# LARS-research/RED-GNN

Hardware: AMD Instinct MI355X
Metric: edges aggregated/sec + MRR-eval queries/sec, family KG n_layer=3 at 1/2/4/8 GPU (higher is better)
Workload: dtype f32; 1 GPU; C2 synthetic KG 10000 entities / 50 relations / 200000 triples (seed 1234), n_layer=3 hidden_dim=64 attn_dim=5, eval step = expansion + fused layers + GRU/readout + filtered ranking, 1024 queries per GPU; batch_per_gpu=1024, global_batch=1024

## Files before the change

include/redgnn.h:

```cpp
#ifndef REDGNN_H
#define REDGNN_H

#include <stddef.h>
#include <stdint.h>

#ifdef __cplusplus
extern "C" {
#endif

typedef struct rg_graph rg_graph;
typedef struct rg_frontier rg_frontier;

const char* rg_last_error(void);
int rg_version(void);
int rg_hipgraph_fill_nodes(void* hip_graph);

int rg_graph_create(int32_t n_ent, int32_t n_rel, const int32_t* triples_host, int64_t n,
                    int add_inverse, rg_graph** out);
int rg_graph_create_device(int32_t n_ent, int32_t n_rel, const int32_t* triples_dev, int64_t n,
                           int add_inverse, void* stream, rg_graph** out);
int rg_graph_export_packs(const rg_graph* g, int32_t* n_packs, int32_t* n_vrows, int32_t* ent_host, int32_t* pack_host, int32_t* rows_host,
                          int32_t* vrows_host);
int rg_tgraph_create(int32_t n_ent, int32_t n_rela_rows, int32_t n_time, const int32_t* quads_host, int64_t n,
                     rg_graph** out);
int rg_tgraph_create_excluding(int32_t n_ent, int32_t n_rela_rows, int32_t n_time, const int32_t* quads_host, int64_t n,
                               const int64_t* exclude_rows_host, int64_t n_exclude, rg_graph** out);
int rg_graph_destroy(rg_graph* g);
int64_t rg_graph_n_fact(const rg_graph* g);
int rg_graph_export(const rg_graph* g, int32_t* out_ptr_host, int32_t* out_rel_tail_host,
                    int32_t* in_ptr_host, int32_t* in_head_rel_host);
int rg_graph_export_time(const rg_graph* g, int32_t* out_time_host, int32_t* in_time_host);

size_t rg_frontier_workspace_bytes(int32_t n_ent, int32_t batch, int32_t n_levels);
int rg_frontier_create(int32_t n_ent, int32_t batch, int32_t n_levels, void* workspace_dev,
                       size_t workspace_bytes, rg_frontier** out);
int rg_frontier_destroy(rg_frontier* f);
int rg_frontier_reset(rg_frontier* f, const int32_t* q_sub_dev, void* stream);
int rg_frontier_reset_nodes(rg_frontier* f, const int32_t* nodes_dev, int64_t n, void* stream);
int rg_frontier_expand(rg_frontier* f, const rg_graph* g, int64_t* counts_host, void* stream);
int rg_frontier_expand_async(rg_frontier* f, const rg_graph* g, void* stream);
int rg_frontier_expand_nodes_async(rg_frontier* f, const rg_graph* g, int32_t* nodes_out, int32_t* prev_idx_out, void* stream);
int rg_frontier_set_edge_hint(rg_frontier* f, int64_t n_edges);
const int32_t* rg_frontier_count_ptr(const rg_frontier* f);
int rg_frontier_level_counts(const rg_frontier* f, int64_t* counts_host, void* stream);
int rg_frontier_nodes(const rg_frontier* f, int32_t* nodes_out, int32_t* prev_idx_out,
                      int32_t* old_nodes_new_idx_out, void* stream);
size_t rg_frontier_edges_scratch_bytes(int64_t n_new);
int rg_frontier_edges(const rg_frontier* f, const rg_graph* g, int32_t level,
                      const int32_t* nodes_new, int64_t n_new, int32_t* edges_out,
                      int32_t* row_ptr_out, void* scratch_dev, void* stream);

size_t rg_layer_fwd_scratch_bytes(const rg_frontier* f, const rg_graph* g, int32_t ld);
int rg_layer_fwd_plan(const rg_frontier* f, const rg_graph* g, int32_t level, int64_t n_old, int64_t n_new,
                      int64_t n_edges, int32_t ld);
int rg_layer_fwd(const rg_frontier* f, const rg_graph* g, int32_t level, int64_t n_new,
                 const float* hidden, const float* rela, int32_t d, int32_t ld,
                 const float* a_s, const float* a_r, const float* a_q, int32_t ap,
                 const float* w_alpha, const float* b_alpha, int32_t attn_dim,
                 float* agg_out, void* scratch_dev, size_t scratch_bytes, int32_t walk, void* stream);

int rg_attn_tables(int32_t n_layer, int32_t n_rela_rows, int32_t batch, int32_t d, int32_t ld, int32_t attn_dim, int32_t ap,
                   const float* const* rela, const float* const* Wr, const float* const* Wqr, const float* const* bqr,
                   const int64_t* q_rel, float* a_r_out, float* a_q_out, float* rela_pad_out, void* stream);

int rg_tlayer_fwd(const rg_frontier* f, const rg_graph* g, int32_t level, int64_t n_new, const int32_t* q_time,
                  const float* hidden_dir, const float* rela_dir, const float* time_dir, int32_t d, int32_t ld,
                  const float* a_s, const float* a_r, const float* a_q, int32_t ap,
                  const float* w_alpha, const float* b_alpha, int32_t attn_dim,
                  float* agg_out, void* scratch_dev, size_t scratch_bytes, void* stream);

int rg_frontier_set_window(rg_frontier* f, const int32_t* win_lo_dev, const int32_t* win_hi_dev, int32_t n_data);
int rg_xlayer_fwd(const rg_frontier* f, const rg_graph* g, int32_t level, int64_t n_new, const int32_t* q_time,
                  const int32_t* loop_time, const int32_t* row_time, int32_t n_data,
                  const float* hidden_p, const float* rela_p, const float* time_p, int32_t n_tab, int32_t d, int32_t ld,
                  const float* a_s, const float* a_r, const float* a_q, int32_t ap,
                  const float* w_alpha, const float* b_alpha, int32_t attn_dim,
                  float* agg_out, void* scratch_dev, size_t scratch_bytes, void* stream);

size_t rg_layer_bwd_scratch_bytes(const rg_frontier* f, const rg_graph* g, int32_t ld, int32_t ap);
int rg_layer_bwd(const rg_frontier* f, const rg_graph* g, int32_t level, int64_t n_old,
                 const float* hidden, const float* rela, int32_t d, int32_t ld,
                 const float* a_s, const float* a_r, const float* a_q, int32_t ap,
                 const float* w_alpha, const float* b_alpha, int32_t attn_dim,
                 const float* grad_agg,
                 float* grad_hidden, float* grad_rela, float* grad_a_s, float* grad_a_r, float* grad_a_q,
                 float* grad_w_alpha, float* grad_b_alpha,
                 void* scratch_dev, size_t scratch_bytes, void* stream);

size_t rg_tlayer_bwd_scratch_bytes(const rg_frontier* f, const rg_graph* g, int32_t ld, int32_t ap);
int rg_tlayer_bwd(const rg_frontier* f, const rg_graph* g, int32_t level, int64_t n_old, const int32_t* q_time,
                  const float* hidden_dir, const float* rela_dir, const float* time_dir, int32_t d, int32_t ld,
                  const float* a_s, const float* a_r, const float* a_q, int32_t ap,
                  const float* w_alpha, const float* b_alpha, int32_t attn_dim,
                  const float* grad_agg,
                  float* grad_hidden_dir, float* grad_rela_dir, float* grad_time_dir, float* grad_a_s, float* grad_a_r,
                  float* grad_a_q, float* grad_w_alpha,
                  void* scratch_dev, size_t scratch_bytes, void* stream);

int rg_xlayer_bwd(const rg_frontier* f, const rg_graph* g, int32_t level, int64_t n_old, const int32_t* q_time,
                  const int32_t* loop_time, const int32_t* row_time, int32_t n_data,
                  const float* hidden_p, const float* rela_p, const float* time_p, int32_t n_tab, int32_t d, int32_t ld,
                  const float* a_s, const float* a_r, const float* a_q, int32_t ap,
                  const float* w_alpha, const float* b_alpha, int32_t attn_dim,
                  const float* grad_agg,
                  float* grad_hidden_p, float* grad_rela_p, float* grad_time_p, float* grad_a_s, float* grad_a_r,
                  float* grad_a_q, float* grad_w_alpha,
                  void* scratch_dev, size_t scratch_bytes, void* stream);

int rg_dense_fwd_supported(int32_t d, int32_t attn_dim);
int rg_dense_fwd(int64_t n, int32_t d, int32_t ld, const float* agg, const float* hidden_prev,
                 const int32_t* prev_idx, const float* W_h, int32_t act,
                 const float* w_ih, const float* w_hh, const float* b_ih, const float* b_hh,
                 const float* Ws_next, int32_t attn_dim, int32_t ap, float* a_s_out,
                 const float* W_final, const int32_t* nodes, int32_t n_ent, float* scores_all,
                 float* hidden_out, int32_t precision, void* scratch, int64_t scratch_bytes, void* stream);
int64_t rg_dense_scratch_bytes(int32_t d, int32_t precision);

int rg_split3_roundtrip(const float* x, int64_t n_rows, int32_t cols, float* back, float* parts, void* stream);
int rg_split3_product_check(int32_t which, int64_t n, int32_t d, const float* agg, const float* hidden_prev, const int32_t* prev_idx,
                            const float* W_h, int32_t act, const float* w_ih, const float* w_hh, const float* b_ih, const float* b_hh,
                            float* out, void* stream);

size_t rg_gram_tn_scratch_bytes(int32_t m, int32_t n);
int rg_gram_tn(const float* g, int64_t ldg, int32_t m, const float* x, int64_t ldx, int32_t n, int64_t n_rows, float* out, float* colsum,
               void* scratch_dev, size_t scratch_bytes, void* stream);

int rg_rank(const float* scores, int32_t batch, int32_t n_ent,
            const int32_t* ans_ptr, const int32_t* ans_idx,
            const int32_t* filt_ptr, const int32_t* filt_idx,
            float* ranks_out, void* stream);

int rg_topk(const float* scores, int32_t batch, int32_t n_ent, int32_t k, const int64_t* q_key,
            const int64_t* known_keys, const int64_t* known_ptr, const int32_t* known_idx, int64_t n_keys,
            int32_t* idx_out, float* score_out, void* stream);

int rg_dense_fwd_dev(int64_t n_cap, const int32_t* n_dev, int64_t n_hint, int32_t d, int32_t ld, const float* agg, const float* hidden_prev,
                     const int32_t* prev_idx, const float* W_h, int32_t act,
                     const float* w_ih, const float* w_hh, const float* b_ih, const float* b_hh,
                     const float* Ws_next, int32_t attn_dim, int32_t ap, float* a_s_out,
                     const float* W_final, const int32_t* nodes, int32_t n_ent, float* scores_all,
                     float* hidden_out, int32_t precision, void* scratch, int64_t scratch_bytes, void* stream);

int rg_dense_train_fwd(int64_t n, int32_t d, const float* agg, const float* hidden_prev, const int32_t* prev_idx,
                       const float* W_h, int32_t act, const float* w_ih, const float* w_hh, const float* b_ih, const float* b_hh,
                       const float* mask, float* hidden_out, float* x_out, float* gates_ws_out, void* stream);

int rg_dense_train_fwd_as(int64_t n, int32_t d, const float* agg, const float* hidden_prev, const int32_t* prev_idx,
                          const float* W_h, int32_t act, const float* w_ih, const float* w_hh, const float* b_ih, const float* b_hh,
                          const float* mask, const float* Ws_next, int32_t attn_dim, int32_t ap,
                          float* hidden_out, float* x_out, float* gates_ws_out, float* a_s_out, void* stream);

int rg_rows_addmm(const float* base, int64_t ldb, const float* g, int64_t ldg, int32_t k, const float* W, int32_t n, int64_t n_rows,
                  float* out, int64_t ldo, void* stream);

int rg_dense_train_bwd(int64_t n, int32_t d, const float* grad_hidden, const float* gates_ws, const float* x, const float* mask,
                       float keep, int32_t act, const float* W_h, const float* w_ih, const float* w_hh,
                       float* grad_gates_i, float* grad_gates_h, float* grad_pre, float* grad_agg, float* grad_h0, void* stream);

int rg_dense_train_bwd2(int64_t n, int32_t d, const float* grad_hidden, const float* gates_ws, const float* x, const float* mask,
                        float keep, int32_t act, const float* W_h, const float* w_ih, const float* w_hh, const int32_t* prev_idx,
                        float* grad_gates_i, float* grad_gates_hn, float* grad_pre, float* grad_agg, float* grad_prev, void* stream);

size_t rg_explain_scratch_bytes(const rg_frontier* f);
int rg_explain_seed(const rg_frontier* f, int32_t batch, int32_t n_ent, int32_t level, const int32_t* objs, uint32_t* marks_out,
                    uint8_t* reached_out, void* stream);
int rg_explain_count(const rg_frontier* f, const rg_graph* g, int32_t batch, int32_t n_ent, int32_t level, const uint32_t* marks,
                     const float* a_s, const float* a_r, const float* a_q, int32_t ap, const float* w_alpha, const float* b_alpha,
                     int32_t attn_dim, float min_alpha, uint32_t* marks_prev_out, int32_t* word_ptr_out, void* scratch,
                     size_t scratch_bytes, int64_t* n_edges_host, void* stream);
int rg_explain_emit(const rg_frontier* f, const rg_graph* g, int32_t batch, int32_t n_ent, int32_t level, const uint32_t* marks,
                    const float* a_s, const float* a_r, const float* a_q, int32_t ap, const float* w_alpha, const float* b_alpha,
                    int32_t attn_dim, float min_alpha, const int32_t* word_ptr, int32_t* edges_out, float* alpha_out, void* stream);
int rg_explain_gather(int64_t n, int32_t hop, int32_t batch, const int32_t* edges, const float* alpha, const int64_t* row_first,
                      const int64_t* row_base, int64_t n_out, int32_t* edges_out, float* alpha_out, void* stream);

int rg_texplain_count(const rg_frontier* f, const rg_graph* g, int32_t batch, int32_t n_ent, int32_t level, const uint32_t* marks,
                      const float* a_s, const float* a_r, const float* a_q, int32_t ap, const float* w_alpha, const float* b_alpha,
                      int32_t attn_dim, float min_alpha, uint32_t* marks_prev_out, int32_t* word_ptr_out, void* scratch,
                      size_t scratch_bytes, int64_t* n_edges_host, void* stream);
int rg_texplain_emit(const rg_frontier* f, const rg_graph* g, int32_t batch, int32_t n_ent, int32_t level, const uint32_t* marks,
                     const float* a_s, const float* a_r, const float* a_q, int32_t ap, const float* w_alpha, const float* b_alpha,
                     int32_t attn_dim, float min_alpha, const int32_t* word_ptr, int32_t* edges_out, float* alpha_out,
                     int32_t* time_out, void* stream);

int rg_attn_profile(const rg_frontier* f, const rg_graph* g, int32_t batch, int32_t n_ent, int32_t level, int64_t n_old,
                    const float* a_s, const float* a_r, const float* a_q, int32_t ap, const float* w_alpha, const float* b_alpha,
                    int32_t attn_dim, int64_t* sum_out, int64_t* count_out, void* stream);

int rg_tattn_profile(const rg_frontier* f, const rg_graph* g, int32_t batch, int32_t n_ent, int32_t level, int64_t n_old,
                     const int32_t* q_time, const float* a_s, const float* a_r, const float* a_q, int32_t ap, const float* w_alpha,
                     const float* b_alpha, int32_t attn_dim, int64_t* sum_out, int64_t* count_out, void* stream);

#ifdef __cplusplus
}
#endif
#endif
```

red-gnn_amd/_lib.py:

```python
import ctypes as C
import os

_PKG = os.path.dirname(os.path.abspath(__file__))
LIB_PATH = os.environ.get("RG_LIB") or os.path.join(_PKG, "libredgnn.so")

SYMBOLS = [
    "rg_last_error", "rg_version", "rg_hipgraph_fill_nodes",
    "rg_graph_create", "rg_graph_create_device", "rg_graph_export_packs", "rg_tgraph_create", "rg_tgraph_create_excluding", "rg_graph_destroy", "rg_graph_n_fact", "rg_graph_export",
    "rg_frontier_workspace_bytes", "rg_frontier_create", "rg_frontier_destroy", "rg_frontier_reset",
    "rg_frontier_reset_nodes", "rg_frontier_expand", "rg_frontier_nodes", "rg_frontier_edges_scratch_bytes", "rg_frontier_edges",
    "rg_layer_fwd_scratch_bytes", "rg_layer_fwd", "rg_layer_fwd_plan", "rg_tlayer_fwd", "rg_xlayer_fwd", "rg_frontier_set_window", "rg_layer_bwd_scratch_bytes", "rg_layer_bwd", "rg_tlayer_bwd_scratch_bytes", "rg_tlayer_bwd", "rg_xlayer_bwd", "rg_dense_fwd_supported", "rg_dense_scratch_bytes", "rg_dense_fwd", "rg_dense_fwd_dev", "rg_dense_train_fwd", "rg_dense_train_fwd_as", "rg_rows_addmm", "rg_dense_train_bwd", "rg_dense_train_bwd2", "rg_split3_roundtrip", "rg_split3_product_check", "rg_gram_tn_scratch_bytes", "rg_gram_tn", "rg_rank",
    "rg_frontier_expand_async", "rg_frontier_expand_nodes_async", "rg_frontier_set_edge_hint", "rg_frontier_count_ptr", "rg_frontier_level_counts", "rg_attn_tables",
    "rg_explain_scratch_bytes", "rg_explain_seed", "rg_explain_count", "rg_explain_emit", "rg_explain_gather",
    "rg_topk",
    "rg_attn_profile",
    "rg_graph_export_time", "rg_texplain_count", "rg_texplain_emit", "rg_tattn_profile",
]

_lib = None


class NativeError(RuntimeError):
    pass


def lib():
    global _lib
    if _lib is not None:
        return _lib
    if not os.path.exists(LIB_PATH):
        raise NativeError(
            "libredgnn.so is missing at %s: the HIP extension is not built. Run "
            "`python -c 'import __graft_entry__ as g; g.build()'` (needs hipcc). There is no CPU fallback." % LIB_PATH)
    import torch
    L = C.CDLL(LIB_PATH)
    vp, i32, i64, sz = C.c_void_p, C.c_int32, C.c_int64, C.c_size_t
    L.rg_last_error.restype = C.c_char_p
    L.rg_version.restype = C.c_int
    L.rg_hipgraph_fill_nodes.argtypes = [vp]
    L.rg_graph_create.argtypes = [i32, i32, vp, i64, C.c_int, C.POINTER(vp)]
    L.rg_graph_create_device.argtypes = [i32, i32, vp, i64, C.c_int, vp, C.POINTER(vp)]
    L.rg_graph_export_packs.argtypes = [vp, C.POINTER(i32), C.POINTER(i32), vp, vp, vp, vp]
    L.rg_tgraph_create.argtypes = [i32, i32, i32, vp, i64, C.POINTER(vp)]
    L.rg_tgraph_create_excluding.argtypes = [i32, i32, i32, vp, i64, vp, i64, C.POINTER(vp)]
    L.rg_graph_destroy.argtypes = [vp]
    L.rg_graph_n_fact.argtypes = [vp]
    L.rg_graph_n_fact.restype = i64
    L.rg_graph_export.argtypes = [vp, vp, vp, vp, vp]
    L.rg_frontier_workspace_bytes.argtypes = [i32, i32, i32]
    L.rg_frontier_workspace_bytes.restype = sz
    L.rg_frontier_create.argtypes = [i32, i32, i32, vp, sz, C.POINTER(vp)]
    L.rg_frontier_destroy.argtypes = [vp]
    L.rg_frontier_reset.argtypes = [vp, vp, vp]
    L.rg_frontier_reset_nodes.argtypes = [vp, vp, i64, vp]
    L.rg_frontier_expand.argtypes = [vp, vp, C.POINTER(i64), vp]
    L.rg_frontier_expand_async.argtypes = [vp, vp, vp]
    L.rg_frontier_expand_nodes_async.argtypes = [vp, vp, vp, vp, vp]
    L.rg_frontier_set_edge_hint.argtypes = [vp, i64]
    L.rg_attn_tables.argtypes = [i32, i32, i32, i32, i32, i32, i32, vp, vp, vp, vp, vp, vp, vp, vp, vp]
    L.rg_frontier_count_ptr.argtypes = [vp]
    L.rg_frontier_count_ptr.restype = vp
    L.rg_frontier_level_counts.argtypes = [vp, C.POINTER(i64), vp]
    L.rg_frontier_nodes.argtypes = [vp, vp, vp, vp, vp]
    L.rg_frontier_edges_scratch_bytes.argtypes = [i64]
    L.rg_frontier_edges_scratch_bytes.restype = sz
    L.rg_frontier_edges.argtypes = [vp, vp, i32, vp, i64, vp, vp, vp, vp]
    L.rg_layer_fwd_scratch_bytes.argtypes = [vp, vp, i32]
    L.rg_layer_fwd_scratch_bytes.restype = sz
    L.rg_layer_fwd.argtypes = [vp, vp, i32, i64, vp, vp, i32, i32, vp, vp, vp, i32, vp, vp, i32, vp, vp, sz, i32, vp]
    L.rg_layer_fwd_plan.argtypes = [vp, vp, i32, i64, i64, i64, i32]
    L.rg_tlayer_fwd.argtypes = [vp, vp, i32, i64, vp, vp, vp, vp, i32, i32, vp, vp, vp, i32, vp, vp, i32, vp, vp, sz, vp]
    L.rg_xlayer_fwd.argtypes = [vp, vp, i32, i64, vp, vp, vp, i32, vp, vp, vp, i32, i32, i32, vp, vp, vp, i32, vp, vp, i32, vp, vp, sz, vp]
    L.rg_frontier_set_window.argtypes = [vp, vp, vp, i32]
    L.rg_layer_bwd_scratch_bytes.argtypes = [vp, vp, i32, i32]
    L.rg_layer_bwd_scratch_bytes.restype = sz
    L.rg_layer_bwd.argtypes = [vp, vp, i32, i64, vp, vp, i32, i32, vp, vp, vp, i32, vp, vp, i32,
                               vp, vp, vp, vp, vp, vp, vp, vp, vp, sz, vp]
    L.rg_tlayer_bwd_scratch_bytes.argtypes = [vp, vp, i32, i32]
    L.rg_tlayer_bwd_scratch_bytes.restype = sz
    L.rg_tlayer_bwd.argtypes = [vp, vp, i32, i64, vp, vp, vp, vp, i32, i32, vp, vp, vp, i32, vp, vp, i32,
                                vp, vp, vp, vp, vp, vp, vp, vp, vp, sz, vp]
    L.rg_xlayer_bwd.argtypes = [vp, vp, i32, i64, vp, vp, vp, i32, vp, vp, vp, i32, i32, i32, vp, vp, vp, i32, vp, vp, i32,
                                vp, vp, vp, vp, vp, vp, vp, vp, vp, sz, vp]
    L.rg_dense_fwd_supported.argtypes = [i32, i32]
    L.rg_dense_fwd.argtypes = [i64, i32, i32, vp, vp, vp, vp, i32, vp, vp, vp, vp, vp, i32, i32, vp, vp, vp, i32, vp, vp, i32, vp, i64, vp]
    L.rg_dense_scratch_bytes.argtypes = [i32, i32]
    L.rg_dense_scratch_bytes.restype = i64
    L.rg_dense_fwd_dev.argtypes = [i64, vp, i64, i32, i32, vp, vp, vp, vp, i32, vp, vp, vp, vp, vp, i32, i32, vp, vp, vp, i32, vp, vp, i32, vp, i64, vp]
    L.rg_dense_train_fwd.argtypes = [i64, i32, vp, vp, vp, vp, i32, vp, vp, vp, vp, vp, vp, vp, vp, vp]
    L.rg_dense_train_fwd_as.argtypes = [i64, i32, vp, vp, vp, vp, i32, vp, vp, vp, vp, vp, vp, i32, i32, vp, vp, vp, vp, vp]
    L.rg_rows_addmm.argtypes = [vp, i64, vp, i64, i32, vp, i32, i64, vp, i64, vp]
    L.rg_dense_train_bwd.argtypes = [i64, i32, vp, vp, vp, vp, C.c_float, i32, vp, vp, vp, vp, vp, vp, vp, vp, vp]
    L.rg_dense_train_bwd2.argtypes = [i64, i32, vp, vp, vp, vp, C.c_float, i32, vp, vp, vp, vp, vp, vp, vp, vp, vp, vp]
    L.rg_rank.argtypes = [vp, i32, i32, vp, vp, vp, vp, vp, vp]
    L.rg_topk.argtypes = [vp, i32, i32, i32, vp, vp, vp, vp, i64, vp, vp, vp]
    L.rg_split3_roundtrip.argtypes = [vp, i64, i32, vp, vp, vp]
    L.rg_gram_tn_scratch_bytes.argtypes = [i32, i32]
    L.rg_gram_tn_scratch_bytes.restype = sz
    L.rg_gram_tn.argtypes = [vp, i64, i32, vp, i64, i32, i64, vp, vp, vp, sz, vp]
    L.rg_split3_product_check.argtypes = [i32, i64, i32, vp, vp, vp, vp, i32, vp, vp, vp, vp, vp, vp]
    L.rg_explain_scratch_bytes.argtypes = [vp]
    L.rg_explain_scratch_bytes.restype = sz
    L.rg_explain_seed.argtypes = [vp, i32, i32, i32, vp, vp, vp, vp]
    L.rg_explain_count.argtypes = [vp, vp, i32, i32, i32, vp, vp, vp, vp, i32, vp, vp, i32, C.c_float, vp, vp, vp, sz,
                                   C.POINTER(i64), vp]
    L.rg_explain_emit.argtypes = [vp, vp, i32, i32, i32, vp, vp, vp, vp, i32, vp, vp, i32, C.c_float, vp, vp, vp, vp]
    L.rg_explain_gather.argtypes = [i64, i32, i32, vp, vp, vp, vp, i64, vp, vp, vp]
    L.rg_attn_profile.argtypes = [vp, vp, i32, i32, i32, i64, vp, vp, vp, i32, vp, vp, i32, vp, vp, vp]
    L.rg_graph_export_time.argtypes = [vp, vp, vp]
    L.rg_texplain_count.argtypes = L.rg_explain_count.argtypes
    L.rg_texplain_emit.argtypes = [vp, vp, i32, i32, i32, vp, vp, vp, vp, i32, vp, vp, i32, C.c_float, vp, vp, vp, vp, vp]
    L.rg_tattn_profile.argtypes = [vp, vp, i32, i32, i32, i64, vp, vp, vp, vp, i32, vp, vp, i32, vp, vp, vp]
    _lib = L
    return L


def check(rc):
    if rc != 0:
        raise NativeError(lib().rg_last_error().decode("utf-8", "replace"))


def ptr(t):
    if t is None:
        return None
    if hasattr(t, "data_ptr"):
        return C.c_void_p(t.data_ptr())
    return C.c_void_p(t.ctypes.data)


def stream_ptr():
    import torch
    return C.c_void_p(torch.cuda.current_stream().cuda_stream)
```

red-gnn_amd/csrc/common.h:

```cpp
#pragma once
#include <hip/hip_runtime.h>
#include <stdint.h>
#include <stdio.h>
#include <string>
#include <type_traits>

#include "redgnn.h"

namespace rg {

void set_error(const char* fmt, ...);

#define RG_CHECK(cond, ...)                 \
  do {                                      \
    if (!(cond)) {                          \
      ::rg::set_error(__VA_ARGS__);         \
      return 1;                             \
    }                                       \
  } while (0)

#define RG_HIP(expr)                                                                  \
  do {                                                                                \
    hipError_t e_ = (expr);                                                           \
    if (e_ != hipSuccess) {                                                           \
      ::rg::set_error("%s failed: %s (%s:%d)", #expr, hipGetErrorString(e_), __FILE__, \
                      __LINE__);                                                      \
      return 1;                                                                       \
    }                                                                                 \
  } while (0)

#define RG_LAUNCH_CHECK() RG_HIP(hipGetLastError())

int zero_async(void* p, size_t bytes, hipStream_t s);
int zero2_async(void* p1, size_t bytes1, void* p2, size_t bytes2, hipStream_t s);
int copy_words_async(void* dst, const void* src, int n_words, hipStream_t s);

static inline int64_t ceil_div(int64_t a, int64_t b) { return (a + b - 1) / b; }
static inline size_t align_up(size_t x, size_t a) { return (x + a - 1) / a * a; }

size_t scan_scratch_elems(int64_t n);
int scan_exclusive(const uint32_t* in, int32_t* out, int64_t n, bool popc, int32_t* total_dev,
                   int32_t* scratch, hipStream_t s);

template <typename F>
inline int with_ap4(int ap4, const char* who, F&& f) {
  switch (ap4) {
    case 1: return f(std::integral_constant<int, 1>());
    case 2: return f(std::integral_constant<int, 2>());
    case 3: return f(std::integral_constant<int, 3>());
    case 4: return f(std::integral_constant<int, 4>());
    case 8: return f(std::integral_constant<int, 8>());
    default: set_error("%s: padded attention dim %d not in {4,8,12,16,32}", who, ap4 * 4); return 1;
  }
}

template <typename F>
inline int with_g(int ld4, F&& f) {
  if (ld4 <= 4) return f(std::integral_constant<int, 4>());
  if (ld4 <= 8) return f(std::integral_constant<int, 8>());
  if (ld4 <= 16) return f(std::integral_constant<int, 16>());
  if (ld4 <= 32) return f(std::integral_constant<int, 32>());
  return f(std::integral_constant<int, 64>());
}

__device__ __forceinline__ float4 f4zero() { return make_float4(0.f, 0.f, 0.f, 0.f); }

template <int CTRL>
__device__ __forceinline__ float dpp_add(float v) {
  const int t = __builtin_amdgcn_update_dpp(0, __float_as_int(v), CTRL, 0xf, 0xf, false);
  return v + __int_as_float(t);
}

template <int G>
__device__ __forceinline__ float group_sum(float v) {
  if constexpr (G >= 16) {
    v = dpp_add<0x128>(v);
    v = dpp_add<0x124>(v);
    v = dpp_add<0x122>(v);
    v = dpp_add<0x121>(v);
    if constexpr (G >= 32) v += __shfl_xor(v, 16, 64);
    if constexpr (G >= 64) v += __shfl_xor(v, 32, 64);
  } else {
    for (int o = G / 2; o > 0; o >>= 1) v += __shfl_xor(v, o, 64);
  }
  return v;
}

}

#include <vector>
namespace rg { int place_rows_best_fit(const int4* vrows, int32_t n_vrows, std::vector<int4>* place, std::vector<int32_t>* pack_nrows); }

constexpr int RG_VROW_MAX = 128;
struct rg_vrows {
  int32_t n = 0, n_split = 0, n_slots = 0;
  int4* rows = nullptr;
  int4* split = nullptr;
};

constexpr int RG_PACK = 128;
struct rg_packs {
  int32_t n = 0;
  int2* ent = nullptr;
  int4* pack = nullptr;
  int2* rows = nullptr;
};

struct rg_graph {
  void* arena = nullptr;
  int32_t n_ent = 0, n_rel = 0;
  int32_t n_rela_rows = 0;
  int32_t n_time = 0;
  int32_t* in_time = nullptr;
  int32_t* out_time = nullptr;
  int64_t n_fact = 0;
  int32_t max_in_deg = 0, max_out_deg = 0;
  int32_t* out_ptr = nullptr;
  int2* out_rt = nullptr;
  int32_t* in_ptr = nullptr;
  int2* in_hr = nullptr;
  uint32_t* in_pk = nullptr;
  uint32_t* out_pk = nullptr;
  rg_vrows in_vr, out_vr;
  rg_packs in_pk_packs;
  int32_t* rel_ptr = nullptr;
  int2* rel_ht = nullptr;
  rg_vrows rel_vr;
  int32_t* rel_tm = nullptr;
  int32_t* time_ptr = nullptr;
  int2* time_ht = nullptr;
  int32_t* time_rel = nullptr;
  rg_vrows time_vr;
};

constexpr int RG_MAX_LEVELS = 16;
constexpr int RG_QSTRIDE = 32;
constexpr size_t RG_QUEUE_BYTES = 8 * RG_QSTRIDE * sizeof(int32_t);
struct rg_frontier {
  int32_t n_ent = 0, B = 0, BW = 0, W = 0, n_levels = 0;
  uint32_t* bitsT[2] = {nullptr, nullptr};
  int2* bm[RG_MAX_LEVELS] = {};
  uint32_t* words_tmp = nullptr;
  int32_t* prefix_tmp = nullptr;
  int32_t* scan_scratch = nullptr;
  int32_t* counters = nullptr;
  const int32_t* win_lo = nullptr;
  const int32_t* win_hi = nullptr;
  int32_t win_n_data = 0;
  mutable bool queues_clean = false;
  int32_t* queues = nullptr;
  int64_t* counts_pinned = nullptr;
  int level = -1;
  int tcur = 0;
  int64_t n_nodes[RG_MAX_LEVELS] = {};
  int64_t n_edges = 0;
  int64_t edge_hint = -1;
  const int2* bm_of(int lvl) const { return bm[lvl % n_levels]; }
};
```

red-gnn_amd/csrc/frontier.hip:

```cpp
#include <string.h>

#include "attn.h"

namespace {

__global__ void reset_level0_kernel(const int32_t* __restrict__ q_sub, int B, int n_ent, int BW, int W, uint32_t* __restrict__ bitsT,
                                    int2* __restrict__ bm0, int32_t* __restrict__ counters) {
  const int64_t i = (int64_t)blockIdx.x * blockDim.x + threadIdx.x;
  if (i >= (int64_t)B * W) return;
  const int b = (int)(i / W), w = (int)(i - (int64_t)b * W);
  const int e = q_sub[b];
  const bool ok = e >= 0 && e < n_ent;
  const int ew = ok ? e >> 5 : W;
  bm0[i] = make_int2(w == ew ? (int)(1u << (e & 31)) : 0, b + (w > ew ? 1 : 0));
  if (w == 0) {
    if (ok) atomicOr(&bitsT[(int64_t)e * BW + (b >> 5)], 1u << (b & 31));
    else atomicOr((unsigned*)&counters[1], 1u);
    if (b == 0) { counters[0] = B; counters[4] = B; }
  }
}

__device__ __forceinline__ void end_of_hop(int32_t* __restrict__ counters, int32_t* __restrict__ queues, int slot, int t) {
  if (t < 4) {
    const int32_t v = counters[t];
    if (slot >= 0) counters[slot + t] = v;
    counters[8 + t] = v;
  }
  if (t >= 8 && t < 16) queues[(t - 8) * RG_QSTRIDE] = 0;
}
__global__ void snapshot_kernel(int32_t* __restrict__ counters, int32_t* __restrict__ queues, int slot) {
  end_of_hop(counters, queues, slot, threadIdx.x);
  __syncthreads();
  if (threadIdx.x == 0) { counters[2] = 0; counters[3] = 0; }
}

__global__ void reset_nodes_kernel(const int32_t* __restrict__ nodes, int64_t n, int B, int n_ent, int BW,
                                   uint32_t* __restrict__ bitsT, int32_t* counters) {
  const int64_t i = (int64_t)blockIdx.x * blockDim.x + threadIdx.x;
  if (i >= n) return;
  const int b = nodes[2 * i], e = nodes[2 * i + 1];
  if (e < 0 || e >= n_ent || b < 0 || b >= B) { atomicOr((unsigned*)&counters[1], 1u); return; }
  atomicOr(&bitsT[(int64_t)e * BW + (b >> 5)], 1u << (b & 31));
}

__global__ __launch_bounds__(256) void hop_or_kernel(const int4* __restrict__ vrows, int n_vrows,
                                                     const int2* __restrict__ in_hr, const uint32_t* __restrict__ oldT,
                                                     uint32_t* __restrict__ newT, int BW, int WL) {
  const int wave = (blockIdx.x * blockDim.x + threadIdx.x) >> 6;
  const int lane = threadIdx.x & 63;
  if (wave >= n_vrows) return;
  const int4 row = vrows[wave];
  const int t = row.x, beg = row.y, end = row.y + row.z;
  const int wl = lane & (WL - 1);
  const int el = lane / WL, EL = 64 / WL;
  for (int w0 = 0; w0 < BW; w0 += WL) {
    const int w = w0 + wl;
    uint32_t acc = 0;
    if (w < BW) {
      for (int j = beg + el; j < end; j += 4 * EL) {
        int hh[4];
#pragma unroll
        for (int u = 0; u < 4; ++u) hh[u] = (j + u * EL < end) ? in_hr[j + u * EL].x : -1;
#pragma unroll
        for (int u = 0; u < 4; ++u)
          if (hh[u] >= 0) acc |= oldT[(int64_t)hh[u] * BW + w];
      }
    }
    for (int o = WL; o < 64; o <<= 1) acc |= __shfl_xor(acc, o, 64);
    if (el == 0 && w < BW && acc) atomicOr(&newT[(int64_t)t * BW + w], acc);
  }
}

__global__ __launch_bounds__(256) void hop_or_window_kernel(const int4* __restrict__ vrows, int n_vrows, const int2* __restrict__ in_hr,
                                                            const int32_t* __restrict__ in_row, const uint32_t* __restrict__ oldT,
                                                            uint32_t* __restrict__ newT, int BW, int WL, int B, const int32_t* __restrict__ win_lo,
                                                            const int32_t* __restrict__ win_hi, int n_data, unsigned long long* total) {
  const int wave = (blockIdx.x * blockDim.x + threadIdx.x) >> 6;
  const int lane = threadIdx.x & 63;
  if (wave >= n_vrows) return;
  const int4 row = vrows[wave];
  const int t = row.x, beg = row.y, end = row.y + row.z;
  const int wl = lane & (WL - 1);
  const int el = lane / WL, EL = 64 / WL;
  unsigned long long cnt = 0;
  for (int w0 = 0; w0 < BW; w0 += WL) {
    const int w = w0 + wl;
    uint32_t acc = 0;
    if (w < BW) {
      for (int j = beg + el; j < end; j += EL) {
        uint32_t v = oldT[(int64_t)in_hr[j].x * BW + w];
        if (v) {
          const int r = in_row[j];
          if (r < n_data) {
            uint32_t m = 0;
            for (uint32_t rest = v; rest; rest &= rest - 1) {
              const int bit = __ffs((int)rest) - 1, b = w * 32 + bit;
              if (b < B && r >= win_lo[b] && r < win_hi[b]) m |= 1u << bit;
            }
            v = m;
          }
          acc |= v;
          cnt += __popc(v);
        }
      }
    }
    for (int o = WL; o < 64; o <<= 1) acc |= __shfl_xor(acc, o, 64);
    if (el == 0 && w < BW && acc) atomicOr(&newT[(int64_t)t * BW + w], acc);
  }
  for (int o = 32; o > 0; o >>= 1) cnt += __shfl_down(cnt, o, 64);
  if (lane == 0 && cnt) atomicAdd(total, cnt);
}

__global__ __launch_bounds__(256) void hop_prologue_kernel(const int32_t* __restrict__ out_ptr,
                                                           const uint32_t* __restrict__ oldT, uint32_t* __restrict__ newT,
                                                           int n_ent, int BW, unsigned long long* total) {
  const int64_t i = (int64_t)blockIdx.x * blockDim.x + threadIdx.x;
  unsigned long long v = 0;
  if (i < (int64_t)n_ent * BW) {
    const int h = (int)(i / BW);
    if (out_ptr) v = (unsigned long long)(out_ptr[h + 1] - out_ptr[h]) * __popc(oldT[i]);
    newT[i] = 0u;
  }
  for (int o = 32; o > 0; o >>= 1) v += __shfl_down(v, o, 64);
  __shared__ unsigned long long ws[4];
  if ((threadIdx.x & 63) == 0) ws[threadIdx.x >> 6] = v;
  __syncthreads();
  if (threadIdx.x == 0) {
    unsigned long long s = ws[0] + ws[1] + ws[2] + ws[3];
    if (s) atomicAdd(total, s);
  }
}

__global__ __launch_bounds__(256) void transpose_kernel(const uint32_t* __restrict__ bitsT, uint32_t* __restrict__ words,
                                                        int n_ent, int B, int BW, int W, int n_pairs) {
  const int wave = (blockIdx.x * blockDim.x + threadIdx.x) >> 6;
  const int lane = threadIdx.x & 63;
  if (wave >= BW * n_pairs) return;
  const int bw = wave / n_pairs, pair = wave - bw * n_pairs;
  const int e = pair * 64 + lane;
  const uint32_t v = (e < n_ent) ? bitsT[(int64_t)e * BW + bw] : 0u;
  uint32_t lo = 0, hi = 0;
#pragma unroll
  for (int b = 0; b < 32; ++b) {
    const unsigned long long m = __ballot((v >> b) & 1u);
    if (lane == b) { lo = (uint32_t)m; hi = (uint32_t)(m >> 32); }
  }
  const int batch = bw * 32 + lane;
  if (lane < 32 && batch < B) {
    const int ew = pair * 2;
    words[(int64_t)batch * W + ew] = lo;
    if (ew + 1 < W) words[(int64_t)batch * W + ew + 1] = hi;
  }
}

__global__ void pack_kernel(const uint32_t* __restrict__ words, const int32_t* __restrict__ prefix,
                            int2* __restrict__ bm, int64_t n) {
  const int64_t i = (int64_t)blockIdx.x * blockDim.x + threadIdx.x;
  if (i < n) bm[i] = make_int2((int)words[i], prefix[i]);
}

__global__ void emit_nodes_kernel(const int2* __restrict__ bm_new, const int2* __restrict__ bm_old, int B, int W,
                                  int32_t* __restrict__ nodes, int32_t* __restrict__ prev_idx,
                                  int32_t* __restrict__ old_new) {
  const int64_t t = (int64_t)blockIdx.x * blockDim.x + threadIdx.x;
  const int64_t i = t >> 5;
  const int pos = (int)(t & 31);
  if (i >= (int64_t)B * W) return;
  const int2 nw = bm_new[i];
  if (!rg::bm_has(nw, pos)) return;
  const int64_t idx = rg::bm_rank(nw, pos);
  const int b = (int)(i / W), w = (int)(i - (int64_t)b * W);
  if (nodes) reinterpret_cast<int2*>(nodes)[idx] = make_int2(b, w * 32 + pos);
  if (prev_idx || old_new) {
    int prev = -1;
    if (bm_old) {
      const int2 ow = bm_old[i];
      if (rg::bm_has(ow, pos)) prev = rg::bm_rank(ow, pos);
    }
    if (prev_idx) prev_idx[idx] = prev;
    if (old_new && prev >= 0) old_new[prev] = (int32_t)idx;
  }
}

__device__ __forceinline__ int rank_in(const int2* __restrict__ bm, int b, int W, int e, bool* present) {
  const int2 wp = bm[(int64_t)b * W + (e >> 5)];
  *present = rg::bm_has(wp, e);
  return rg::bm_rank(wp, e);
}

__global__ void edge_count_kernel(const int32_t* __restrict__ nodes_new, int64_t n_new, const int32_t* __restrict__ in_ptr,
                                  const int2* __restrict__ in_hr, const int2* __restrict__ bm_old, int W,
                                  uint32_t* __restrict__ deg) {
  const int64_t i = (int64_t)blockIdx.x * blockDim.x + threadIdx.x;
  if (i >= n_new) return;
  const int b = nodes_new[2 * i], t = nodes_new[2 * i + 1];
  int c = 0;
  for (int j = in_ptr[t]; j < in_ptr[t + 1]; ++j) {
    bool p;
    rank_in(bm_old, b, W, in_hr[j].x, &p);
    c += p;
  }
  deg[i] = c;
}

__global__ void edge_fill_kernel(const int32_t* __restrict__ nodes_new, int64_t n_new, const int32_t* __restrict__ in_ptr,
                                 const int2* __restrict__ in_hr, const int2* __restrict__ bm_old, int W,
                                 const int32_t* __restrict__ row_ptr, int32_t* __restrict__ edges) {
  const int64_t i = (int64_t)blockIdx.x * blockDim.x + threadIdx.x;
  if (i >= n_new) return;
  const int b = nodes_new[2 * i], t = nodes_new[2 * i + 1];
  int64_t o = row_ptr[i];
  for (int j = in_ptr[t]; j < in_ptr[t + 1]; ++j) {
    const int2 hr = in_hr[j];
    bool p;
    const int s = rank_in(bm_old, b, W, hr.x, &p);
    if (p) {
      int32_t* e = edges + 6 * o;
      e[0] = b; e[1] = hr.x; e[2] = hr.y; e[3] = t; e[4] = s; e[5] = (int32_t)i;
      ++o;
    }
  }
}

constexpr int SMALL_T = 1024;
constexpr int SMALL_MAX_WORDS = 12288;

__global__ __launch_bounds__(SMALL_T) void build_level_small_kernel(const uint32_t* __restrict__ bitsT, int n_ent, int B, int BW, int W,
                                                                    int n_pairs, int2* __restrict__ bm_new, const int2* __restrict__ bm_old,
                                                                    int32_t* __restrict__ counters, int32_t* __restrict__ queues, int slot,
                                                                    int32_t* __restrict__ nodes, int32_t* __restrict__ prev_idx,
                                                                    int32_t* __restrict__ old_new) {
  extern __shared__ uint32_t words[];
  __shared__ int32_t wsum[SMALL_T / 64];
  const int lane = threadIdx.x & 63, wv = threadIdx.x >> 6;
  const int nw = B * W;
  for (int task = wv; task < BW * n_pairs; task += SMALL_T / 64) {
    const int bw = task / n_pairs, pair = task - bw * n_pairs;
    const int e = pair * 64 + lane;
    const uint32_t v = (e < n_ent) ? bitsT[(int64_t)e * BW + bw] : 0u;
    uint32_t lo = 0, hi = 0;
#pragma unroll
    for (int b = 0; b < 32; ++b) {
      const unsigned long long m = __ballot((v >> b) & 1u);
      if (lane == b) { lo = (uint32_t)m; hi = (uint32_t)(m >> 32); }
    }
    const int batch = bw * 32 + lane;
    if (lane < 32 && batch < B) {
      words[batch * W + 2 * pair] = lo;
      if (2 * pair + 1 < W) words[batch * W + 2 * pair + 1] = hi;
    }
  }
  __syncthreads();
  const int per = (nw + SMALL_T - 1) / SMALL_T;
  const int beg = min((int)threadIdx.x * per, nw), end = min(beg + per, nw);
  int32_t sum = 0;
  for (int i = beg; i < end; ++i) sum += __popc(words[i]);
  int32_t inc = sum;
#pragma unroll
  for (int o = 1; o < 64; o <<= 1) {
    const int32_t t = __shfl_up(inc, o, 64);
    if (lane >= o) inc += t;
  }
  if (lane == 63) wsum[wv] = inc;
  __syncthreads();
  int32_t pre = inc - sum, total = 0;
  for (int w = 0; w < SMALL_T / 64; ++w) {
    const int32_t x = wsum[w];
    if (w < wv) pre += x;
    total += x;
  }
  for (int i = beg; i < end; ++i) {
    uint32_t w = words[i];
    bm_new[i] = make_int2((int)w, pre);
    if (nodes || prev_idx || old_new) {
      const int b = i / W, e0 = (i - b * W) * 32;
      uint32_t ow = 0; int op = 0;
      if ((prev_idx || old_new) && bm_old) { const int2 o = bm_old[i]; ow = (uint32_t)o.x; op = o.y; }
      int idx = pre;
      for (uint32_t rest = w; rest; rest &= rest - 1, ++idx) {
        const int pos = __ffs((int)rest) - 1;
        if (nodes) reinterpret_cast<int2*>(nodes)[idx] = make_int2(b, e0 + pos);
        const int prev = ((ow >> pos) & 1u) ? op + __popc(ow & ((1u << pos) - 1u)) : -1;
        if (prev_idx) prev_idx[idx] = prev;
        if (old_new && prev >= 0) old_new[prev] = idx;
      }
    }
    pre += __popc(w);
  }
  const int t = threadIdx.x;
  if (t < 4) {
    const int32_t v = t == 0 ? total : counters[t];
    if (t == 0) counters[0] = total;
    if (slot >= 0) counters[slot + t] = v;
    counters[8 + t] = v;
  }
  if (t >= 8 && t < 16) queues[(t - 8) * RG_QSTRIDE] = 0;
  __syncthreads();
  if (t == 0) { counters[2] = 0; counters[3] = 0; }
}

__global__ void set_last_kernel(int32_t* row_ptr, int64_t n, const int32_t* total) { row_ptr[n] = *total; }

size_t ws_layout(int32_t n_ent, int32_t B, int32_t n_levels, size_t* off ) {
  const size_t BW = (B + 31) / 32, W = (n_ent + 31) / 32;
  size_t o = 0;
  auto take = [&](size_t bytes) { size_t r = o; o = rg::align_up(o + bytes, 256); return r; };
  off[0] = take((size_t)n_ent * BW * 4);
  off[1] = take((size_t)n_ent * BW * 4);
  off[2] = take((size_t)B * W * 4);
  off[3] = take((size_t)B * W * 4);
  off[4] = take(rg::scan_scratch_elems((int64_t)B * W) * 4);
  off[5] = take(1024 + RG_QUEUE_BYTES);
  off[6] = take((size_t)n_levels * B * W * 8);
  return o;
}

}

extern "C" {

size_t rg_frontier_workspace_bytes(int32_t n_ent, int32_t batch, int32_t n_levels) {
  if (n_ent <= 0 || batch <= 0 || n_levels < 2 || n_levels > RG_MAX_LEVELS) return 0;
  size_t off[8];
  return ws_layout(n_ent, batch, n_levels, off);
}

int rg_frontier_create(int32_t n_ent, int32_t batch, int32_t n_levels, void* ws, size_t ws_bytes, rg_frontier** out) {
  RG_CHECK(out != nullptr, "rg_frontier_create: out is NULL");
  *out = nullptr;
  RG_CHECK(n_ent > 0 && batch > 0, "rg_frontier_create: n_ent=%d batch=%d must be positive", n_ent, batch);
  RG_CHECK(n_levels >= 2 && n_levels <= RG_MAX_LEVELS, "rg_frontier_create: n_levels=%d not in [2,%d]", n_levels, RG_MAX_LEVELS);
  RG_CHECK((int64_t)n_ent * batch < ((int64_t)1 << 31), "rg_frontier_create: batch*n_ent = %lld does not fit int32",
           (long long)n_ent * batch);
  size_t off[8];
  const size_t need = ws_layout(n_ent, batch, n_levels, off);
  RG_CHECK(ws != nullptr && ws_bytes >= need, "rg_frontier_create: workspace %zu B < required %zu B", ws_bytes, need);
  RG_CHECK(((uintptr_t)ws & 255) == 0, "rg_frontier_create: workspace must be 256-B aligned");
  rg_frontier* f = new rg_frontier();
  f->n_ent = n_ent; f->B = batch; f->BW = (batch + 31) / 32; f->W = (n_ent + 31) / 32; f->n_levels = n_levels;
  char* base = (char*)ws;
  f->bitsT[0] = (uint32_t*)(base + off[0]);
  f->bitsT[1] = (uint32_t*)(base + off[1]);
  f->words_tmp = (uint32_t*)(base + off[2]);
  f->prefix_tmp = (int32_t*)(base + off[3]);
  f->scan_scratch = (int32_t*)(base + off[4]);
  f->counters = (int32_t*)(base + off[5]);
  f->queues = f->counters + 256;
  for (int l = 0; l < n_levels; ++l) f->bm[l] = (int2*)(base + off[6] + (size_t)l * batch * f->W * 8);
  if (hipHostMalloc((void**)&f->counts_pinned, 1024, hipHostMallocDefault) != hipSuccess) {
    delete f;
    rg::set_error("rg_frontier_create: hipHostMalloc failed");
    return 1;
  }
  *out = f;
  return 0;
}

int rg_frontier_destroy(rg_frontier* f) {
  if (!f) return 0;
  if (f->counts_pinned) (void)hipHostFree(f->counts_pinned);
  delete f;
  return 0;
}

static int build_level(rg_frontier* f, hipStream_t s) {
  const int n_pairs = (f->W + 1) / 2;
  const int64_t waves = (int64_t)f->BW * n_pairs;
  hipLaunchKernelGGL(transpose_kernel, dim3(rg::ceil_div(waves, 4)), dim3(256), 0, s, f->bitsT[f->tcur], f->words_tmp,
                     f->n_ent, f->B, f->BW, f->W, n_pairs);
  RG_LAUNCH_CHECK();
  const int64_t nw = (int64_t)f->B * f->W;
  if (rg::scan_exclusive(f->words_tmp, f->prefix_tmp, nw, true, &f->counters[0], f->scan_scratch, s)) return 1;
  hipLaunchKernelGGL(pack_kernel, dim3(rg::ceil_div(nw, 256)), dim3(256), 0, s, f->words_tmp, f->prefix_tmp,
                     f->bm[f->level % f->n_levels], nw);
  RG_LAUNCH_CHECK();
  return 0;
}

int rg_frontier_reset(rg_frontier* f, const int32_t* q_sub, void* stream) {
  RG_CHECK(f && q_sub, "rg_frontier_reset: NULL argument");
  hipStream_t s = (hipStream_t)stream;
  f->level = 0; f->tcur = 0; f->n_edges = 0;
  if (rg::zero2_async(f->bitsT[0], rg::align_up((size_t)f->n_ent * f->BW * 4, 16), f->counters, 1024, s)) return 1;
  f->queues_clean = false;
  const int64_t nw = (int64_t)f->B * f->W;
  hipLaunchKernelGGL(reset_level0_kernel, dim3(rg::ceil_div(nw, 256)), dim3(256), 0, s, q_sub, f->B, f->n_ent, f->BW, f->W,
                     f->bitsT[0], f->bm[0], f->counters);
  RG_LAUNCH_CHECK();
  f->n_nodes[0] = f->B;
  return 0;
}

int rg_frontier_set_window(rg_frontier* f, const int32_t* win_lo, const int32_t* win_hi, int32_t n_data) {
  RG_CHECK(f != nullptr, "rg_frontier_set_window: frontier is NULL");
  RG_CHECK((win_lo == nullptr) == (win_hi == nullptr) && n_data >= 0, "rg_frontier_set_window: give both bounds (or neither)");
  f->win_lo = win_lo; f->win_hi = win_hi; f->win_n_data = n_data;
  return 0;
}

int rg_frontier_reset_nodes(rg_frontier* f, const int32_t* nodes, int64_t n, void* stream) {
  RG_CHECK(f && (nodes || n == 0) && n >= 0, "rg_frontier_reset_nodes: bad argument");
  hipStream_t s = (hipStream_t)stream;
  f->level = 0; f->tcur = 0; f->n_edges = 0;
  if (rg::zero2_async(f->bitsT[0], rg::align_up((size_t)f->n_ent * f->BW * 4, 16), f->counters, 1024, s)) return 1;
  f->queues_clean = false;
  if (n > 0) {
    hipLaunchKernelGGL(reset_nodes_kernel, dim3(rg::ceil_div(n, 256)), dim3(256), 0, s, nodes, n, f->B, f->n_ent, f->BW,
                       f->bitsT[0], f->counters);
    RG_LAUNCH_CHECK();
  }
  if (build_level(f, s)) return 1;
  if (rg::copy_words_async(&f->counters[4], &f->counters[0], 1, s)) return 1;
  f->n_nodes[0] = n;
  return 0;
}

static int enqueue_expand(rg_frontier* f, const rg_graph* g, hipStream_t s, int32_t* nodes = nullptr, int32_t* prev_idx = nullptr) {
  const uint32_t* oldT = f->bitsT[f->tcur];
  uint32_t* newT = f->bitsT[f->tcur ^ 1];
  int WL = 1;
  while (WL < f->BW && WL < 64) WL <<= 1;
  const bool windowed = f->win_lo != nullptr;
  RG_CHECK(!windowed || g->in_time, "rg_frontier_expand: time windows are set but the graph carries no data-row ids (rg_tgraph_create)");
  hipLaunchKernelGGL(hop_prologue_kernel, dim3(rg::ceil_div((int64_t)f->n_ent * f->BW, 256)), dim3(256), 0, s,
                     windowed ? (const int32_t*)nullptr : g->out_ptr, oldT, newT, f->n_ent, f->BW, (unsigned long long*)&f->counters[2]);
  RG_LAUNCH_CHECK();
  if (windowed)
    hipLaunchKernelGGL(hop_or_window_kernel, dim3(rg::ceil_div(g->in_vr.n, 4)), dim3(256), 0, s, g->in_vr.rows, g->in_vr.n, g->in_hr,
                       g->in_time, oldT, newT, f->BW, WL, f->B, f->win_lo, f->win_hi, f->win_n_data, (unsigned long long*)&f->counters[2]);
  else
    hipLaunchKernelGGL(hop_or_kernel, dim3(rg::ceil_div(g->in_vr.n, 4)), dim3(256), 0, s, g->in_vr.rows, g->in_vr.n, g->in_hr,
                       oldT, newT, f->BW, WL);
  RG_LAUNCH_CHECK();
  f->tcur ^= 1;
  f->level += 1;
  const int slot = f->level < RG_MAX_LEVELS ? 64 + 8 * f->level : -1;
  const int64_t nw = (int64_t)f->B * f->W;
  const int2* bm_old = f->bm_of(f->level - 1);
  if (nw <= SMALL_MAX_WORDS) {
    const bool split_emit = (nodes || prev_idx) && nw > 1024;
    hipLaunchKernelGGL(build_level_small_kernel, dim3(1), dim3(SMALL_T), (size_t)nw * 4, s, f->bitsT[f->tcur], f->n_ent, f->B, f->BW,
                       f->W, (f->W + 1) / 2, f->bm[f->level % f->n_levels], bm_old, f->counters, f->queues, slot,
                       split_emit ? (int32_t*)nullptr : nodes, split_emit ? (int32_t*)nullptr : prev_idx, (int32_t*)nullptr);
    RG_LAUNCH_CHECK();
    if (split_emit) {
      hipLaunchKernelGGL(emit_nodes_kernel, dim3(rg::ceil_div(nw * 32, 256)), dim3(256), 0, s, f->bm_of(f->level), bm_old, f->B, f->W,
                         nodes, prev_idx, (int32_t*)nullptr);
      RG_LAUNCH_CHECK();
    }
  } else {
    if (build_level(f, s)) return 1;
    hipLaunchKernelGGL(snapshot_kernel, dim3(1), dim3(64), 0, s, f->counters, f->queues, slot);
    RG_LAUNCH_CHECK();
    if (nodes || prev_idx) {
      hipLaunchKernelGGL(emit_nodes_kernel, dim3(rg::ceil_div(nw * 32, 256)), dim3(256), 0, s, f->bm_of(f->level), bm_old, f->B, f->W,
                         nodes, prev_idx, (int32_t*)nullptr);
      RG_LAUNCH_CHECK();
    }
  }
  f->queues_clean = true;
  return 0;
}

int rg_frontier_expand(rg_frontier* f, const rg_graph* g, int64_t* counts_host, void* stream) {
  RG_CHECK(f && g, "rg_frontier_expand: NULL argument");
  RG_CHECK(f->level >= 0, "rg_frontier_expand: call rg_frontier_reset first");
  RG_CHECK(g->n_ent == f->n_ent, "rg_frontier_expand: graph has %d entities, frontier %d", g->n_ent, f->n_ent);
  hipStream_t s = (hipStream_t)stream;
  const int64_t n_old = f->n_nodes[f->level % f->n_levels];
  if (enqueue_expand(f, g, s)) return 1;
  RG_HIP(hipMemcpyAsync(f->counts_pinned, f->counters, 64, hipMemcpyDeviceToHost, s));
  RG_HIP(hipStreamSynchronize(s));
  const int32_t* c32 = (const int32_t*)f->counts_pinned;
  RG_CHECK(c32[1] == 0, "rg_frontier_expand: a start node had batch or entity id out of range");
  RG_CHECK(f->level != 1 || n_old < 0 || c32[4] == n_old, "rg_frontier_expand: %lld start nodes given but %d distinct (duplicates?)",
           (long long)n_old, c32[4]);
  const int64_t n_new = c32[8];
  int64_t e;
  memcpy(&e, &c32[10], 8);
  f->n_nodes[f->level % f->n_levels] = n_new;
  f->n_edges = e;
  if (counts_host) { counts_host[0] = n_new; counts_host[1] = e; counts_host[2] = n_old; counts_host[3] = f->level; }
  return 0;
}

int rg_frontier_expand_async(rg_frontier* f, const rg_graph* g, void* stream) {
  return rg_frontier_expand_nodes_async(f, g, nullptr, nullptr, stream);
}

int rg_frontier_expand_nodes_async(rg_frontier* f, const rg_graph* g, int32_t* nodes_out, int32_t* prev_idx_out, void* stream) {
  RG_CHECK(f && g, "rg_frontier_expand_async: NULL argument");
  RG_CHECK(f->level >= 0, "rg_frontier_expand_async: call rg_frontier_reset first");
  RG_CHECK(g->n_ent == f->n_ent, "rg_frontier_expand_async: graph has %d entities, frontier %d", g->n_ent, f->n_ent);
  RG_CHECK(f->level + 1 < RG_MAX_LEVELS, "rg_frontier_expand_async: at most %d levels", RG_MAX_LEVELS - 1);
  RG_CHECK(!nodes_out || ((uintptr_t)nodes_out & 7) == 0, "rg_frontier_expand_nodes_async: nodes_out must be 8-byte aligned");
  if (enqueue_expand(f, g, (hipStream_t)stream, nodes_out, prev_idx_out)) return 1;
  f->n_nodes[f->level % f->n_levels] = -1;
  f->n_edges = -1;
  f->edge_hint = -1;
  return 0;
}

int rg_frontier_set_edge_hint(rg_frontier* f, int64_t n_edges) {
  RG_CHECK(f != nullptr, "rg_frontier_set_edge_hint: NULL frontier");
  f->edge_hint = n_edges;
  return 0;
}

const int32_t* rg_frontier_count_ptr(const rg_frontier* f) { return f ? f->counters : nullptr; }

int rg_frontier_level_counts(const rg_frontier* f, int64_t* counts_host, void* stream) {
  RG_CHECK(f && counts_host, "rg_frontier_level_counts: NULL argument");
  RG_CHECK(f->level >= 0 && f->level < RG_MAX_LEVELS, "rg_frontier_level_counts: level %d", f->level);
  hipStream_t s = (hipStream_t)stream;
  int32_t* host = (int32_t*)f->counts_pinned + 16;
  RG_HIP(hipMemcpyAsync(host, &f->counters[64], sizeof(int32_t) * 8 * (f->level + 1), hipMemcpyDeviceToHost, s));
  RG_HIP(hipStreamSynchronize(s));
  counts_host[0] = f->n_nodes[0]; counts_host[1] = 0;
  for (int l = 1; l <= f->level; ++l) {
    const int32_t* c = host + 8 * l;
    RG_CHECK(c[1] == 0, "rg_frontier_level_counts: a start node had batch or entity id out of range");
    counts_host[2 * l] = c[0];
    memcpy(&counts_host[2 * l + 1], &c[2], 8);
  }
  return 0;
}

int rg_frontier_nodes(const rg_frontier* f, int32_t* nodes, int32_t* prev_idx, int32_t* old_new, void* stream) {
  RG_CHECK(f && f->level >= 0, "rg_frontier_nodes: frontier not initialised");
  hipStream_t s = (hipStream_t)stream;
  const int2* bm_old = f->level > 0 ? f->bm_of(f->level - 1) : nullptr;
  RG_CHECK(!(old_new && !bm_old), "rg_frontier_nodes: level 0 has no previous level");
  const int64_t nw = (int64_t)f->B * f->W;
  RG_CHECK(!nodes || ((uintptr_t)nodes & 7) == 0, "rg_frontier_nodes: nodes_out must be 8-byte aligned");
  hipLaunchKernelGGL(emit_nodes_kernel, dim3(rg::ceil_div(nw * 32, 256)), dim3(256), 0, s, f->bm_of(f->level), bm_old, f->B, f->W,
                     nodes, prev_idx, old_new);
  RG_LAUNCH_CHECK();
  return 0;
}

size_t rg_frontier_edges_scratch_bytes(int64_t n_new) {
  return rg::align_up((size_t)(n_new + 1) * 4, 256) + rg::scan_scratch_elems(n_new) * 4 + 256;
}

int rg_frontier_edges(const rg_frontier* f, const rg_graph* g, int32_t level, const int32_t* nodes_new, int64_t n_new,
                      int32_t* edges, int32_t* row_ptr, void* scratch, void* stream) {
  RG_CHECK(f && g && nodes_new && row_ptr && scratch, "rg_frontier_edges: NULL argument");
  RG_CHECK(level >= 1 && level <= f->level && level > f->level - f->n_levels + 1,
           "rg_frontier_edges: level %d not resident (current %d, %d kept)", level, f->level, f->n_levels);
  RG_CHECK(n_new == f->n_nodes[level % f->n_levels], "rg_frontier_edges: n_new=%lld but level %d has %lld nodes",
           (long long)n_new, level, (long long)f->n_nodes[level % f->n_levels]);
  hipStream_t s = (hipStream_t)stream;
  uint32_t* deg = (uint32_t*)scratch;
  int32_t* scan_scr = (int32_t*)((char*)scratch + rg::align_up((size_t)(n_new + 1) * 4, 256));
  int32_t* total = scan_scr;
  const int2* bm_old = f->bm_of(level - 1);
  if (n_new == 0) return rg::zero_async(row_ptr, 4, s);
  hipLaunchKernelGGL(edge_count_kernel, dim3(rg::ceil_div(n_new, 256)), dim3(256), 0, s, nodes_new, n_new, g->in_ptr,
                     g->in_hr, bm_old, f->W, deg);
  RG_LAUNCH_CHECK();
  if (rg::scan_exclusive(deg, row_ptr, n_new, false, total, scan_scr + 64, s)) return 1;
  hipLaunchKernelGGL(set_last_kernel, dim3(1), dim3(1), 0, s, row_ptr, n_new, total);
  RG_LAUNCH_CHECK();
  if (edges) {
    hipLaunchKernelGGL(edge_fill_kernel, dim3(rg::ceil_div(n_new, 256)), dim3(256), 0, s, nodes_new, n_new, g->in_ptr,
                       g->in_hr, bm_old, f->W, row_ptr, edges);
    RG_LAUNCH_CHECK();
  }
  return 0;
}

}
```

red-gnn_amd/csrc/graph.hip:

```cpp
#include <stdarg.h>
#include <string.h>

#include <algorithm>
#include <vector>

#include "common.h"

namespace rg {

static thread_local std::string g_err;

void set_error(const char* fmt, ...) {
  char buf[1024];
  va_list ap;
  va_start(ap, fmt);
  vsnprintf(buf, sizeof(buf), fmt, ap);
  va_end(ap);
  g_err = buf;
}

constexpr int SCAN_T = 256;
constexpr int SCAN_ITEMS = 8;
constexpr int SCAN_TILE = SCAN_T * SCAN_ITEMS;

template <bool POPC>
__device__ __forceinline__ int32_t scan_load(const uint32_t* in, int64_t i, int64_t n) {
  if (i >= n) return 0;
  uint32_t v = in[i];
  return POPC ? __popc(v) : (int32_t)v;
}

__device__ __forceinline__ int32_t wave_incl_scan(int32_t v) {
  const int lane = threadIdx.x & 63;
#pragma unroll
  for (int o = 1; o < 64; o <<= 1) {
    int32_t t = __shfl_up(v, o, 64);
    if (lane >= o) v += t;
  }
  return v;
}

__device__ __forceinline__ int32_t block_excl_scan(int32_t v, int32_t* block_total) {
  __shared__ int32_t wsum[SCAN_T / 64];
  const int lane = threadIdx.x & 63, w = threadIdx.x >> 6;
  int32_t inc = wave_incl_scan(v);
  if (lane == 63) wsum[w] = inc;
  __syncthreads();
  int32_t base = 0, tot = 0;
#pragma unroll
  for (int i = 0; i < SCAN_T / 64; ++i) {
    int32_t x = wsum[i];
    if (i < w) base += x;
    tot += x;
  }
  __syncthreads();
  *block_total = tot;
  return base + inc - v;
}

template <bool POPC>
__global__ __launch_bounds__(SCAN_T) void scan_reduce_kernel(const uint32_t* in, int64_t n, int32_t* sums) {
  const int64_t base = (int64_t)blockIdx.x * SCAN_TILE + (int64_t)threadIdx.x * SCAN_ITEMS;
  int32_t acc = 0;
#pragma unroll
  for (int i = 0; i < SCAN_ITEMS; ++i) acc += scan_load<POPC>(in, base + i, n);
  int32_t tot;
  block_excl_scan(acc, &tot);
  if (threadIdx.x == 0) sums[blockIdx.x] = tot;
}

template <bool POPC>
__global__ __launch_bounds__(SCAN_T) void scan_apply_kernel(const uint32_t* in, int32_t* out, int64_t n,
                                                            const int32_t* offsets, int32_t* total) {
  const int64_t base = (int64_t)blockIdx.x * SCAN_TILE + (int64_t)threadIdx.x * SCAN_ITEMS;
  int32_t v[SCAN_ITEMS];
  int32_t acc = 0;
#pragma unroll
  for (int i = 0; i < SCAN_ITEMS; ++i) {
    v[i] = scan_load<POPC>(in, base + i, n);
    acc += v[i];
  }
  int32_t tot;
  int32_t ex = block_excl_scan(acc, &tot);
  if (offsets) ex += offsets[blockIdx.x];
#pragma unroll
  for (int i = 0; i < SCAN_ITEMS; ++i) {
    if (base + i < n) out[base + i] = ex;
    ex += v[i];
  }
  if (!offsets && total && threadIdx.x == 0) *total = tot;
}

__global__ void zero_words_kernel(uint32_t* __restrict__ p, int64_t n_words) {
  const int64_t stride = (int64_t)gridDim.x * blockDim.x;
  for (int64_t i = (int64_t)blockIdx.x * blockDim.x + threadIdx.x; i < n_words; i += stride) p[i] = 0u;
}
__global__ void zero_quads_kernel(uint4* __restrict__ p, int64_t n_quads) {
  const int64_t stride = (int64_t)gridDim.x * blockDim.x;
  for (int64_t i = (int64_t)blockIdx.x * blockDim.x + threadIdx.x; i < n_quads; i += stride) p[i] = make_uint4(0u, 0u, 0u, 0u);
}
__global__ void copy_words_kernel(uint32_t* __restrict__ dst, const uint32_t* __restrict__ src, int n) {
  if ((int)threadIdx.x < n) dst[threadIdx.x] = src[threadIdx.x];
}

int zero_async(void* p, size_t bytes, hipStream_t s) {
  if (bytes == 0) return 0;
  RG_CHECK(((uintptr_t)p & 3) == 0 && (bytes & 3) == 0, "zero_async: unaligned fill (%p, %zu B)", p, bytes);
  if (((uintptr_t)p & 15) == 0 && (bytes & 15) == 0 && bytes >= 4096) {
    const int64_t n = (int64_t)(bytes / 16);
    hipLaunchKernelGGL(zero_quads_kernel, dim3((unsigned)std::min<int64_t>(ceil_div(n, 256), 4096)), dim3(256), 0, s, (uint4*)p, n);
  } else {
    const int64_t n = (int64_t)(bytes / 4);
    hipLaunchKernelGGL(zero_words_kernel, dim3((unsigned)std::min<int64_t>(ceil_div(n, 256), 4096)), dim3(256), 0, s, (uint32_t*)p, n);
  }
  RG_LAUNCH_CHECK();
  return 0;
}

__global__ void zero2_quads_kernel(uint4* __restrict__ p1, int64_t n1, uint4* __restrict__ p2, int64_t n2) {
  const int64_t stride = (int64_t)gridDim.x * blockDim.x;
  for (int64_t i = (int64_t)blockIdx.x * blockDim.x + threadIdx.x; i < n1 + n2; i += stride) {
    if (i < n1) p1[i] = make_uint4(0u, 0u, 0u, 0u);
    else p2[i - n1] = make_uint4(0u, 0u, 0u, 0u);
  }
}

int zero2_async(void* p1, size_t bytes1, void* p2, size_t bytes2, hipStream_t s) {
  if ((((uintptr_t)p1 | (uintptr_t)p2) & 15) != 0 || ((bytes1 | bytes2) & 15) != 0) return zero_async(p1, bytes1, s) || zero_async(p2, bytes2, s);
  const int64_t n = (int64_t)((bytes1 + bytes2) / 16);
  if (n == 0) return 0;
  hipLaunchKernelGGL(zero2_quads_kernel, dim3((unsigned)std::min<int64_t>(ceil_div(n, 256), 4096)), dim3(256), 0, s, (uint4*)p1,
                     (int64_t)(bytes1 / 16), (uint4*)p2, (int64_t)(bytes2 / 16));
  RG_LAUNCH_CHECK();
  return 0;
}

int copy_words_async(void* dst, const void* src, int n_words, hipStream_t s) {
  RG_CHECK(n_words > 0 && n_words <= 256, "copy_words_async: %d words", n_words);
  hipLaunchKernelGGL(copy_words_kernel, dim3(1), dim3(256), 0, s, (uint32_t*)dst, (const uint32_t*)src, n_words);
  RG_LAUNCH_CHECK();
  return 0;
}

size_t scan_scratch_elems(int64_t n) {
  size_t tot = 0;
  while (n > SCAN_TILE) {
    n = ceil_div(n, SCAN_TILE);
    tot += align_up((size_t)n, 64) * 2;
  }
  return tot + 64;
}

int scan_exclusive(const uint32_t* in, int32_t* out, int64_t n, bool popc, int32_t* total_dev,
                   int32_t* scratch, hipStream_t s) {
  if (n <= 0) {
    if (total_dev && zero_async(total_dev, sizeof(int32_t), s)) return 1;
    return 0;
  }
  const int64_t nb = ceil_div(n, SCAN_TILE);
  if (nb == 1) {
    if (popc)
      hipLaunchKernelGGL(scan_apply_kernel<true>, dim3(1), dim3(SCAN_T), 0, s, in, out, n, nullptr, total_dev);
    else
      hipLaunchKernelGGL(scan_apply_kernel<false>, dim3(1), dim3(SCAN_T), 0, s, in, out, n, nullptr, total_dev);
    RG_LAUNCH_CHECK();
    return 0;
  }
  int32_t* sums = scratch;
  int32_t* sums_scanned = scratch + align_up((size_t)nb, 64);
  int32_t* next = sums_scanned + align_up((size_t)nb, 64);
  if (popc)
    hipLaunchKernelGGL(scan_reduce_kernel<true>, dim3(nb), dim3(SCAN_T), 0, s, in, n, sums);
  else
    hipLaunchKernelGGL(scan_reduce_kernel<false>, dim3(nb), dim3(SCAN_T), 0, s, in, n, sums);
  RG_LAUNCH_CHECK();
  if (scan_exclusive((const uint32_t*)sums, sums_scanned, nb, false, total_dev, next, s)) return 1;
  if (popc)
    hipLaunchKernelGGL(scan_apply_kernel<true>, dim3(nb), dim3(SCAN_T), 0, s, in, out, n, sums_scanned, nullptr);
  else
    hipLaunchKernelGGL(scan_apply_kernel<false>, dim3(nb), dim3(SCAN_T), 0, s, in, out, n, sums_scanned, nullptr);
  RG_LAUNCH_CHECK();
  return 0;
}

}

struct HostVrows { std::vector<int4> rows, split; };
static void host_vrows(const std::vector<int32_t>& ptr, int32_t n_ent, HostVrows* h, rg_vrows* out) {
  std::vector<int4>& rows = h->rows;
  std::vector<int4>& split = h->split;
  int32_t slots = 0;
  for (int32_t e = 0; e < n_ent; ++e) {
    const int32_t beg = ptr[e], len = ptr[e + 1] - ptr[e];
    if (len <= RG_VROW_MAX) {
      rows.push_back(make_int4(e, beg, len, -1));
    } else {
      const int32_t n_seg = (len + RG_VROW_MAX - 1) / RG_VROW_MAX;
      split.push_back(make_int4(e, slots, n_seg, 0));
      for (int32_t k = 0; k < n_seg; ++k) {
        const int32_t b = beg + k * RG_VROW_MAX;
        rows.push_back(make_int4(e, b, std::min(RG_VROW_MAX, beg + len - b), slots + k));
      }
      slots += n_seg;
    }
  }
  std::stable_sort(rows.begin(), rows.end(), [](const int4& a, const int4& b) { return a.z > b.z; });
  out->n = (int32_t)rows.size(); out->n_split = (int32_t)split.size(); out->n_slots = slots;
}

struct HostPacks { std::vector<int2> ent; std::vector<int4> pack; std::vector<int2> rows; };

namespace rg {
int place_rows_best_fit(const int4* vrows, int32_t n_vrows, std::vector<int4>* place, std::vector<int32_t>* pack_nrows) {
  std::vector<int32_t> open_by_room[RG_PACK + 1];
  std::vector<int32_t> fill;
  place->assign(n_vrows, make_int4(-1, 0, 0, 0));
  pack_nrows->clear();
  for (int32_t i = 0; i < n_vrows; ++i) {
    const int4& r = vrows[i];
    if (r.z <= 0) continue;
    int32_t p;
    if (r.w >= 0) { p = (int32_t)fill.size(); fill.push_back(0); pack_nrows->push_back(0); }
    else {
      int room = r.z;
      while (room <= RG_PACK && open_by_room[room].empty()) ++room;
      if (room > RG_PACK) { p = (int32_t)fill.size(); fill.push_back(0); pack_nrows->push_back(0); room = RG_PACK; }
      else { p = open_by_room[room].back(); open_by_room[room].pop_back(); }
      if (room - r.z > 0) open_by_room[room - r.z].push_back(p);
    }
    (*place)[i] = make_int4(p, fill[p], (*pack_nrows)[p], 0);
    fill[p] += r.z;
    (*pack_nrows)[p] += 1;
  }
  return (int)fill.size();
}
}

static void host_packs(const std::vector<int4>& vrows, const std::vector<uint32_t>& in_pk, HostPacks* hp, rg_packs* out) {
  std::vector<int4> place;
  std::vector<int32_t> pack_nrows;
  const size_t n = (size_t)rg::place_rows_best_fit(vrows.data(), (int32_t)vrows.size(), &place, &pack_nrows);
  std::vector<int32_t> row0(n + 1, 0);
  for (size_t p = 0; p < n; ++p) row0[p + 1] = row0[p] + pack_nrows[p];
  hp->ent.assign(n * RG_PACK, make_int2(-1, 0));
  hp->pack.resize(n);
  hp->rows.resize(row0[n]);
  for (size_t i = 0; i < vrows.size(); ++i) {
    const int4& r = vrows[i];
    const int4& pl = place[i];
    if (pl.x < 0) continue;
    for (int32_t j = 0; j < r.z; ++j) hp->ent[(size_t)pl.x * RG_PACK + pl.y + j] = make_int2((int32_t)in_pk[r.y + j], pl.z);
    hp->rows[row0[pl.x] + pl.z] = make_int2(r.x, r.w);
    if (pl.z == 0) hp->pack[pl.x] = make_int4(row0[pl.x], pack_nrows[pl.x], r.w, r.x);
  }
  out->n = (int32_t)n;
}

struct Arena {
  struct Item { void** field; const void* src; size_t bytes, off; };
  std::vector<Item> items;
  size_t total = 0;
  template <typename P, typename V>
  void add(P** field, const V& v) {
    const size_t bytes = v.size() * sizeof(typename V::value_type);
    items.push_back({(void**)field, (const void*)v.data(), bytes, total});
    total += rg::align_up(std::max<size_t>(bytes, 16), 256);
  }
};

extern "C" {

const char* rg_last_error(void) { return rg::g_err.c_str(); }
int rg_version(void) { return 10; }

static int build_graph(int32_t n_ent, int32_t n_rel, int32_t n_rela_rows, const std::vector<int32_t>& H,
                       const std::vector<int32_t>& R, const std::vector<int32_t>& T, const std::vector<int32_t>* TIME,
                       int32_t n_time, rg_graph** out) {
  const int64_t n_fact = (int64_t)H.size();
  std::vector<int32_t> out_ptr(n_ent + 1, 0), in_ptr(n_ent + 1, 0);
  for (int64_t i = 0; i < n_fact; ++i) { out_ptr[H[i] + 1]++; in_ptr[T[i] + 1]++; }
  int32_t max_in = 0, max_out = 0;
  for (int32_t e = 0; e < n_ent; ++e) {
    max_out = out_ptr[e + 1] > max_out ? out_ptr[e + 1] : max_out;
    max_in = in_ptr[e + 1] > max_in ? in_ptr[e + 1] : max_in;
    out_ptr[e + 1] += out_ptr[e];
    in_ptr[e + 1] += in_ptr[e];
  }
  std::vector<int2> out_rt(n_fact), in_hr(n_fact);
  std::vector<int32_t> in_time(TIME ? n_fact : 0), out_time(TIME ? n_fact : 0);
  {
    std::vector<int32_t> po(out_ptr.begin(), out_ptr.end() - 1), pi(in_ptr.begin(), in_ptr.end() - 1);
    for (int64_t i = 0; i < n_fact; ++i) {
      const int32_t q = pi[T[i]]++;
      in_hr[q] = make_int2(H[i], R[i]);
      if (TIME) in_time[q] = (*TIME)[i];
    }
    std::vector<int32_t> by_rel(n_fact), out_fact(n_fact);
    {
      std::vector<int32_t> pr(n_rela_rows + 1, 0);
      for (int64_t i = 0; i < n_fact; ++i) pr[R[i] + 1]++;
      for (int32_t r = 0; r < n_rela_rows; ++r) pr[r + 1] += pr[r];
      for (int64_t i = 0; i < n_fact; ++i) by_rel[pr[R[i]]++] = (int32_t)i;
    }
    for (int64_t k = 0; k < n_fact; ++k) out_fact[po[H[by_rel[k]]]++] = by_rel[k];
    for (int64_t j = 0; j < n_fact; ++j) {
      const int32_t i = out_fact[j];
      out_rt[j] = make_int2(R[i], T[i]);
      if (TIME) out_time[j] = (*TIME)[i];
    }
  }
  rg_graph* g = new rg_graph();
  g->n_ent = n_ent; g->n_rel = n_rel; g->n_rela_rows = n_rela_rows; g->n_time = n_time;
  g->n_fact = n_fact; g->max_in_deg = max_in; g->max_out_deg = max_out;
  Arena A;
  A.add(&g->out_ptr, out_ptr); A.add(&g->in_ptr, in_ptr); A.add(&g->out_rt, out_rt); A.add(&g->in_hr, in_hr);
  if (TIME) { A.add(&g->in_time, in_time); A.add(&g->out_time, out_time); }
  std::vector<uint32_t> in_pk, out_pk;
  if (n_ent <= (1 << 20) && n_rela_rows <= (1 << 12)) {
    in_pk.resize(n_fact); out_pk.resize(n_fact);
    for (int64_t i = 0; i < n_fact; ++i) {
      in_pk[i] = ((uint32_t)in_hr[i].y << 20) | (uint32_t)in_hr[i].x;
      out_pk[i] = ((uint32_t)out_rt[i].x << 20) | (uint32_t)out_rt[i].y;
    }
    A.add(&g->in_pk, in_pk); A.add(&g->out_pk, out_pk);
  }
  std::vector<int32_t> rel_ptr(n_rela_rows + 1, 0), rel_tm(TIME ? n_fact : 0);
  std::vector<int2> rel_ht(n_fact);
  for (int64_t i = 0; i < n_fact; ++i) rel_ptr[R[i] + 1]++;
  for (int32_t r = 0; r < n_rela_rows; ++r) rel_ptr[r + 1] += rel_ptr[r];
  {
    std::vector<int32_t> pr(rel_ptr.begin(), rel_ptr.end() - 1);
    for (int64_t i = 0; i < n_fact; ++i) {
      const int32_t q = pr[R[i]]++;
      rel_ht[q] = make_int2(H[i], T[i]);
      if (TIME) rel_tm[q] = (*TIME)[i];
    }
  }
  A.add(&g->rel_ptr, rel_ptr); A.add(&g->rel_ht, rel_ht);
  std::vector<int32_t> time_ptr, time_rel;
  std::vector<int2> time_ht;
  HostVrows hv_in, hv_out, hv_rel, hv_time;
  if (TIME) {
    A.add(&g->rel_tm, rel_tm);
    time_ptr.assign(n_time + 1, 0); time_rel.resize(n_fact); time_ht.resize(n_fact);
    for (int64_t i = 0; i < n_fact; ++i) time_ptr[(*TIME)[i] + 1]++;
    for (int32_t t = 0; t < n_time; ++t) time_ptr[t + 1] += time_ptr[t];
    std::vector<int32_t> pt(time_ptr.begin(), time_ptr.end() - 1);
    for (int64_t i = 0; i < n_fact; ++i) {
      const int32_t q = pt[(*TIME)[i]]++;
      time_ht[q] = make_int2(H[i], T[i]);
      time_rel[q] = R[i];
    }
    A.add(&g->time_ptr, time_ptr); A.add(&g->time_ht, time_ht); A.add(&g->time_rel, time_rel);
    host_vrows(time_ptr, n_time, &hv_time, &g->time_vr);
    A.add(&g->time_vr.rows, hv_time.rows); A.add(&g->time_vr.split, hv_time.split);
  }
  host_vrows(in_ptr, n_ent, &hv_in, &g->in_vr);
  host_vrows(out_ptr, n_ent, &hv_out, &g->out_vr);
  host_vrows(rel_ptr, n_rela_rows, &hv_rel, &g->rel_vr);
  A.add(&g->in_vr.rows, hv_in.rows); A.add(&g->in_vr.split, hv_in.split);
  A.add(&g->out_vr.rows, hv_out.rows); A.add(&g->out_vr.split, hv_out.split);
  A.add(&g->rel_vr.rows, hv_rel.rows); A.add(&g->rel_vr.split, hv_rel.split);
  HostPacks hp;
  if (!TIME && !in_pk.empty() && n_rela_rows < (1 << 12)) {
    host_packs(hv_in.rows, in_pk, &hp, &g->in_pk_packs);
    A.add(&g->in_pk_packs.ent, hp.ent); A.add(&g->in_pk_packs.pack, hp.pack); A.add(&g->in_pk_packs.rows, hp.rows);
  }

  std::vector<char> staging(A.total);
  for (const Arena::Item& it : A.items)
    if (it.bytes) memcpy(staging.data() + it.off, it.src, it.bytes);
  hipError_t e = hipMalloc(&g->arena, A.total);
  if (e == hipSuccess) e = hipMemcpy(g->arena, staging.data(), A.total, hipMemcpyHostToDevice);
  if (e != hipSuccess) {
    rg::set_error("rg_graph_create: uploading %zu B failed: %s", A.total, hipGetErrorString(e));
    rg_graph_destroy(g);
    return 1;
  }
  for (const Arena::Item& it : A.items) *it.field = (char*)g->arena + it.off;
  *out = g;
  return 0;
}

int rg_graph_create(int32_t n_ent, int32_t n_rel, const int32_t* triples, int64_t n, int add_inverse,
                    rg_graph** out) {
  RG_CHECK(out != nullptr, "rg_graph_create: out is NULL");
  *out = nullptr;
  RG_CHECK(n_ent > 0 && n_rel > 0, "rg_graph_create: n_ent=%d n_rel=%d must be positive", n_ent, n_rel);
  RG_CHECK(n >= 0 && (n == 0 || triples != nullptr), "rg_graph_create: bad triples (n=%lld)", (long long)n);
  const int64_t n_fact = (add_inverse ? 2 * n : n) + n_ent;
  RG_CHECK(n_fact < (int64_t)1 << 31, "rg_graph_create: %lld fact rows do not fit int32", (long long)n_fact);
  std::vector<int32_t> H(n_fact), R(n_fact), T(n_fact);
  const int32_t max_rel = add_inverse ? n_rel : 2 * n_rel;
  for (int64_t i = 0; i < n; ++i) {
    const int32_t h = triples[3 * i], r = triples[3 * i + 1], t = triples[3 * i + 2];
    RG_CHECK(h >= 0 && h < n_ent && t >= 0 && t < n_ent && r >= 0 && r < max_rel,
             "rg_graph_create: triple %lld = (%d,%d,%d) out of range", (long long)i, h, r, t);
    H[i] = h; R[i] = r; T[i] = t;
    if (add_inverse) { H[n + i] = t; R[n + i] = r + n_rel; T[n + i] = h; }
  }
  const int64_t id0 = n_fact - n_ent;
  for (int32_t e = 0; e < n_ent; ++e) { H[id0 + e] = e; R[id0 + e] = 2 * n_rel; T[id0 + e] = e; }
  return build_graph(n_ent, n_rel, 2 * n_rel + 1, H, R, T, nullptr, 0, out);
}

static int tgraph_create(const char* who, int32_t n_ent, int32_t n_rela_rows, int32_t n_time, const int32_t* quads, int64_t n,
                         const int64_t* exclude, int64_t n_exclude, rg_graph** out) {
  RG_CHECK(out != nullptr, "%s: out is NULL", who);
  *out = nullptr;
  RG_CHECK(n_ent > 0 && n_rela_rows > 0 && n_time > 0, "%s: n_ent=%d n_rela_rows=%d n_time=%d must be positive", who, n_ent, n_rela_rows, n_time);
  RG_CHECK(n >= 0 && n < ((int64_t)1 << 31) && (n == 0 || quads != nullptr), "%s: bad quadruples (n=%lld)", who, (long long)n);
  RG_CHECK(n_exclude >= 0 && (n_exclude == 0 || exclude != nullptr), "%s: bad exclusion list", who);
  std::vector<char> drop(n_exclude ? n : 0, 0);
  for (int64_t k = 0; k < n_exclude; ++k) {
    RG_CHECK(exclude[k] >= 0 && exclude[k] < n, "%s: excluded row %lld out of range (n=%lld)", who, (long long)exclude[k], (long long)n);
    drop[exclude[k]] = 1;
  }
  std::vector<int32_t> H, R, T, TM;
  H.reserve(n); R.reserve(n); T.reserve(n); TM.reserve(n);
  for (int64_t i = 0; i < n; ++i) {
    if (n_exclude && drop[i]) continue;
    const int32_t h = quads[4 * i], r = quads[4 * i + 1], t = quads[4 * i + 2], tm = quads[4 * i + 3];
    RG_CHECK(h >= 0 && h < n_ent && t >= 0 && t < n_ent && r >= 0 && r < n_rela_rows && tm >= 0 && tm < n_time,
             "%s: quadruple %lld = (%d,%d,%d,%d) out of range", who, (long long)i, h, r, t, tm);
    H.push_back(h); R.push_back(r); T.push_back(t); TM.push_back(tm);
  }
  return build_graph(n_ent, 0, n_rela_rows, H, R, T, &TM, n_time, out);
}

int rg_tgraph_create(int32_t n_ent, int32_t n_rela_rows, int32_t n_time, const int32_t* quads, int64_t n, rg_graph** out) {
  return tgraph_create("rg_tgraph_create", n_ent, n_rela_rows, n_time, quads, n, nullptr, 0, out);
}

int rg_tgraph_create_excluding(int32_t n_ent, int32_t n_rela_rows, int32_t n_time, const int32_t* quads, int64_t n,
                               const int64_t* exclude_rows, int64_t n_exclude, rg_graph** out) {
  return tgraph_create("rg_tgraph_create_excluding", n_ent, n_rela_rows, n_time, quads, n, exclude_rows, n_exclude, out);
}

int rg_graph_destroy(rg_graph* g) {
  if (!g) return 0;
  if (g->arena) (void)hipFree(g->arena);
  delete g;
  return 0;
}

int64_t rg_graph_n_fact(const rg_graph* g) { return g ? g->n_fact : -1; }

int rg_graph_export(const rg_graph* g, int32_t* out_ptr, int32_t* out_rt, int32_t* in_ptr, int32_t* in_hr) {
  RG_CHECK(g != nullptr, "rg_graph_export: graph is NULL");
  if (out_ptr) RG_HIP(hipMemcpy(out_ptr, g->out_ptr, (g->n_ent + 1) * sizeof(int32_t), hipMemcpyDeviceToHost));
  if (in_ptr) RG_HIP(hipMemcpy(in_ptr, g->in_ptr, (g->n_ent + 1) * sizeof(int32_t), hipMemcpyDeviceToHost));
  if (out_rt) RG_HIP(hipMemcpy(out_rt, g->out_rt, g->n_fact * sizeof(int2), hipMemcpyDeviceToHost));
  if (in_hr) RG_HIP(hipMemcpy(in_hr, g->in_hr, g->n_fact * sizeof(int2), hipMemcpyDeviceToHost));
  return 0;
}

int rg_graph_export_time(const rg_graph* g, int32_t* out_time, int32_t* in_time) {
  RG_CHECK(g != nullptr, "rg_graph_export_time: graph is NULL");
  RG_CHECK(g->n_time > 0 && g->in_time && g->out_time, "rg_graph_export_time: the graph has no timestamps (build it with rg_tgraph_create)");
  if (out_time) RG_HIP(hipMemcpy(out_time, g->out_time, g->n_fact * sizeof(int32_t), hipMemcpyDeviceToHost));
  if (in_time) RG_HIP(hipMemcpy(in_time, g->in_time, g->n_fact * sizeof(int32_t), hipMemcpyDeviceToHost));
  return 0;
}

int rg_hipgraph_fill_nodes(void* graph) {
  size_t n = 0;
  if (hipGraphGetNodes((hipGraph_t)graph, nullptr, &n) != hipSuccess) { rg::set_error("rg_hipgraph_fill_nodes: hipGraphGetNodes failed"); return -1; }
  std::vector<hipGraphNode_t> nodes(n);
  if (n && hipGraphGetNodes((hipGraph_t)graph, nodes.data(), &n) != hipSuccess) { rg::set_error("rg_hipgraph_fill_nodes: hipGraphGetNodes failed"); return -1; }
  int count = 0;
  for (size_t i = 0; i < n; ++i) {
    hipGraphNodeType t;
    if (hipGraphNodeGetType(nodes[i], &t) != hipSuccess) { rg::set_error("rg_hipgraph_fill_nodes: hipGraphNodeGetType failed"); return -1; }
    if (t == hipGraphNodeTypeMemset) ++count;
  }
  return count;
}

int rg_graph_export_packs(const rg_graph* g, int32_t* n_packs, int32_t* n_vrows, int32_t* ent, int32_t* pack, int32_t* rows, int32_t* vrows) {
  RG_CHECK(g != nullptr, "rg_graph_export_packs: graph is NULL");
  if (n_packs) *n_packs = g->in_pk_packs.n;
  if (n_vrows) *n_vrows = g->in_vr.n;
  if (ent && g->in_pk_packs.n) RG_HIP(hipMemcpy(ent, g->in_pk_packs.ent, (size_t)g->in_pk_packs.n * RG_PACK * sizeof(int2), hipMemcpyDeviceToHost));
  if (pack && g->in_pk_packs.n) RG_HIP(hipMemcpy(pack, g->in_pk_packs.pack, (size_t)g->in_pk_packs.n * sizeof(int4), hipMemcpyDeviceToHost));
  if (rows && g->in_pk_packs.n) RG_HIP(hipMemcpy(rows, g->in_pk_packs.rows, (size_t)g->in_vr.n * sizeof(int2), hipMemcpyDeviceToHost));
  if (vrows) RG_HIP(hipMemcpy(vrows, g->in_vr.rows, (size_t)g->in_vr.n * sizeof(int4), hipMemcpyDeviceToHost));
  return 0;
}

}
```

red-gnn_amd/csrc/graph_device.hip:

```cpp
#include <hipcub/hipcub.hpp>

#include <algorithm>
#include <vector>

#include "common.h"

namespace {

struct Tmp {
  std::vector<void*> ptrs;
  char* block = nullptr;
  size_t block_bytes = 0, used = 0;
  explicit Tmp(size_t bytes) {
    if (hipMalloc((void**)&block, bytes) == hipSuccess) block_bytes = bytes; else block = nullptr;
  }
  template <typename T>
  T* get(size_t n) {
    const size_t bytes = rg::align_up(std::max<size_t>(n, 1) * sizeof(T), 256);
    if (used + bytes <= block_bytes) { T* p = (T*)(block + used); used += bytes; return p; }
    void* p = nullptr;
    if (hipMalloc(&p, bytes) != hipSuccess) return nullptr;
    ptrs.push_back(p);
    return (T*)p;
  }
  ~Tmp() {
    for (void* p : ptrs) (void)hipFree(p);
    if (block) (void)hipFree(block);
  }
};

__global__ void rows_kernel(const int32_t* __restrict__ trip, int64_t n, int add_inverse, int n_ent, int n_rel, int max_rel,
                            int32_t* __restrict__ H, int32_t* __restrict__ R, int32_t* __restrict__ T, int64_t n_fact, int32_t* __restrict__ err) {
  const int64_t i = (int64_t)blockIdx.x * blockDim.x + threadIdx.x;
  if (i >= n_fact) return;
  const int64_t n_dir = add_inverse ? 2 * n : n;
  if (i < n_dir) {
    const int64_t j = i < n ? i : i - n;
    const int32_t h = trip[3 * j], r = trip[3 * j + 1], t = trip[3 * j + 2];
    if (h < 0 || h >= n_ent || t < 0 || t >= n_ent || r < 0 || r >= max_rel) { atomicMax(err, 1 + (int32_t)std::min<int64_t>(j, 0x7ffffffe)); H[i] = R[i] = T[i] = 0; return; }
    if (i < n) { H[i] = h; R[i] = r; T[i] = t; }
    else { H[i] = t; R[i] = r + n_rel; T[i] = h; }
  } else {
    const int32_t e = (int32_t)(i - n_dir);
    H[i] = e; R[i] = 2 * n_rel; T[i] = e;
  }
}

__global__ void iota_kernel(uint32_t* __restrict__ v, int64_t n) {
  const int64_t i = (int64_t)blockIdx.x * blockDim.x + threadIdx.x;
  if (i < n) v[i] = (uint32_t)i;
}

template <int MODE>
__global__ void keys_kernel(const int32_t* __restrict__ H, const int32_t* __restrict__ R, const int32_t* __restrict__ T, int rel_bits,
                            uint64_t* __restrict__ keys, int64_t n) {
  const int64_t i = (int64_t)blockIdx.x * blockDim.x + threadIdx.x;
  if (i >= n) return;
  keys[i] = MODE == 0 ? (uint64_t)T[i] : (MODE == 1 ? (((uint64_t)H[i] << rel_bits) | (uint64_t)R[i]) : (uint64_t)R[i]);
}

__global__ void hist_kernel(const int32_t* __restrict__ key, int64_t n, uint32_t* __restrict__ cnt) {
  const int64_t i = (int64_t)blockIdx.x * blockDim.x + threadIdx.x;
  if (i < n) atomicAdd(&cnt[key[i]], 1u);
}

__global__ void gather_pairs_kernel(const uint32_t* __restrict__ perm, const int32_t* __restrict__ A, const int32_t* __restrict__ B,
                                    int2* __restrict__ out, uint32_t* __restrict__ pk, int pk_mode, int64_t n) {
  const int64_t q = (int64_t)blockIdx.x * blockDim.x + threadIdx.x;
  if (q >= n) return;
  const uint32_t i = perm[q];
  const int2 v = make_int2(A[i], B[i]);
  out[q] = v;
  if (pk) pk[q] = pk_mode == 0 ? (((uint32_t)v.y << 20) | (uint32_t)v.x)
                               : (((uint32_t)v.x << 20) | (uint32_t)v.y);
}

__global__ void vrow_count_kernel(const int32_t* __restrict__ ptr, int n_rows, uint32_t* __restrict__ n_seg, uint32_t* __restrict__ is_split,
                                  uint32_t* __restrict__ split_seg) {
  const int e = blockIdx.x * blockDim.x + threadIdx.x;
  if (e >= n_rows) return;
  const int len = ptr[e + 1] - ptr[e];
  const int cut = len > RG_VROW_MAX;
  const int k = cut ? (len + RG_VROW_MAX - 1) / RG_VROW_MAX : 1;
  n_seg[e] = k; is_split[e] = cut; split_seg[e] = cut ? k : 0;
}

__global__ void vrow_emit_kernel(const int32_t* __restrict__ ptr, int n_rows, const int32_t* __restrict__ row_off, const int32_t* __restrict__ split_off,
                                 const int32_t* __restrict__ slot_off, int4* __restrict__ rows, uint32_t* __restrict__ keys, int4* __restrict__ split) {
  const int e = blockIdx.x * blockDim.x + threadIdx.x;
  if (e >= n_rows) return;
  const int beg = ptr[e], len = ptr[e + 1] - ptr[e];
  if (len <= RG_VROW_MAX) {
    rows[row_off[e]] = make_int4(e, beg, len, -1);
    keys[row_off[e]] = (uint32_t)(RG_VROW_MAX - len);
  } else {
    const int k = (len + RG_VROW_MAX - 1) / RG_VROW_MAX;
    split[split_off[e]] = make_int4(e, slot_off[e], k, 0);
    for (int j = 0; j < k; ++j) {
      const int b = beg + j * RG_VROW_MAX, l = min(RG_VROW_MAX, beg + len - b);
      rows[row_off[e] + j] = make_int4(e, b, l, slot_off[e] + j);
      keys[row_off[e] + j] = (uint32_t)(RG_VROW_MAX - l);
    }
  }
}

__global__ void gather_rows_kernel(const uint32_t* __restrict__ perm, const int4* __restrict__ in, int4* __restrict__ out, int n) {
  const int i = blockIdx.x * blockDim.x + threadIdx.x;
  if (i < n) out[i] = in[perm[i]];
}

__global__ void pack_emit_kernel(const int4* __restrict__ vrows, const int4* __restrict__ place, int n_vrows, const int32_t* __restrict__ pack_row0,
                                 const uint32_t* __restrict__ in_pk, int2* __restrict__ ent, int4* __restrict__ pack, int2* __restrict__ rows) {
  const int i = blockIdx.x;
  if (i >= n_vrows) return;
  const int4 r = vrows[i];
  const int4 pl = place[i];
  if (pl.x < 0) return;
  for (int j = threadIdx.x; j < r.z; j += blockDim.x) ent[(int64_t)pl.x * RG_PACK + pl.y + j] = make_int2((int)in_pk[r.y + j], pl.z);
  if (threadIdx.x == 0) {
    rows[pack_row0[pl.x] + pl.z] = make_int2(r.x, r.w);
    if (pl.z == 0) pack[pl.x] = make_int4(pack_row0[pl.x], 0, r.w, r.x);
  }
}

__global__ void pack_count_kernel(const int32_t* __restrict__ pack_nrows, int4* __restrict__ pack, int n_packs) {
  const int p = blockIdx.x * blockDim.x + threadIdx.x;
  if (p < n_packs) pack[p].y = pack_nrows[p];
}

__global__ void fill_int2_kernel(int2* __restrict__ p, int64_t n, int2 v) {
  const int64_t i = (int64_t)blockIdx.x * blockDim.x + threadIdx.x;
  if (i < n) p[i] = v;
}

__global__ void max_kernel(const int32_t* __restrict__ ptr, int n_rows, int32_t* __restrict__ out) {
  const int e = blockIdx.x * blockDim.x + threadIdx.x;
  if (e < n_rows) atomicMax(out, ptr[e + 1] - ptr[e]);
}

#define DEV_HIP(expr)                                                                          \
  do {                                                                                         \
    hipError_t e_ = (expr);                                                                    \
    if (e_ != hipSuccess) {                                                                    \
      ::rg::set_error("rg_graph_create_device: %s failed: %s", #expr, hipGetErrorString(e_)); \
      return 1;                                                                                \
    }                                                                                          \
  } while (0)

inline unsigned blocks(int64_t n, int t = 256) { return (unsigned)std::max<int64_t>(rg::ceil_div(n, t), 1); }

static int sort_perm(Tmp& tmp, const uint64_t* keys, int bits, int64_t n, uint32_t* perm_out, hipStream_t s) {
  uint64_t* keys_out = tmp.get<uint64_t>(n);
  uint32_t* iota = tmp.get<uint32_t>(n);
  if (!keys_out || !iota) { rg::set_error("rg_graph_create_device: out of device memory"); return 1; }
  hipLaunchKernelGGL(iota_kernel, dim3(blocks(n)), dim3(256), 0, s, iota, n);
  size_t bytes = 0;
  DEV_HIP(hipcub::DeviceRadixSort::SortPairs(nullptr, bytes, keys, keys_out, iota, perm_out, (int)n, 0, bits, s));
  char* scratch = tmp.get<char>(bytes);
  if (!scratch) { rg::set_error("rg_graph_create_device: out of device memory"); return 1; }
  DEV_HIP(hipcub::DeviceRadixSort::SortPairs(scratch, bytes, keys, keys_out, iota, perm_out, (int)n, 0, bits, s));
  return 0;
}

static int build_ptr(Tmp& tmp, const int32_t* key, int64_t n, int n_rows, int32_t* ptr, hipStream_t s) {
  uint32_t* cnt = tmp.get<uint32_t>(n_rows + 1);
  int32_t* scr = tmp.get<int32_t>(rg::scan_scratch_elems(n_rows + 1));
  if (!cnt || !scr) { rg::set_error("rg_graph_create_device: out of device memory"); return 1; }
  DEV_HIP(hipMemsetAsync(cnt, 0, (size_t)(n_rows + 1) * 4, s));
  hipLaunchKernelGGL(hist_kernel, dim3(blocks(n)), dim3(256), 0, s, key, n, cnt);
  return rg::scan_exclusive(cnt, ptr, n_rows + 1, false, nullptr, scr, s);
}

struct VrowsDev { int4* rows = nullptr; int4* split = nullptr; int32_t* counts = nullptr; int cap_rows = 0, cap_split = 0; };

static int build_vrows(Tmp& tmp, const int32_t* ptr, int n_rows, int64_t n_fact, VrowsDev* out, hipStream_t s) {
  uint32_t* n_seg = tmp.get<uint32_t>(n_rows + 1);
  uint32_t* is_split = tmp.get<uint32_t>(n_rows + 1);
  uint32_t* split_seg = tmp.get<uint32_t>(n_rows + 1);
  int32_t* row_off = tmp.get<int32_t>(n_rows + 1);
  int32_t* split_off = tmp.get<int32_t>(n_rows + 1);
  int32_t* slot_off = tmp.get<int32_t>(n_rows + 1);
  int32_t* scr = tmp.get<int32_t>(rg::scan_scratch_elems(n_rows + 1));
  out->cap_rows = (int)(n_rows + n_fact / RG_VROW_MAX + 2);
  out->cap_split = (int)(n_fact / (RG_VROW_MAX + 1) + 2);
  int4* rows_u = tmp.get<int4>(out->cap_rows);
  uint32_t* keys = tmp.get<uint32_t>(out->cap_rows);
  uint32_t* keys_o = tmp.get<uint32_t>(out->cap_rows);
  uint32_t* iota = tmp.get<uint32_t>(out->cap_rows);
  uint32_t* perm = tmp.get<uint32_t>(out->cap_rows);
  out->rows = tmp.get<int4>(out->cap_rows);
  out->split = tmp.get<int4>(out->cap_split);
  out->counts = tmp.get<int32_t>(4);
  if (!n_seg || !is_split || !split_seg || !row_off || !split_off || !slot_off || !scr || !rows_u || !keys || !keys_o || !iota || !perm ||
      !out->rows || !out->split || !out->counts) { rg::set_error("rg_graph_create_device: out of device memory"); return 1; }
  hipLaunchKernelGGL(vrow_count_kernel, dim3(blocks(n_rows)), dim3(256), 0, s, ptr, n_rows, n_seg, is_split, split_seg);
  if (rg::scan_exclusive(n_seg, row_off, n_rows, false, &out->counts[0], scr, s)) return 1;
  if (rg::scan_exclusive(is_split, split_off, n_rows, false, &out->counts[1], scr, s)) return 1;
  if (rg::scan_exclusive(split_seg, slot_off, n_rows, false, &out->counts[2], scr, s)) return 1;
  hipLaunchKernelGGL(vrow_emit_kernel, dim3(blocks(n_rows)), dim3(256), 0, s, ptr, n_rows, row_off, split_off, slot_off, rows_u, keys, out->split);
  int32_t n_v = 0;
  DEV_HIP(hipMemcpyAsync(&n_v, &out->counts[0], 4, hipMemcpyDeviceToHost, s));
  DEV_HIP(hipStreamSynchronize(s));
  hipLaunchKernelGGL(iota_kernel, dim3(blocks(n_v)), dim3(256), 0, s, iota, (int64_t)n_v);
  size_t bytes = 0;
  DEV_HIP(hipcub::DeviceRadixSort::SortPairs(nullptr, bytes, keys, keys_o, iota, perm, n_v, 0, 8, s));
  char* scratch = tmp.get<char>(bytes);
  if (!scratch) { rg::set_error("rg_graph_create_device: out of device memory"); return 1; }
  DEV_HIP(hipcub::DeviceRadixSort::SortPairs(scratch, bytes, keys, keys_o, iota, perm, n_v, 0, 8, s));
  hipLaunchKernelGGL(gather_rows_kernel, dim3(blocks(n_v)), dim3(256), 0, s, perm, rows_u, out->rows, n_v);
  RG_LAUNCH_CHECK();
  return 0;
}

}

extern "C" int rg_graph_create_device(int32_t n_ent, int32_t n_rel, const int32_t* triples_dev, int64_t n, int add_inverse, void* stream,
                                      rg_graph** out) {
  RG_CHECK(out != nullptr, "rg_graph_create_device: out is NULL");
  *out = nullptr;
  RG_CHECK(n_ent > 0 && n_rel > 0, "rg_graph_create_device: n_ent=%d n_rel=%d must be positive", n_ent, n_rel);
  RG_CHECK(n >= 0 && (n == 0 || triples_dev != nullptr), "rg_graph_create_device: bad triples (n=%lld)", (long long)n);
  const int64_t n_fact = (add_inverse ? 2 * n : n) + n_ent;
  RG_CHECK(n_fact < (int64_t)1 << 31, "rg_graph_create_device: %lld fact rows do not fit int32", (long long)n_fact);
  hipStream_t s = (hipStream_t)stream;
  const int n_rela_rows = 2 * n_rel + 1;
  const int max_rel = add_inverse ? n_rel : 2 * n_rel;
  int rel_bits = 1, ent_bits = 1;
  while ((1 << rel_bits) < n_rela_rows) ++rel_bits;
  while (((int64_t)1 << ent_bits) < n_ent) ++ent_bits;
  Tmp tmp((size_t)n_fact * 160 + (size_t)n_ent * 96 + ((size_t)8 << 20));
  int32_t* H = tmp.get<int32_t>(n_fact); int32_t* R = tmp.get<int32_t>(n_fact); int32_t* T = tmp.get<int32_t>(n_fact);
  uint64_t* keys = tmp.get<uint64_t>(n_fact);
  uint32_t* perm_in = tmp.get<uint32_t>(n_fact); uint32_t* perm_out = tmp.get<uint32_t>(n_fact); uint32_t* perm_rel = tmp.get<uint32_t>(n_fact);
  int32_t* flags = tmp.get<int32_t>(16);
  int32_t* out_ptr = tmp.get<int32_t>(n_ent + 2); int32_t* in_ptr = tmp.get<int32_t>(n_ent + 2); int32_t* rel_ptr = tmp.get<int32_t>(n_rela_rows + 2);
  int2* out_rt = tmp.get<int2>(n_fact); int2* in_hr = tmp.get<int2>(n_fact); int2* rel_ht = tmp.get<int2>(n_fact);
  const bool packed = n_ent <= (1 << 20) && n_rela_rows <= (1 << 12);
  uint32_t* in_pk = packed ? tmp.get<uint32_t>(n_fact) : nullptr; uint32_t* out_pk = packed ? tmp.get<uint32_t>(n_fact) : nullptr;
  RG_CHECK(H && R && T && keys && perm_in && perm_out && perm_rel && flags && out_ptr && in_ptr && rel_ptr && out_rt && in_hr && rel_ht &&
           (!packed || (in_pk && out_pk)), "rg_graph_create_device: out of device memory");
  DEV_HIP(hipMemsetAsync(flags, 0, 64, s));
  hipLaunchKernelGGL(rows_kernel, dim3(blocks(n_fact)), dim3(256), 0, s, triples_dev, n, add_inverse, n_ent, n_rel, max_rel, H, R, T, n_fact, flags);
  hipLaunchKernelGGL(keys_kernel<0>, dim3(blocks(n_fact)), dim3(256), 0, s, H, R, T, rel_bits, keys, n_fact);
  if (sort_perm(tmp, keys, ent_bits, n_fact, perm_in, s)) return 1;
  hipLaunchKernelGGL(keys_kernel<1>, dim3(blocks(n_fact)), dim3(256), 0, s, H, R, T, rel_bits, keys, n_fact);
  if (sort_perm(tmp, keys, ent_bits + rel_bits, n_fact, perm_out, s)) return 1;
  hipLaunchKernelGGL(keys_kernel<2>, dim3(blocks(n_fact)), dim3(256), 0, s, H, R, T, rel_bits, keys, n_fact);
  if (sort_perm(tmp, keys, rel_bits, n_fact, perm_rel, s)) return 1;
  hipLaunchKernelGGL(gather_pairs_kernel, dim3(blocks(n_fact)), dim3(256), 0, s, perm_in, H, R, in_hr, in_pk, 0, n_fact);
  hipLaunchKernelGGL(gather_pairs_kernel, dim3(blocks(n_fact)), dim3(256), 0, s, perm_out, R, T, out_rt, out_pk, 1, n_fact);
  hipLaunchKernelGGL(gather_pairs_kernel, dim3(blocks(n_fact)), dim3(256), 0, s, perm_rel, H, T, rel_ht, (uint32_t*)nullptr, 0, n_fact);
  if (build_ptr(tmp, T, n_fact, n_ent, in_ptr, s) || build_ptr(tmp, H, n_fact, n_ent, out_ptr, s) || build_ptr(tmp, R, n_fact, n_rela_rows, rel_ptr, s)) return 1;
  hipLaunchKernelGGL(max_kernel, dim3(blocks(n_ent)), dim3(256), 0, s, in_ptr, n_ent, &flags[1]);
  hipLaunchKernelGGL(max_kernel, dim3(blocks(n_ent)), dim3(256), 0, s, out_ptr, n_ent, &flags[2]);
  VrowsDev vin, vout, vrel;
  if (build_vrows(tmp, in_ptr, n_ent, n_fact, &vin, s) || build_vrows(tmp, out_ptr, n_ent, n_fact, &vout, s) ||
      build_vrows(tmp, rel_ptr, n_rela_rows, n_fact, &vrel, s)) return 1;
  int32_t host[16];
  DEV_HIP(hipMemcpyAsync(host, vin.counts, 12, hipMemcpyDeviceToHost, s));
  DEV_HIP(hipMemcpyAsync(host + 4, vout.counts, 12, hipMemcpyDeviceToHost, s));
  DEV_HIP(hipMemcpyAsync(host + 8, vrel.counts, 12, hipMemcpyDeviceToHost, s));
  DEV_HIP(hipMemcpyAsync(host + 12, flags, 16, hipMemcpyDeviceToHost, s));
  DEV_HIP(hipStreamSynchronize(s));
  RG_CHECK(host[12] == 0, "rg_graph_create_device: triple %d out of range", host[12] - 1);
  const bool want_packs = packed && n_rela_rows < (1 << 12);
  int4* place = nullptr; int32_t* pack_nrows = nullptr; int32_t* pack_row0 = nullptr;
  int n_packs = 0;
  if (want_packs) {
    const int nv = host[0];
    place = tmp.get<int4>(nv);
    pack_nrows = tmp.get<int32_t>(nv + 1);
    pack_row0 = tmp.get<int32_t>(nv + 1);
    int32_t* scr = tmp.get<int32_t>(rg::scan_scratch_elems(nv + 1));
    RG_CHECK(place && pack_nrows && pack_row0 && scr, "rg_graph_create_device: out of device memory");
    std::vector<int4> vrows_h(nv), place_h;
    std::vector<int32_t> nrows_h;
    DEV_HIP(hipMemcpyAsync(vrows_h.data(), vin.rows, (size_t)nv * sizeof(int4), hipMemcpyDeviceToHost, s));
    DEV_HIP(hipStreamSynchronize(s));
    n_packs = rg::place_rows_best_fit(vrows_h.data(), nv, &place_h, &nrows_h);
    DEV_HIP(hipMemcpyAsync(place, place_h.data(), (size_t)nv * sizeof(int4), hipMemcpyHostToDevice, s));
    if (n_packs) DEV_HIP(hipMemcpyAsync(pack_nrows, nrows_h.data(), (size_t)n_packs * sizeof(int32_t), hipMemcpyHostToDevice, s));
    DEV_HIP(hipStreamSynchronize(s));
    if (rg::scan_exclusive((const uint32_t*)pack_nrows, pack_row0, n_packs, false, nullptr, scr, s)) return 1;
  }
  rg_graph* g = new rg_graph();
  g->n_ent = n_ent; g->n_rel = n_rel; g->n_rela_rows = n_rela_rows; g->n_time = 0; g->n_fact = n_fact;
  g->max_in_deg = host[13]; g->max_out_deg = host[14];
  g->in_vr.n = host[0]; g->in_vr.n_split = host[1]; g->in_vr.n_slots = host[2];
  g->out_vr.n = host[4]; g->out_vr.n_split = host[5]; g->out_vr.n_slots = host[6];
  g->rel_vr.n = host[8]; g->rel_vr.n_split = host[9]; g->rel_vr.n_slots = host[10];
  g->in_pk_packs.n = n_packs;
  struct Item { void** field; const void* src; size_t bytes, off; };
  std::vector<Item> items;
  size_t total = 0;
  auto add = [&](void** field, const void* src, size_t bytes) {
    items.push_back({field, src, bytes, total});
    total += rg::align_up(std::max<size_t>(bytes, 16), 256);
  };
  add((void**)&g->out_ptr, out_ptr, (size_t)(n_ent + 1) * 4); add((void**)&g->in_ptr, in_ptr, (size_t)(n_ent + 1) * 4);
  add((void**)&g->out_rt, out_rt, (size_t)n_fact * 8); add((void**)&g->in_hr, in_hr, (size_t)n_fact * 8);
  if (packed) { add((void**)&g->in_pk, in_pk, (size_t)n_fact * 4); add((void**)&g->out_pk, out_pk, (size_t)n_fact * 4); }
  add((void**)&g->rel_ptr, rel_ptr, (size_t)(n_rela_rows + 1) * 4); add((void**)&g->rel_ht, rel_ht, (size_t)n_fact * 8);
  add((void**)&g->in_vr.rows, vin.rows, (size_t)g->in_vr.n * 16); add((void**)&g->in_vr.split, vin.split, (size_t)g->in_vr.n_split * 16);
  add((void**)&g->out_vr.rows, vout.rows, (size_t)g->out_vr.n * 16); add((void**)&g->out_vr.split, vout.split, (size_t)g->out_vr.n_split * 16);
  add((void**)&g->rel_vr.rows, vrel.rows, (size_t)g->rel_vr.n * 16); add((void**)&g->rel_vr.split, vrel.split, (size_t)g->rel_vr.n_split * 16);
  const size_t ent_off = total;
  if (n_packs > 0) {
    add((void**)&g->in_pk_packs.ent, nullptr, (size_t)n_packs * RG_PACK * 8);
    add((void**)&g->in_pk_packs.pack, nullptr, (size_t)n_packs * 16);
    add((void**)&g->in_pk_packs.rows, nullptr, (size_t)g->in_vr.n * 8);
  }
  hipError_t e = hipMalloc(&g->arena, total);
  if (e != hipSuccess) {
    rg::set_error("rg_graph_create_device: allocating %zu B failed: %s", total, hipGetErrorString(e));
    delete g;
    return 1;
  }
  for (const Item& it : items) {
    *it.field = (char*)g->arena + it.off;
    if (it.src && it.bytes) (void)hipMemcpyAsync(*it.field, it.src, it.bytes, hipMemcpyDeviceToDevice, s);
  }
  (void)ent_off;
  if (n_packs > 0) {
    hipLaunchKernelGGL(fill_int2_kernel, dim3(blocks((int64_t)n_packs * RG_PACK)), dim3(256), 0, s, g->in_pk_packs.ent, (int64_t)n_packs * RG_PACK,
                       make_int2(-1, 0));
    hipLaunchKernelGGL(pack_emit_kernel, dim3(g->in_vr.n), dim3(64), 0, s, g->in_vr.rows, place, g->in_vr.n, pack_row0, g->in_pk, g->in_pk_packs.ent,
                       g->in_pk_packs.pack, g->in_pk_packs.rows);
    hipLaunchKernelGGL(pack_count_kernel, dim3(blocks(n_packs)), dim3(256), 0, s, pack_nrows, g->in_pk_packs.pack, n_packs);
  }
  e = hipStreamSynchronize(s);
  if (e == hipSuccess) e = hipGetLastError();
  if (e != hipSuccess) {
    rg::set_error("rg_graph_create_device: build failed: %s", hipGetErrorString(e));
    rg_graph_destroy(g);
    return 1;
  }
  *out = g;
  return 0;
}
```

red-gnn_amd/csrc/layer_fwd.hip:

```cpp
#include "layer_fwd_kernel.h"
#include "layer_fwd_wp.h"

extern "C" size_t rg_layer_fwd_scratch_bytes(const rg_frontier* f, const rg_graph* g, int32_t ld) {
  if (!f || !g) return 0;
  return rg::align_up((size_t)f->B * g->in_vr.n_slots * ld * sizeof(float), 256) + rg::align_up((size_t)f->B * g->in_vr.n_slots, 256) + 256;
}

static int plan_walk(const rg_frontier* f, const rg_graph* g, int32_t level, int64_t n_old, int64_t n_new, int64_t n_edges, int32_t ld) {
  if (g->in_pk_packs.n == 0 || level != f->level || n_old < 0 || n_new <= 0 || n_edges < 0 || !rgwp::offsets_fit(n_old, ld)) return 1;
  const double candidates = (double)n_new * (double)g->n_fact / (double)g->n_ent;
  const bool tiny = n_new * 16 < (int64_t)f->B * f->n_ent;
  const bool short_rows = (double)g->n_fact < 12.0 * (double)g->n_ent;
  if (!tiny && !short_rows && (double)n_edges >= 0.4 * candidates) return 1;
  const double group_bytes = (double)n_old * ld * sizeof(float) / f->BW;
  int code = group_bytes <= 3.0 * (1 << 20) ? 2 : (group_bytes <= 6.0 * (1 << 20) ? 3 : 4);
  auto items = [&](int c) { return (int64_t)f->BW * (1 << (c - 2)) * g->in_pk_packs.n; };
  while (code < 5 && items(code) < 16384 && n_edges > 256 * items(code)) ++code;
  return code;
}

extern "C" int rg_layer_fwd_plan(const rg_frontier* f, const rg_graph* g, int32_t level, int64_t n_old, int64_t n_new,
                                 int64_t n_edges, int32_t ld) {
  if (!f || !g) return 1;
  return plan_walk(f, g, level, n_old, n_new, n_edges, ld);
}

extern "C" int rg_layer_fwd(const rg_frontier* f, const rg_graph* g, int32_t level, int64_t n_new, const float* hidden,
                            const float* rela, int32_t d, int32_t ld, const float* a_s, const float* a_r,
                            const float* a_q, int32_t ap, const float* w_alpha, const float* b_alpha, int32_t attn_dim,
                            float* agg_out, void* scratch, size_t scratch_bytes, int32_t walk, void* stream) {
  RG_CHECK(f && g && hidden && rela && a_s && a_r && a_q && w_alpha && b_alpha && agg_out, "rg_layer_fwd: NULL argument");
  RG_CHECK((((uintptr_t)hidden | (uintptr_t)rela | (uintptr_t)a_s | (uintptr_t)a_r | (uintptr_t)a_q | (uintptr_t)agg_out |
             (uintptr_t)scratch) & 15) == 0, "rg_layer_fwd: float buffers must be 16-B aligned");
  RG_CHECK(walk >= 0 && walk <= 7, "rg_layer_fwd: walk=%d not in 0..7", walk);
  rgfwd::FwdArgs A;
  if (rgfwd::fill_common("rg_layer_fwd", f, g, level, n_new, d, ld, ap, attn_dim, scratch, scratch_bytes,
                         rg_layer_fwd_scratch_bytes(f, g, ld), &A)) return 1;
  if (n_new == 0) return 0;
  A.hidden = (const float4*)hidden; A.rela = (const float4*)rela;
  A.a_s = (const float4*)a_s; A.a_r = (const float4*)a_r; A.a_q = (const float4*)a_q;
  A.w_alpha = w_alpha; A.b_alpha = b_alpha;
  A.agg = (float4*)agg_out; A.partial = (float4*)scratch;
  hipStream_t s = (hipStream_t)stream;
  if (walk == 0)
    walk = plan_walk(f, g, level, f->n_nodes[(level - 1) % f->n_levels], f->n_nodes[level % f->n_levels],
                     level == f->level ? f->n_edges : -1, ld);
  if (walk >= 2 && f->n_nodes[(level - 1) % f->n_levels] < 0 && !rgwp::offsets_fit((int64_t)f->B * f->n_ent, ld))
    walk = 1;
  if (walk >= 2) {
    RG_CHECK(g->in_pk_packs.n > 0, "rg_layer_fwd: the word-parallel walk needs a static graph with packed entries");
    RG_CHECK(level == f->level, "rg_layer_fwd: the word-parallel walk reads the entity-major bitmaps of the newest hop only "
             "(level %d, newest %d)", level, f->level);
    const int64_t n_old = f->n_nodes[(level - 1) % f->n_levels] >= 0 ? f->n_nodes[(level - 1) % f->n_levels] : (int64_t)f->B * f->n_ent;
    RG_CHECK(rgwp::offsets_fit(n_old, ld), "rg_layer_fwd: the word-parallel walk addresses the previous level by 32-bit byte offsets "
             "(%lld rows x %d floats is 4 GiB or more)", (long long)n_old, ld);
    rgwp::WpArgs W;
    W.n_sub = 1 << (walk - 2);
    W.n_packs = g->in_pk_packs.n; W.BW = f->BW; W.W = f->W; W.n_slots = g->in_vr.n_slots;
    W.n_items = (int64_t)f->BW * W.n_sub * W.n_packs;
    W.ent = g->in_pk_packs.ent; W.pack = g->in_pk_packs.pack; W.rows = g->in_pk_packs.rows;
    W.bits_old = f->bitsT[f->tcur ^ 1]; W.bits_new = f->bitsT[f->tcur];
    W.bm_old = A.bm_old; W.bm_new = A.bm_new;
    W.hidden = A.hidden; W.rela = A.rela; W.ld4 = A.ld4; W.a_s = A.a_s; W.a_r = A.a_r; W.a_q = A.a_q;
    W.w_alpha = w_alpha; W.b_alpha = b_alpha; W.attn_dim = attn_dim; W.n_rela_rows = g->n_rela_rows;
    W.agg = A.agg; W.partial = A.partial; W.queues = f->queues; W.queues_clean = A.walk.queues_clean;
    const int64_t n_e = level == f->level ? (f->n_edges >= 0 ? f->n_edges : f->edge_hint) : -1;
    const int64_t by_work = n_e < 0 ? 2 : 200 * W.n_items / std::max<int64_t>(n_e, 1);
    W.ipt = (int32_t)std::max<int64_t>(std::min<int64_t>(std::min<int64_t>(by_work, W.n_items / 8192), 32), 1);
    const size_t n_part = (size_t)f->B * g->in_vr.n_slots;
    W.written = n_part ? (uint8_t*)scratch + rg::align_up(n_part * ld * sizeof(float), 256) : nullptr;
    if (n_part && rg::zero_async(W.written, rg::align_up(n_part, 256), s)) return 1;
    if (rgwp::launch(W, ap / 4, s)) return 1;
    return rgfwd::launch_combine(A, f->B, g->in_vr, s, W.written);
  }
  const bool dense = n_new * 4 >= (int64_t)f->B * f->n_ent;
  return rgfwd::dispatch<false>(A, ld / 4, ap / 4, f->B, g->in_vr, dense, rg::walk_kpg(g->n_fact, g->in_vr.n), s);
}
```

red-gnn_amd/csrc/layer_fwd_wp.h:

```cpp
#pragma once
#include "common.h"

namespace rgwp {

struct WpArgs {
  int64_t n_items;
  int32_t n_packs, n_sub, BW, W, n_slots;
  const int2* ent;
  const int4* pack;
  const int2* rows;
  const uint32_t* bits_old;
  const uint32_t* bits_new;
  const int2* bm_old;
  const int2* bm_new;
  const float4* hidden;
  const float4* rela;
  int ld4;
  const float4* a_s;
  const float4* a_r;
  const float4* a_q;
  const float* w_alpha;
  const float* b_alpha;
  int attn_dim, n_rela_rows;
  float4* agg;
  float4* partial;
  uint8_t* written;
  int32_t* queues;
  int32_t ipt;
  bool queues_clean;
};

int launch(const WpArgs& A, int ap4, hipStream_t s);
bool offsets_fit(int64_t n_old, int32_t ld);

}
```

red-gnn_amd/csrc/layer_fwd_wp.hip:

```cpp
#include "attn.h"
#include "layer_fwd_wp.h"

namespace rgwp {
namespace {

constexpr int WP_BLOCK = 512, WP_WAVES = WP_BLOCK / 64;
constexpr int QCAP = 256;
constexpr int WAVE_LDS = QCAP * 16 + 64;
static_assert(QCAP == 256 && RG_PACK == 128, "a lane holds two entries of a pack; phase 1 takes four queued edges per lane");

__device__ __forceinline__ uint32_t wave_or(uint32_t v) {
#pragma unroll
  for (int o = 32; o > 0; o >>= 1) v |= (uint32_t)__shfl_xor((int)v, o, 64);
  return (uint32_t)__builtin_amdgcn_readfirstlane((int)v);
}

template <int G, int F, int AP4, bool RELA_LDS, bool EXACT>
__global__ __launch_bounds__(WP_BLOCK, 4) void layer_fwd_wp_kernel(WpArgs A) {
  extern __shared__ float4 lds[];
  constexpr int GW = 64 / G, RW = G * F + 1;
  char* wave_lds = reinterpret_cast<char*>(lds);
  float4* ar_l = reinterpret_cast<float4*>(wave_lds + WP_WAVES * WAVE_LDS);
  float4* w_l = ar_l + A.n_rela_rows * AP4;
  float4* rela_l = w_l + AP4;

  rg::stage_attention<AP4, WP_BLOCK>(ar_l, w_l, A.a_r, A.n_rela_rows, A.w_alpha, A.attn_dim);
  if constexpr (RELA_LDS) {
    for (int i = threadIdx.x; i < A.n_rela_rows * RW; i += WP_BLOCK) {
      const int r = i / RW, c = i - r * RW;
      rela_l[i] = c < A.ld4 ? A.rela[(int64_t)r * A.ld4 + c] : rg::f4zero();
    }
  }
  __syncthreads();
  const float b_alpha = A.b_alpha[0];

  const int lane = threadIdx.x & 63, wv = threadIdx.x >> 6;
  const int lane_g = lane & (G - 1), gi_w = lane / G;
  const unsigned long long lt = (1ull << lane) - 1ull;
  float4* st = reinterpret_cast<float4*>(wave_lds + wv * WAVE_LDS);
  int2* q8 = reinterpret_cast<int2*>(st) + QCAP;
  unsigned long long* hmask = reinterpret_cast<unsigned long long*>(st + QCAP);
  const int qbits = 32 / A.n_sub;
  const uint32_t row_bytes = (uint32_t)A.ld4 * 16u;
  const uint32_t lane_off = (uint32_t)lane_g * 16u;
  uint32_t col_d[F];
  bool col_ok[F];
#pragma unroll
  for (int f = 0; f < F; ++f) {
    const int c = lane_g + G * f;
    col_ok[f] = EXACT || c < A.ld4;
    col_d[f] = EXACT ? (uint32_t)(f * G * 16) : (uint32_t)((col_ok[f] ? c : A.ld4 - 1) - lane_g) * 16u;
  }
  const char* hidden_b = reinterpret_cast<const char*>(A.hidden);
  const char* rela_b = reinterpret_cast<const char*>(A.rela);
  const char* rela_lb = reinterpret_cast<const char*>(rela_l) + lane_g * 16;

  auto store_row = [&](int out, const float4 (&acc)[F]) {
    float4* row = out >= 0 ? A.agg + (int64_t)out * A.ld4 : A.partial + (int64_t)(-out - 1) * A.ld4;
#pragma unroll
    for (int f = 0; f < F; ++f)
      if (col_ok[f]) row[lane_g + G * f] = acc[f];
    if (out < 0 && lane_g == 0) A.written[-out - 1] = 1;
  };
  auto gather = [&](const float4& t, float4 (&hv)[F]) {
    const uint32_t off = (uint32_t)__float_as_int(t.x) + lane_off;
#pragma unroll
    for (int f = 0; f < F; ++f) {
      if constexpr (EXACT) hv[f] = *reinterpret_cast<const float4*>(hidden_b + off + f * (G * 16));
      else hv[f] = *reinterpret_cast<const float4*>(hidden_b + (off + col_d[f]));
    }
  };
  auto consume = [&](const float4& t, const float4 (&hv)[F], float4 (&acc)[F]) {
    const float al = t.z;
    const uint32_t ro = (uint32_t)__float_as_int(t.y);
#pragma unroll
    for (int f = 0; f < F; ++f) {
      float4 rv;
      if constexpr (RELA_LDS) rv = *reinterpret_cast<const float4*>(rela_lb + ro + f * (G * 16));
      else if constexpr (EXACT) rv = *reinterpret_cast<const float4*>(rela_b + (ro + lane_off) + f * (G * 16));
      else rv = *reinterpret_cast<const float4*>(rela_b + (ro + lane_off + col_d[f]));
      acc[f].x = fmaf(al, hv[f].x + rv.x, acc[f].x);
      acc[f].y = fmaf(al, hv[f].y + rv.y, acc[f].y);
      acc[f].z = fmaf(al, hv[f].z + rv.z, acc[f].z);
      acc[f].w = fmaf(al, hv[f].w + rv.w, acc[f].w);
    }
  };

  auto run_item = [&](long long item) {
    const int grp = (int)(item / A.n_packs);
    const int pi = __builtin_amdgcn_readfirstlane((int)(item - (long long)grp * A.n_packs));
    const int bw = __builtin_amdgcn_readfirstlane(grp / A.n_sub), sub = grp - bw * A.n_sub;
    const uint32_t qmask = A.n_sub == 1 ? 0xFFFFFFFFu : (((1u << qbits) - 1u) << (sub * qbits));
    const int2 e0 = A.ent[(int64_t)pi * RG_PACK + lane], e1 = A.ent[(int64_t)pi * RG_PACK + 64 + lane];
    uint32_t w0 = 0, w1 = 0;
    if (e0.x != -1) w0 = A.bits_old[(int64_t)(e0.x & 0xFFFFF) * A.BW + bw] & qmask;
    if (e1.x != -1) w1 = A.bits_old[(int64_t)(e1.x & 0xFFFFF) * A.BW + bw] & qmask;
    const int row0 = A.pack[pi].x;
    uint32_t todo = wave_or(w0 | w1);
    while (todo) {
      int qn = 0;
      while (todo) {
        const int b = __ffs((int)todo) - 1;
        const bool v0 = (w0 >> b) & 1u, v1 = (w1 >> b) & 1u;
        const unsigned long long m0 = __ballot(v0), m1 = __ballot(v1);
        const int c0 = __popcll(m0), c1 = __popcll(m1);
        if (qn + c0 + c1 > QCAP) break;
        if (v0) q8[qn + __popcll(m0 & lt)] = make_int2(e0.x, (b << 8) | e0.y);
        if (v1) q8[qn + c0 + __popcll(m1 & lt)] = make_int2(e1.x, (b << 8) | e1.y);
        qn += c0 + c1;
        todo &= todo - 1;
      }
      __builtin_amdgcn_fence(__ATOMIC_ACQ_REL, "wavefront");
      __builtin_amdgcn_wave_barrier();
      {
        int2 en[4];
        int s[4], out[4];
        bool valid[4];
#pragma unroll
        for (int j = 0; j < 4; ++j) {
          const int i = j * 64 + lane;
          valid[j] = i < qn;
          en[j] = valid[j] ? q8[i] : make_int2(0, -1);
          const int prev_key = (valid[j] && i > 0) ? q8[i - 1].y : -2;
          const unsigned long long hm = __ballot(valid[j] && en[j].y != prev_key);
          if (lane == 0) hmask[j] = hm;
        }
        int2 wp[4], dst[4];
#pragma unroll
        for (int j = 0; j < 4; ++j) {
          wp[j] = make_int2(0, 0); dst[j] = make_int2(0, 0);
          if (valid[j]) {
            const int hd = en[j].x & 0xFFFFF, bq = bw * 32 + (en[j].y >> 8);
            wp[j] = A.bm_old[(int64_t)bq * A.W + (hd >> 5)];
            dst[j] = A.rows[row0 + (en[j].y & 255)];
          }
        }
#pragma unroll
        for (int j = 0; j < 4; ++j) {
          s[j] = 0; out[j] = 0;
          if (valid[j]) {
            const int hd = en[j].x & 0xFFFFF, bq = bw * 32 + (en[j].y >> 8);
            s[j] = rg::bm_rank(wp[j], hd);
            if (dst[j].y < 0) {
              const int2 wn = A.bm_new[(int64_t)bq * A.W + (dst[j].x >> 5)];
              out[j] = rg::bm_rank(wn, dst[j].x);
            } else {
              out[j] = -(bq * A.n_slots + dst[j].y) - 1;
            }
          }
        }
#pragma unroll
        for (int j = 0; j < 4; ++j) {
          if (valid[j]) {
            const int r = (uint32_t)en[j].x >> 20;
            const float4* aq_p = A.a_q + (int64_t)(bw * 32 + (en[j].y >> 8)) * AP4;
            float z = b_alpha;
#pragma unroll
            for (int k = 0; k < AP4; ++k) {
              const float4 as = A.a_s[(int64_t)s[j] * AP4 + k];
              const float4 ar = ar_l[r * AP4 + k];
              const float4 w = w_l[k];
              rg::attn_acc_fwd(z, w, as, ar, aq_p[k]);
            }
            const float alpha = rg::attn_alpha(z);
            const uint32_t hoff = (uint32_t)s[j] * row_bytes;
            const uint32_t roff = (uint32_t)r * (RELA_LDS ? (uint32_t)(RW * 16) : row_bytes);
            st[j * 64 + lane] = make_float4(__int_as_float((int)hoff), __int_as_float((int)roff), alpha, __int_as_float(out[j]));
          }
        }
      }
      __builtin_amdgcn_fence(__ATOMIC_ACQ_REL, "wavefront");
      __builtin_amdgcn_wave_barrier();
      auto next_head = [&](int c) -> int {
        int pos = qn;
#pragma unroll
        for (int w = 3; w >= 0; --w) {
          unsigned long long m = hmask[w];
          if (w == (c >> 6)) m &= ~0ull << (c & 63);
          else if (w < (c >> 6)) m = 0ull;
          if (m) pos = w * 64 + __ffsll((long long)m) - 1;
        }
        return pos;
      };
      int e = 0, end = qn;
      if constexpr (GW > 1) {
        e = gi_w == 0 ? 0 : next_head(gi_w * qn / GW);
        end = gi_w == GW - 1 ? qn : next_head((gi_w + 1) * qn / GW);
      }
      if (e < end) {
        float4 acc[F], hvA[F], hvB[F];
#pragma unroll
        for (int f = 0; f < F; ++f) acc[f] = rg::f4zero();
        float4 tA = st[e], tB;
        int cur = __float_as_int(tA.w);
        gather(tA, hvA);
        for (;;) {
          tB = st[min(e + 1, end - 1)];
          gather(tB, hvB);
          consume(tA, hvA, acc);
          if (e + 1 >= end || __float_as_int(tB.w) != cur) {
            store_row(cur, acc);
#pragma unroll
            for (int f = 0; f < F; ++f) acc[f] = rg::f4zero();
            cur = __float_as_int(tB.w);
          }
          if (e + 1 >= end) break;
          tA = st[min(e + 2, end - 1)];
          gather(tA, hvA);
          consume(tB, hvB, acc);
          if (e + 2 >= end || __float_as_int(tA.w) != cur) {
            store_row(cur, acc);
#pragma unroll
            for (int f = 0; f < F; ++f) acc[f] = rg::f4zero();
            cur = __float_as_int(tA.w);
          }
          if (e + 2 >= end) break;
          e += 2;
        }
      }
      __builtin_amdgcn_fence(__ATOMIC_ACQ_REL, "wavefront");
      __builtin_amdgcn_wave_barrier();
    }
  };

  int q = __builtin_amdgcn_s_getreg((3 << 11) | 20) & 7;
  auto ticket = [&]() -> int {
    int off = 0;
    if (lane == 0) off = atomicAdd(&A.queues[q * RG_QSTRIDE], A.ipt);
    return off;
  };
  auto resolve = [&](int off, long long* first) -> int {
    off = __builtin_amdgcn_readfirstlane(off);
    for (;;) {
      const long long qs = A.n_items * q / 8, ql = A.n_items * (q + 1) / 8 - qs;
      if (off < ql) {
        *first = qs + off;
        return (int)min((long long)A.ipt, ql - off);
      }
      const int k = (q + 1 + lane) & 7;
      bool has = false;
      if (lane < 7) has = __hip_atomic_load(&A.queues[k * RG_QSTRIDE], __ATOMIC_RELAXED, __HIP_MEMORY_SCOPE_AGENT) < A.n_items * (k + 1) / 8 - A.n_items * k / 8;
      const unsigned long long m = __ballot(has);
      if (m == 0ull) return 0;
      q = (q + 1 + (__ffsll((long long)m) - 1)) & 7;
      off = __builtin_amdgcn_readfirstlane(ticket());
    }
  };
  int off = ticket();
  for (;;) {
    long long first = 0;
    const int cnt = resolve(off, &first);
    if (cnt == 0) break;
    off = ticket();
    for (int k = 0; k < cnt; ++k) run_item(first + k);
  }
}

template <int G, int F, int AP4, bool RELA_LDS, bool EXACT>
int launch4(const WpArgs& A, size_t lds, hipStream_t s) {
  auto kern = layer_fwd_wp_kernel<G, F, AP4, RELA_LDS, EXACT>;
  if (lds > 64 * 1024) RG_HIP(hipFuncSetAttribute((const void*)kern, hipFuncAttributeMaxDynamicSharedMemorySize, (int)lds));
  const int per_cu = lds <= 80 * 1024 ? 2 : 1;
  const int grid = (int)std::max<int64_t>(std::min<int64_t>(rg::ceil_div(A.n_items, WP_WAVES * A.ipt), 256 * per_cu), 1);
  if (!A.queues_clean && rg::zero_async(A.queues, RG_QUEUE_BYTES, s)) return 1;
  hipLaunchKernelGGL(kern, dim3(grid), dim3(WP_BLOCK), lds, s, A);
  RG_LAUNCH_CHECK();
  return 0;
}

template <int G, int F, int AP4, bool RELA_LDS>
int launch3(const WpArgs& A, size_t lds, hipStream_t s) {
  if constexpr (G * F >= 16) {
    if (A.ld4 == G * F) return launch4<G, F, AP4, RELA_LDS, true>(A, lds, s);
  }
  return launch4<G, F, AP4, RELA_LDS, false>(A, lds, s);
}

template <int G, int F, int AP4>
int launch2(const WpArgs& A, hipStream_t s) {
  const size_t lds = (size_t)WP_WAVES * WAVE_LDS + (size_t)(A.n_rela_rows * AP4 + AP4) * sizeof(float4);
  const size_t rela_bytes = (size_t)A.n_rela_rows * (G * F + 1) * sizeof(float4);
  RG_CHECK(lds <= 160 * 1024, "rg_layer_fwd: attention tables need %zu B of LDS (> 160 KiB)", lds);
  if (lds + rela_bytes <= 80 * 1024) return launch3<G, F, AP4, true>(A, lds + rela_bytes, s);
  return launch3<G, F, AP4, false>(A, lds, s);
}

}

bool offsets_fit(int64_t n_old, int32_t ld) { return n_old >= 0 && (uint64_t)n_old * ld * sizeof(float) < ((uint64_t)1 << 32); }

int launch(const WpArgs& A, int ap4, hipStream_t s) {
  RG_CHECK(A.n_items / 8 + ((int64_t)1 << 26) < ((int64_t)1 << 31), "rg_layer_fwd: work space too large for 32-bit queue tickets");
  return rg::with_g(A.ld4, [&](auto g) {
    return rg::with_ap4(ap4, "rg_layer_fwd", [&](auto ap) { return launch2<decltype(g)::value / 2, 2, decltype(ap)::value>(A, s); });
  });
}

}
```

red-gnn_amd/engine.py:

```python
import ctypes as C

import numpy as np
import torch

from . import _lib


FORCE_WALK = 0

KERNEL_EVENTS = None
DENSE_EVENTS = None
BWD_EVENTS = None
EXPLAIN_EVENTS = None
PROFILE_EVENTS = None


def _require_gpu(device):
    device = torch.device(device)
    if device.type != "cuda":
        raise _lib.NativeError("red_gnn_amd runs on an MI355X (device 'cuda'); got device %r. "
                               "There is no CPU path in the product — the CPU restatement lives in oracle/ for tests only."
                               % (device,))
    if not torch.cuda.is_available():
        raise _lib.NativeError("red_gnn_amd needs an MI355X: no ROCm device is visible to this process. The HIP path has "
                               "no CPU fallback (the CPU restatement in oracle/ is test infrastructure only).")
    return device


_GRAPH_SERIAL = [0]


def _next_serial():
    _GRAPH_SERIAL[0] += 1
    return _GRAPH_SERIAL[0]


class Graph:

    def __init__(self, n_ent, n_rel, triples, add_inverse=True, device="cuda"):
        self.serial = _next_serial()
        self.device = _require_gpu(device)
        trip = np.ascontiguousarray(np.asarray(triples, dtype=np.int32).reshape(-1, 3))
        self.n_ent, self.n_rel = int(n_ent), int(n_rel)
        h = C.c_void_p()
        with torch.cuda.device(self.device):
            _lib.check(_lib.lib().rg_graph_create(self.n_ent, self.n_rel, _lib.ptr(trip), len(trip),
                                                  1 if add_inverse else 0, C.byref(h)))
        self.handle = h
        self.n_fact = int(_lib.lib().rg_graph_n_fact(h))

    @classmethod
    def from_device(cls, n_ent, n_rel, triples_dev, add_inverse=True):
        self = cls.__new__(cls)
        self.serial = _next_serial()
        self.device = _require_gpu(triples_dev.device)
        assert triples_dev.dtype == torch.int32 and triples_dev.dim() == 2 and triples_dev.shape[1] == 3
        trip = triples_dev.contiguous()
        self.n_ent, self.n_rel = int(n_ent), int(n_rel)
        h = C.c_void_p()
        with torch.cuda.device(self.device):
            _lib.check(_lib.lib().rg_graph_create_device(self.n_ent, self.n_rel, _lib.ptr(trip), trip.shape[0], 1 if add_inverse else 0,
                                                         _lib.stream_ptr(), C.byref(h)))
        self.handle = h
        self.n_fact = int(_lib.lib().rg_graph_n_fact(h))
        return self

    def export_packs(self):
        L = _lib.lib()
        n_packs, n_vrows = C.c_int32(), C.c_int32()
        _lib.check(L.rg_graph_export_packs(self.handle, C.byref(n_packs), C.byref(n_vrows), None, None, None, None))
        vr = np.empty((n_vrows.value, 4), np.int32)
        ent = np.empty((n_packs.value * 128, 2), np.int32)
        pack = np.empty((n_packs.value, 4), np.int32)
        rows = np.empty((n_vrows.value if n_packs.value else 0, 2), np.int32)
        _lib.check(L.rg_graph_export_packs(self.handle, None, None, _lib.ptr(ent), _lib.ptr(pack), _lib.ptr(rows), _lib.ptr(vr)))
        return vr, ent, pack, rows

    def export(self):
        op = np.empty(self.n_ent + 1, np.int32)
        ip = np.empty(self.n_ent + 1, np.int32)
        ort = np.empty((self.n_fact, 2), np.int32)
        ihr = np.empty((self.n_fact, 2), np.int32)
        _lib.check(_lib.lib().rg_graph_export(self.handle, _lib.ptr(op), _lib.ptr(ort), _lib.ptr(ip), _lib.ptr(ihr)))
        return op, ort, ip, ihr

    def close(self):
        if getattr(self, "handle", None) is not None and _lib._lib is not None:
            _lib.lib().rg_graph_destroy(self.handle)
        self.handle = None

    def __del__(self):
        try:
            self.close()
        except Exception:
            pass


class TemporalGraph(Graph):

    def __init__(self, n_ent, n_rela_rows, n_time, quads, device="cuda", exclude=None):
        self.serial = _next_serial()
        self.device = _require_gpu(device)
        q = quads if (isinstance(quads, np.ndarray) and quads.dtype == np.int32 and quads.flags.c_contiguous and quads.ndim == 2) \
            else np.ascontiguousarray(np.asarray(quads, dtype=np.int32).reshape(-1, 4))
        self.n_ent, self.n_rel, self.n_rela_rows, self.n_time = int(n_ent), 0, int(n_rela_rows), int(n_time)
        h = C.c_void_p()
        with torch.cuda.device(self.device):
            if exclude is None:
                _lib.check(_lib.lib().rg_tgraph_create(self.n_ent, self.n_rela_rows, self.n_time, _lib.ptr(q), len(q), C.byref(h)))
            else:
                ex = np.ascontiguousarray(np.asarray(exclude, dtype=np.int64).reshape(-1))
                _lib.check(_lib.lib().rg_tgraph_create_excluding(self.n_ent, self.n_rela_rows, self.n_time, _lib.ptr(q), len(q),
                                                                 _lib.ptr(ex), len(ex), C.byref(h)))
        self.handle = h
        self.n_fact = int(_lib.lib().rg_graph_n_fact(h))


    def export_time(self):
        ot = np.empty(self.n_fact, np.int32)
        it = np.empty(self.n_fact, np.int32)
        _lib.check(_lib.lib().rg_graph_export_time(self.handle, _lib.ptr(ot), _lib.ptr(it)))
        return ot, it


class Frontier:

    def __init__(self, n_ent, batch, n_levels=2, device="cuda"):
        self.device = _require_gpu(device)
        L = _lib.lib()
        self.n_ent, self.batch, self.n_levels = int(n_ent), int(batch), int(n_levels)
        nbytes = L.rg_frontier_workspace_bytes(self.n_ent, self.batch, self.n_levels)
        if nbytes == 0:
            raise _lib.NativeError("bad frontier shape n_ent=%d batch=%d n_levels=%d" % (n_ent, batch, n_levels))
        self.workspace = torch.empty(nbytes + 256, dtype=torch.uint8, device=self.device)
        base = self.workspace.data_ptr()
        aligned = (base + 255) // 256 * 256
        h = C.c_void_p()
        _lib.check(L.rg_frontier_create(self.n_ent, self.batch, self.n_levels, C.c_void_p(aligned), nbytes, C.byref(h)))
        self.handle = h
        self._counts = (C.c_int64 * 4)()
        self.level = -1
        self.n_new = self.n_old = self.n_edges = 0
        self.generation = 0
        self.leases = 0

    def reset(self, q_sub):
        assert q_sub.dtype == torch.int32 and q_sub.is_cuda and q_sub.numel() == self.batch
        _lib.check(_lib.lib().rg_frontier_reset(self.handle, _lib.ptr(q_sub), _lib.stream_ptr()))
        self.level, self.n_new, self.n_old, self.n_edges = 0, self.batch, 0, 0
        self.generation += 1

    def reset_nodes(self, nodes):
        assert nodes.dtype == torch.int32 and nodes.is_cuda and nodes.dim() == 2 and nodes.shape[1] == 2
        nodes = nodes.contiguous()
        _lib.check(_lib.lib().rg_frontier_reset_nodes(self.handle, _lib.ptr(nodes), nodes.shape[0], _lib.stream_ptr()))
        self.level, self.n_new, self.n_old, self.n_edges = 0, nodes.shape[0], 0, 0
        self.generation += 1

    def set_window(self, win_lo, win_hi, n_data):
        if win_lo is None:
            self._window = None
            _lib.check(_lib.lib().rg_frontier_set_window(self.handle, None, None, 0))
            return
        assert win_lo.dtype == torch.int32 and win_hi.dtype == torch.int32 and win_lo.is_cuda and win_lo.numel() == self.batch == win_hi.numel()
        self._window = (win_lo.contiguous(), win_hi.contiguous())
        _lib.check(_lib.lib().rg_frontier_set_window(self.handle, _lib.ptr(self._window[0]), _lib.ptr(self._window[1]), int(n_data)))

    def expand(self, graph):
        _lib.check(_lib.lib().rg_frontier_expand(self.handle, graph.handle, self._counts, _lib.stream_ptr()))
        self.n_new, self.n_edges, self.n_old, self.level = (int(self._counts[i]) for i in range(4))
        return self.n_new, self.n_edges, self.n_old

    def expand_async(self, graph):
        _lib.check(_lib.lib().rg_frontier_expand_async(self.handle, graph.handle, _lib.stream_ptr()))
        self.level += 1
        self.n_new = self.n_old = self.n_edges = -1

    def expand_nodes_async(self, graph, nodes, prev, edge_hint=None):
        _lib.check(_lib.lib().rg_frontier_expand_nodes_async(self.handle, graph.handle, _lib.ptr(nodes), _lib.ptr(prev), _lib.stream_ptr()))
        if edge_hint is not None and edge_hint >= 0:
            _lib.check(_lib.lib().rg_frontier_set_edge_hint(self.handle, int(edge_hint)))
        self.level += 1
        self.n_new = self.n_old = self.n_edges = -1

    def count_ptr(self):
        return C.c_void_p(_lib.lib().rg_frontier_count_ptr(self.handle))

    def level_counts(self):
        buf = (C.c_int64 * 32)()
        _lib.check(_lib.lib().rg_frontier_level_counts(self.handle, buf, _lib.stream_ptr()))
        return [(int(buf[2 * l]), int(buf[2 * l + 1])) for l in range(self.level + 1)]

    def nodes_into(self, nodes, prev):
        _lib.check(_lib.lib().rg_frontier_nodes(self.handle, _lib.ptr(nodes), _lib.ptr(prev), None, _lib.stream_ptr()))

    def nodes(self, want_prev=True, want_old_new=True):
        nodes = torch.empty((self.n_new, 2), dtype=torch.int32, device=self.device)
        prev = torch.empty(self.n_new, dtype=torch.int32, device=self.device) if want_prev else None
        old_new = (torch.empty(self.n_old, dtype=torch.int32, device=self.device)
                   if (want_old_new and self.level > 0) else None)
        _lib.check(_lib.lib().rg_frontier_nodes(self.handle, _lib.ptr(nodes), _lib.ptr(prev), _lib.ptr(old_new),
                                                _lib.stream_ptr()))
        return nodes, prev, old_new

    def edges(self, graph, nodes_new, level=None):
        level = self.level if level is None else level
        n_new = nodes_new.shape[0]
        L = _lib.lib()
        scratch = torch.empty(L.rg_frontier_edges_scratch_bytes(n_new), dtype=torch.uint8, device=self.device)
        row_ptr = torch.empty(n_new + 1, dtype=torch.int32, device=self.device)
        _lib.check(L.rg_frontier_edges(self.handle, graph.handle, level, _lib.ptr(nodes_new), n_new, None,
                                       _lib.ptr(row_ptr), _lib.ptr(scratch), _lib.stream_ptr()))
        n_e = int(row_ptr[-1].item())
        edges = torch.empty((n_e, 6), dtype=torch.int32, device=self.device)
        _lib.check(L.rg_frontier_edges(self.handle, graph.handle, level, _lib.ptr(nodes_new), n_new, _lib.ptr(edges),
                                       _lib.ptr(row_ptr), _lib.ptr(scratch), _lib.stream_ptr()))
        return edges, row_ptr

    def scratch(self, nbytes):
        buf = getattr(self, "_scratch", None)
        if buf is None or buf.numel() < nbytes:
            buf = self._scratch = torch.empty(max(nbytes, 256), dtype=torch.uint8, device=self.device)
        return buf

    def close(self):
        if getattr(self, "handle", None) is not None and _lib._lib is not None:
            _lib.lib().rg_frontier_destroy(self.handle)
        self.handle = None

    def __del__(self):
        try:
            self.close()
        except Exception:
            pass


class FrontierLease:
    __slots__ = ("frontier", "generation", "released")

    def __init__(self, frontier):
        self.frontier, self.generation, self.released = frontier, frontier.generation, False
        frontier.leases += 1

    def release(self):
        if not self.released:
            self.released = True
            self.frontier.leases -= 1

    def check(self):
        if self.frontier.generation != self.generation:
            raise RuntimeError("red_gnn_amd: the frontier of this autograd graph was reset by a later forward (generation %d, now %d); "
                               "its level bitmaps are gone, the backward cannot run" % (self.generation, self.frontier.generation))

    def __del__(self):
        self.release()


class FrontierPool:

    def __init__(self, max_keys=64):
        self.max_keys, self.pool = max_keys, {}

    def get(self, n_ent, batch, n_levels, device):
        key = (n_ent, batch, n_levels, str(device), torch.cuda.current_stream(device).cuda_stream)
        frs = self.pool.get(key)
        if frs is None:
            if len(self.pool) >= self.max_keys:
                self.pool = {k: [f for f in v if f.leases > 0] for k, v in self.pool.items()}
                self.pool = {k: v for k, v in self.pool.items() if v}
            frs = self.pool[key] = []
        for fr in frs:
            if fr.leases == 0:
                return fr
        fr = Frontier(n_ent, batch, n_levels, device)
        frs.append(fr)
        return fr

    def clear(self):
        self.pool = {}


def layer_fwd(frontier, graph, level, nodes_new, hidden, rela, d, a_s, a_r, a_q, w_alpha, b_alpha, attn_dim):
    ld, ap = hidden.shape[1], a_s.shape[1]
    for t in (hidden, rela, a_s, a_r, a_q, w_alpha, b_alpha):
        assert t.is_cuda and t.dtype == torch.float32 and t.is_contiguous()
    assert rela.shape[1] == ld and a_r.shape[1] == ap and a_q.shape[1] == ap
    n_new = nodes_new.shape[0]
    agg = torch.empty((n_new, ld), dtype=torch.float32, device=hidden.device)
    nbytes = _lib.lib().rg_layer_fwd_scratch_bytes(frontier.handle, graph.handle, ld)
    scratch = frontier.scratch(nbytes)
    ev = None
    if KERNEL_EVENTS is not None:
        ev = (torch.cuda.Event(enable_timing=True), torch.cuda.Event(enable_timing=True))
        ev[0].record()
    _lib.check(_lib.lib().rg_layer_fwd(frontier.handle, graph.handle, level, n_new,
                                       _lib.ptr(hidden), _lib.ptr(rela), d, ld, _lib.ptr(a_s), _lib.ptr(a_r),
                                       _lib.ptr(a_q), ap, _lib.ptr(w_alpha), _lib.ptr(b_alpha), attn_dim,
                                       _lib.ptr(agg), _lib.ptr(scratch), nbytes, FORCE_WALK, _lib.stream_ptr()))
    if ev is not None:
        ev[1].record()
        KERNEL_EVENTS.append((ev[0], ev[1], frontier.n_edges, n_new))
    return agg


def explain_seed(frontier, level, objs):
    assert objs.dtype == torch.int32 and objs.is_cuda and objs.numel() == frontier.batch
    W = (frontier.n_ent + 31) // 32
    marks = torch.empty((frontier.batch, W), dtype=torch.int32, device=frontier.device)
    reached = torch.empty(frontier.batch, dtype=torch.bool, device=frontier.device)
    _lib.check(_lib.lib().rg_explain_seed(frontier.handle, frontier.batch, frontier.n_ent, level, _lib.ptr(objs.contiguous()),
                                          _lib.ptr(marks), _lib.ptr(reached), _lib.stream_ptr()))
    return marks, reached


def explain_hop(frontier, graph, level, marks, a_s, a_r, a_q, w_alpha, b_alpha, attn_dim, min_alpha):
    for t in (a_s, a_r, a_q, w_alpha, b_alpha):
        assert t.is_cuda and t.dtype == torch.float32 and t.is_contiguous()
    ap = a_s.shape[1]
    assert a_r.shape[1] == ap and a_q.shape[1] == ap
    L, dev = _lib.lib(), frontier.device
    marks_prev = torch.empty_like(marks)
    word_ptr = torch.empty(marks.numel() + 1, dtype=torch.int32, device=dev)
    scratch = frontier.scratch(L.rg_explain_scratch_bytes(frontier.handle) + 256)
    base = scratch.data_ptr()
    aligned = (base + 255) // 256 * 256
    n_e = C.c_int64()
    args = (frontier.handle, graph.handle, frontier.batch, frontier.n_ent, level, _lib.ptr(marks), _lib.ptr(a_s), _lib.ptr(a_r),
            _lib.ptr(a_q), ap, _lib.ptr(w_alpha), _lib.ptr(b_alpha), attn_dim, float(min_alpha))
    ev = None
    if EXPLAIN_EVENTS is not None:
        ev = (torch.cuda.Event(enable_timing=True), torch.cuda.Event(enable_timing=True))
        ev[0].record()
    _lib.check(L.rg_explain_count(*args, _lib.ptr(marks_prev), _lib.ptr(word_ptr), C.c_void_p(aligned),
                                  scratch.numel() - (aligned - base), C.byref(n_e), _lib.stream_ptr()))
    edges = torch.empty((n_e.value, 4), dtype=torch.int32, device=dev)
    alpha = torch.empty(n_e.value, dtype=torch.float32, device=dev)
    if n_e.value:
        _lib.check(L.rg_explain_emit(*args, _lib.ptr(word_ptr), _lib.ptr(edges), _lib.ptr(alpha), _lib.stream_ptr()))
    if ev is not None:
        ev[1].record()
        EXPLAIN_EVENTS.append((ev[0], ev[1], level, n_e.value))
    return marks_prev, edges, alpha


def texplain_hop(frontier, graph, level, marks, a_s, a_r, a_q, w_alpha, b_alpha, attn_dim, min_alpha):
    for t in (a_s, a_r, a_q, w_alpha, b_alpha):
        assert t.is_cuda and t.dtype == torch.float32 and t.is_contiguous()
    ap = a_s.shape[1]
    assert a_r.shape == (graph.n_rela_rows, ap) and a_q.shape == (frontier.batch, ap)
    L, dev = _lib.lib(), frontier.device
    marks_prev = torch.empty_like(marks)
    word_ptr = torch.empty(marks.numel() + 1, dtype=torch.int32, device=dev)
    scratch = frontier.scratch(L.rg_explain_scratch_bytes(frontier.handle) + 256)
    base = scratch.data_ptr()
    aligned = (base + 255) // 256 * 256
    n_e = C.c_int64()
    args = (frontier.handle, graph.handle, frontier.batch, frontier.n_ent, level, _lib.ptr(marks), _lib.ptr(a_s), _lib.ptr(a_r),
            _lib.ptr(a_q), ap, _lib.ptr(w_alpha), _lib.ptr(b_alpha), attn_dim, float(min_alpha))
    ev = None
    if EXPLAIN_EVENTS is not None:
        ev = (torch.cuda.Event(enable_timing=True), torch.cuda.Event(enable_timing=True))
        ev[0].record()
    _lib.check(L.rg_texplain_count(*args, _lib.ptr(marks_prev), _lib.ptr(word_ptr), C.c_void_p(aligned),
                                   scratch.numel() - (aligned - base), C.byref(n_e), _lib.stream_ptr()))
    edges = torch.empty((n_e.value, 4), dtype=torch.int32, device=dev)
    alpha = torch.empty(n_e.value, dtype=torch.float32, device=dev)
    time = torch.empty(n_e.value, dtype=torch.int32, device=dev)
    if n_e.value:
        _lib.check(L.rg_texplain_emit(*args, _lib.ptr(word_ptr), _lib.ptr(edges), _lib.ptr(alpha), _lib.ptr(time), _lib.stream_ptr()))
    if ev is not None:
        ev[1].record()
        EXPLAIN_EVENTS.append((ev[0], ev[1], level, n_e.value))
    return marks_prev, edges, alpha, time


def explain_gather(hop, batch, edges, alpha, row_first, row_base, edges_out, alpha_out):
    assert edges.dtype == torch.int32 and edges.is_contiguous() and edges_out.is_contiguous() and alpha_out.is_contiguous()
    assert row_first.dtype == torch.int64 and row_base.dtype == torch.int64
    _lib.check(_lib.lib().rg_explain_gather(edges.shape[0], hop, batch, _lib.ptr(edges), _lib.ptr(alpha.contiguous()),
                                            _lib.ptr(row_first.contiguous()), _lib.ptr(row_base.contiguous()), edges_out.shape[0],
                                            _lib.ptr(edges_out), _lib.ptr(alpha_out), _lib.stream_ptr()))


def attn_profile(frontier, graph, level, a_s, a_r, a_q, w_alpha, b_alpha, attn_dim, sum_out, count_out):
    for t in (a_s, a_r, a_q, w_alpha, b_alpha):
        assert t.is_cuda and t.dtype == torch.float32 and t.is_contiguous()
    ap = a_s.shape[1]
    assert a_r.shape == (2 * graph.n_rel + 1, ap) and a_q.shape == (frontier.batch, ap)
    for t in (sum_out, count_out):
        assert t.is_cuda and t.dtype == torch.int64 and t.is_contiguous() and t.shape == (frontier.batch, a_r.shape[0])
    ev = None
    if PROFILE_EVENTS is not None:
        ev = (torch.cuda.Event(enable_timing=True), torch.cuda.Event(enable_timing=True))
        ev[0].record()
    _lib.check(_lib.lib().rg_attn_profile(frontier.handle, graph.handle, frontier.batch, frontier.n_ent, level, a_s.shape[0],
                                          _lib.ptr(a_s), _lib.ptr(a_r), _lib.ptr(a_q), ap, _lib.ptr(w_alpha), _lib.ptr(b_alpha),
                                          attn_dim, _lib.ptr(sum_out), _lib.ptr(count_out), _lib.stream_ptr()))
    if ev is not None:
        ev[1].record()
        PROFILE_EVENTS.append((ev[0], ev[1], level))


def tattn_profile(frontier, graph, level, q_time, a_s, a_r, a_q, w_alpha, b_alpha, attn_dim, sum_out, count_out):
    for t in (a_s, a_r, a_q, w_alpha, b_alpha):
        assert t.is_cuda and t.dtype == torch.float32 and t.is_contiguous()
    ap = a_s.shape[1]
    assert a_r.shape == (graph.n_rela_rows, ap) and a_q.shape == (frontier.batch, ap)
    assert q_time.is_cuda and q_time.dtype == torch.int32 and q_time.is_contiguous() and q_time.numel() == frontier.batch
    for t in (sum_out, count_out):
        assert t.is_cuda and t.dtype == torch.int64 and t.is_contiguous() and t.shape == (frontier.batch, 3, a_r.shape[0])
    ev = None
    if PROFILE_EVENTS is not None:
        ev = (torch.cuda.Event(enable_timing=True), torch.cuda.Event(enable_timing=True))
        ev[0].record()
    _lib.check(_lib.lib().rg_tattn_profile(frontier.handle, graph.handle, frontier.batch, frontier.n_ent, level, a_s.shape[0],
                                           _lib.ptr(q_time), _lib.ptr(a_s), _lib.ptr(a_r), _lib.ptr(a_q), ap, _lib.ptr(w_alpha),
                                           _lib.ptr(b_alpha), attn_dim, _lib.ptr(sum_out), _lib.ptr(count_out), _lib.stream_ptr()))
    if ev is not None:
        ev[1].record()
        PROFILE_EVENTS.append((ev[0], ev[1], level))


def layer_fwd_plan(frontier, graph, level, n_old, n_new, n_edges, ld):
    return int(_lib.lib().rg_layer_fwd_plan(frontier.handle, graph.handle, level, n_old, n_new, n_edges, ld))


def layer_fwd_scratch_bytes(frontier, graph, ld):
    return _lib.lib().rg_layer_fwd_scratch_bytes(frontier.handle, graph.handle, ld)


def layer_fwd_into(frontier, graph, level, n_hint, hidden, rela, d, a_s, a_r, a_q, w_alpha, b_alpha, attn_dim, agg, scratch, walk=1):
    ld, ap = hidden.shape[1], a_s.shape[1]
    _lib.check(_lib.lib().rg_layer_fwd(frontier.handle, graph.handle, level, max(int(n_hint), 1),
                                       _lib.ptr(hidden), _lib.ptr(rela), d, ld, _lib.ptr(a_s), _lib.ptr(a_r),
                                       _lib.ptr(a_q), ap, _lib.ptr(w_alpha), _lib.ptr(b_alpha), attn_dim,
                                       _lib.ptr(agg), _lib.ptr(scratch), scratch.numel(), FORCE_WALK or max(int(walk), 1), _lib.stream_ptr()))


def tlayer_fwd(frontier, graph, level, n_new, q_time, hidden_dir, rela_dir, time_dir, d, a_s, a_r, a_q, w_alpha, b_alpha, attn_dim):
    ld, ap = hidden_dir.shape[1], a_s.shape[1]
    for t in (hidden_dir, rela_dir, time_dir, a_s, a_r, a_q, w_alpha, b_alpha):
        assert t.is_cuda and t.dtype == torch.float32 and t.is_contiguous()
    assert q_time.dtype == torch.int32 and q_time.is_cuda
    agg = torch.empty((n_new, ld), dtype=torch.float32, device=hidden_dir.device)
    nbytes = _lib.lib().rg_layer_fwd_scratch_bytes(frontier.handle, graph.handle, ld)
    scratch = frontier.scratch(nbytes)
    ev = None
    if KERNEL_EVENTS is not None:
        ev = (torch.cuda.Event(enable_timing=True), torch.cuda.Event(enable_timing=True))
        ev[0].record()
    _lib.check(_lib.lib().rg_tlayer_fwd(frontier.handle, graph.handle, level, n_new, _lib.ptr(q_time), _lib.ptr(hidden_dir),
                                        _lib.ptr(rela_dir), _lib.ptr(time_dir), d, ld, _lib.ptr(a_s), _lib.ptr(a_r), _lib.ptr(a_q),
                                        ap, _lib.ptr(w_alpha), _lib.ptr(b_alpha), attn_dim, _lib.ptr(agg), _lib.ptr(scratch),
                                        nbytes, _lib.stream_ptr()))
    if ev is not None:
        ev[1].record()
        KERNEL_EVENTS.append((ev[0], ev[1], frontier.n_edges, n_new))
    return agg


def xlayer_fwd(frontier, graph, level, n_new, q_time, loop_time, row_time, n_data, hidden_p, rela_p, time_p, d, a_s, a_r, a_q, w_alpha, b_alpha, attn_dim):
    ld, ap = hidden_p.shape[1], a_s.shape[1]
    for t in (hidden_p, rela_p, time_p, a_s, a_r, a_q, w_alpha, b_alpha):
        assert t.is_cuda and t.dtype == torch.float32 and t.is_contiguous()
    for t in (q_time, loop_time, row_time):
        assert t.dtype == torch.int32 and t.is_cuda and t.is_contiguous()
    agg = torch.empty((n_new, ld), dtype=torch.float32, device=hidden_p.device)
    nbytes = _lib.lib().rg_layer_fwd_scratch_bytes(frontier.handle, graph.handle, ld)
    scratch = frontier.scratch(nbytes)
    ev = None
    if KERNEL_EVENTS is not None:
        ev = (torch.cuda.Event(enable_timing=True), torch.cuda.Event(enable_timing=True))
        ev[0].record()
    _lib.check(_lib.lib().rg_xlayer_fwd(frontier.handle, graph.handle, level, n_new, _lib.ptr(q_time), _lib.ptr(loop_time), _lib.ptr(row_time),
                                        int(n_data), _lib.ptr(hidden_p), _lib.ptr(rela_p), _lib.ptr(time_p), time_p.shape[0], d, ld,
                                        _lib.ptr(a_s), _lib.ptr(a_r), _lib.ptr(a_q), ap, _lib.ptr(w_alpha), _lib.ptr(b_alpha), attn_dim,
                                        _lib.ptr(agg), _lib.ptr(scratch), nbytes, _lib.stream_ptr()))
    if ev is not None:
        ev[1].record()
        KERNEL_EVENTS.append((ev[0], ev[1], frontier.n_edges, n_new))
    return agg


def layer_bwd(frontier, graph, level, nodes_old, hidden, rela, d, a_s, a_r, a_q, w_alpha, b_alpha, attn_dim, grad_agg):
    ld, ap = hidden.shape[1], a_s.shape[1]
    grad_agg = grad_agg.contiguous()
    n_old = nodes_old.shape[0]
    dev = hidden.device
    g_h = torch.empty_like(hidden)
    g_as = torch.empty_like(a_s)
    g_rela = torch.zeros_like(rela)
    g_ar = torch.zeros_like(a_r)
    g_aq = torch.empty_like(a_q)
    g_w = torch.zeros(attn_dim, dtype=torch.float32, device=dev)
    g_b = torch.zeros(1, dtype=torch.float32, device=dev)
    nbytes = _lib.lib().rg_layer_bwd_scratch_bytes(frontier.handle, graph.handle, ld, ap)
    scratch = frontier.scratch(nbytes)
    ev = None
    if BWD_EVENTS is not None:
        ev = (torch.cuda.Event(enable_timing=True), torch.cuda.Event(enable_timing=True))
        ev[0].record()
    _lib.check(_lib.lib().rg_layer_bwd(frontier.handle, graph.handle, level, n_old,
                                       _lib.ptr(hidden), _lib.ptr(rela), d, ld, _lib.ptr(a_s), _lib.ptr(a_r),
                                       _lib.ptr(a_q), ap, _lib.ptr(w_alpha), _lib.ptr(b_alpha), attn_dim,
                                       _lib.ptr(grad_agg), _lib.ptr(g_h), _lib.ptr(g_rela), _lib.ptr(g_as),
                                       _lib.ptr(g_ar), _lib.ptr(g_aq), _lib.ptr(g_w), _lib.ptr(g_b), _lib.ptr(scratch), nbytes,
                                       _lib.stream_ptr()))
    if ev is not None:
        ev[1].record()
        BWD_EVENTS.append((ev[0], ev[1], level, n_old))
    return g_h, g_rela, g_as, g_ar, g_aq, g_w, g_b


def tlayer_bwd(frontier, graph, level, n_old, q_time, hidden_dir, rela_dir, time_dir, d, a_s, a_r, a_q, w_alpha, b_alpha, attn_dim,
               grad_agg):
    ld, ap = hidden_dir.shape[1], a_s.shape[1]
    grad_agg = grad_agg.contiguous()
    dev = hidden_dir.device
    g_hd = torch.empty_like(hidden_dir)
    g_as = torch.empty_like(a_s)
    g_rd = torch.zeros_like(rela_dir)
    g_td = torch.zeros_like(time_dir)
    g_ar = torch.zeros_like(a_r)
    g_aq = torch.empty_like(a_q)
    g_w = torch.zeros(attn_dim, dtype=torch.float32, device=dev)
    nbytes = _lib.lib().rg_tlayer_bwd_scratch_bytes(frontier.handle, graph.handle, ld, ap)
    scratch = frontier.scratch(nbytes)
    _lib.check(_lib.lib().rg_tlayer_bwd(frontier.handle, graph.handle, level, n_old, _lib.ptr(q_time), _lib.ptr(hidden_dir),
                                        _lib.ptr(rela_dir), _lib.ptr(time_dir), d, ld, _lib.ptr(a_s), _lib.ptr(a_r), _lib.ptr(a_q),
                                        ap, _lib.ptr(w_alpha), _lib.ptr(b_alpha), attn_dim, _lib.ptr(grad_agg), _lib.ptr(g_hd),
                                        _lib.ptr(g_rd), _lib.ptr(g_td), _lib.ptr(g_as), _lib.ptr(g_ar), _lib.ptr(g_aq), _lib.ptr(g_w),
                                        _lib.ptr(scratch), nbytes, _lib.stream_ptr()))
    return g_hd, g_rd, g_td, g_as, g_ar, g_aq, g_w


def xlayer_bwd(frontier, graph, level, n_old, q_time, loop_time, row_time, n_data, hidden_p, rela_p, time_p, d, a_s, a_r, a_q, w_alpha,
               b_alpha, attn_dim, grad_agg):
    ld, ap = hidden_p.shape[1], a_s.shape[1]
    grad_agg = grad_agg.contiguous()
    dev = hidden_p.device
    g_hp = torch.empty_like(hidden_p)
    g_as = torch.empty_like(a_s)
    g_rp = torch.zeros_like(rela_p)
    g_tp = torch.zeros_like(time_p)
    g_ar = torch.zeros_like(a_r)
    g_aq = torch.empty_like(a_q)
    g_w = torch.zeros(attn_dim, dtype=torch.float32, device=dev)
    nbytes = _lib.lib().rg_tlayer_bwd_scratch_bytes(frontier.handle, graph.handle, ld, ap)
    scratch = frontier.scratch(nbytes)
    _lib.check(_lib.lib().rg_xlayer_bwd(frontier.handle, graph.handle, level, n_old, _lib.ptr(q_time), _lib.ptr(loop_time), _lib.ptr(row_time),
                                        int(n_data), _lib.ptr(hidden_p), _lib.ptr(rela_p), _lib.ptr(time_p), time_p.shape[0], d, ld,
                                        _lib.ptr(a_s), _lib.ptr(a_r), _lib.ptr(a_q), ap, _lib.ptr(w_alpha), _lib.ptr(b_alpha), attn_dim,
                                        _lib.ptr(grad_agg), _lib.ptr(g_hp), _lib.ptr(g_rp), _lib.ptr(g_tp), _lib.ptr(g_as), _lib.ptr(g_ar),
                                        _lib.ptr(g_aq), _lib.ptr(g_w), _lib.ptr(scratch), nbytes, _lib.stream_ptr()))
    return g_hp, g_rp, g_tp, g_as, g_ar, g_aq, g_w


_GRAM_SCRATCH = {}


def gram_tn(g, x, colsum=False):
    assert g.is_cuda and x.is_cuda and g.dtype == torch.float32 and x.dtype == torch.float32 and g.shape[0] == x.shape[0]
    assert g.stride(1) == 1 and x.stride(1) == 1
    n_rows, m, n = g.shape[0], g.shape[1], x.shape[1]
    L = _lib.lib()
    out = torch.empty((m, n), dtype=torch.float32, device=g.device)
    cs = torch.empty(m, dtype=torch.float32, device=g.device) if colsum else None
    for m0 in range(0, m, 192):
        mc = min(192, m - m0)
        for n0 in range(0, n, 64):
            nc = min(64, n - n0)
            nbytes = L.rg_gram_tn_scratch_bytes(mc, nc)
            key = (str(g.device), torch.cuda.current_stream(g.device).cuda_stream)
            scratch = _GRAM_SCRATCH.get(key)
            if scratch is None or scratch.numel() < nbytes:
                scratch = _GRAM_SCRATCH[key] = torch.empty(nbytes, dtype=torch.uint8, device=g.device)
            tile = out if (mc == m and nc == n) else torch.empty((mc, nc), dtype=torch.float32, device=g.device)
            cs_t = None
            if colsum and n0 == 0:
                cs_t = cs if mc == m else torch.empty(mc, dtype=torch.float32, device=g.device)
            gv, xv = g[:, m0:m0 + mc], x[:, n0:n0 + nc]
            _lib.check(L.rg_gram_tn(C.c_void_p(gv.data_ptr()), g.stride(0), mc, C.c_void_p(xv.data_ptr()), x.stride(0), nc, n_rows,
                                    _lib.ptr(tile), _lib.ptr(cs_t), _lib.ptr(scratch), scratch.numel(), _lib.stream_ptr()))
            if tile is not out:
                out[m0:m0 + mc, n0:n0 + nc] = tile
            if cs_t is not None and cs_t is not cs:
                cs[m0:m0 + mc] = cs_t
    return (out, cs) if colsum else out


_BLAS_CHOICE = [None]


def prefer_blas(n_rows):
    choice = "cublas" if n_rows < (1 << 17) else "cublaslt"
    if _BLAS_CHOICE[0] != choice:
        import warnings
        with warnings.catch_warnings():
            warnings.simplefilter("ignore")
            torch.backends.cuda.preferred_blas_library(choice)
        _BLAS_CHOICE[0] = choice


def dense_supported(d, attn_dim):
    return bool(_lib.lib().rg_dense_fwd_supported(d, attn_dim))


DENSE_PRECISIONS = {"f32": 0, "f16x2": 1, "f16x3": 2}


def dense_scratch(d, precision, device):
    nbytes = int(_lib.lib().rg_dense_scratch_bytes(d, DENSE_PRECISIONS[precision]))
    return torch.empty(nbytes, dtype=torch.uint8, device=device) if nbytes else None


def dense_fwd(agg, hidden_prev, prev_idx, d, W_h, act, gate, Ws_next=None, attn_dim=0, ap=0, W_final=None, nodes=None,
              n_ent=0, scores_all=None, precision="f32"):
    n, ld = agg.shape
    hidden = torch.empty_like(agg)
    a_s = torch.empty((n, ap), dtype=torch.float32, device=agg.device) if Ws_next is not None else None
    c = lambda t: None if t is None else t.detach().contiguous()
    W_h, w_ih, w_hh, b_ih, b_hh = c(W_h), c(gate.weight_ih_l0), c(gate.weight_hh_l0), c(gate.bias_ih_l0), c(gate.bias_hh_l0)
    Ws_next, W_final = c(Ws_next), c(W_final)
    scratch = dense_scratch(d, precision, agg.device)
    ev = None
    if DENSE_EVENTS is not None:
        ev = (torch.cuda.Event(enable_timing=True), torch.cuda.Event(enable_timing=True))
        ev[0].record()
    _lib.check(_lib.lib().rg_dense_fwd(n, d, ld, _lib.ptr(agg), _lib.ptr(hidden_prev), _lib.ptr(prev_idx), _lib.ptr(W_h),
                                       {"idd": 0, "relu": 1, "tanh": 2}[act], _lib.ptr(w_ih), _lib.ptr(w_hh), _lib.ptr(b_ih),
                                       _lib.ptr(b_hh), _lib.ptr(Ws_next), attn_dim, ap, _lib.ptr(a_s), _lib.ptr(W_final),
                                       _lib.ptr(nodes), n_ent, _lib.ptr(scores_all), _lib.ptr(hidden), DENSE_PRECISIONS[precision],
                                       _lib.ptr(scratch), 0 if scratch is None else scratch.numel(), _lib.stream_ptr()))
    if ev is not None:
        ev[1].record()
        DENSE_EVENTS.append((ev[0], ev[1], n))
    return hidden, a_s


def dense_fwd_dev(n_cap, count_ptr, agg, hidden_prev, prev_idx, d, W_h, act, gate, hidden_out, Ws_next=None, attn_dim=0, ap=0,
                  a_s_out=None, W_final=None, nodes=None, n_ent=0, scores_all=None, n_hint=0, precision="f32", scratch=None):
    ld = agg.shape[1]
    c = lambda t: None if t is None else t.detach().contiguous()
    W_h, w_ih, w_hh, b_ih, b_hh = c(W_h), c(gate.weight_ih_l0), c(gate.weight_hh_l0), c(gate.bias_ih_l0), c(gate.bias_hh_l0)
    Ws_next, W_final = c(Ws_next), c(W_final)
    if scratch is None:
        scratch = dense_scratch(d, precision, agg.device)
    _lib.check(_lib.lib().rg_dense_fwd_dev(n_cap, count_ptr, int(n_hint), d, ld, _lib.ptr(agg), _lib.ptr(hidden_prev), _lib.ptr(prev_idx),
                                           _lib.ptr(W_h), {"idd": 0, "relu": 1, "tanh": 2}[act], _lib.ptr(w_ih), _lib.ptr(w_hh),
                                           _lib.ptr(b_ih), _lib.ptr(b_hh), _lib.ptr(Ws_next), attn_dim, ap, _lib.ptr(a_s_out),
                                           _lib.ptr(W_final), _lib.ptr(nodes), n_ent, _lib.ptr(scores_all), _lib.ptr(hidden_out),
                                           DENSE_PRECISIONS[precision], _lib.ptr(scratch), 0 if scratch is None else scratch.numel(),
                                           _lib.stream_ptr()))


def dense_train_supported(d, act):
    return ((16 <= d <= 64 and d % 4 == 0) or d == 128) and act in ("idd", "relu", "tanh")


def dense_train_fwd(agg, hidden_prev, prev_idx, W_h, act, gate, mask=None, Ws_next=None):
    n, d = agg.shape
    dev = agg.device
    hidden = torch.empty((n, d), dtype=torch.float32, device=dev)
    x = torch.empty((n, d), dtype=torch.float32, device=dev)
    ws = torch.empty((n, 5 * d), dtype=torch.float32, device=dev)
    c = lambda t: None if t is None else t.detach().contiguous()
    common = (n, d, _lib.ptr(c(agg)), _lib.ptr(c(hidden_prev)), _lib.ptr(prev_idx), _lib.ptr(c(W_h)),
              {"idd": 0, "relu": 1, "tanh": 2}[act], _lib.ptr(c(gate.weight_ih_l0)), _lib.ptr(c(gate.weight_hh_l0)),
              _lib.ptr(c(gate.bias_ih_l0)), _lib.ptr(c(gate.bias_hh_l0)), _lib.ptr(c(mask)))
    if Ws_next is None:
        _lib.check(_lib.lib().rg_dense_train_fwd(*common, _lib.ptr(hidden), _lib.ptr(x), _lib.ptr(ws), _lib.stream_ptr()))
        return hidden, x, ws, None
    attn = Ws_next.shape[0]
    ap = (attn + 3) // 4 * 4
    a_s = torch.empty((n, ap), dtype=torch.float32, device=dev)
    _lib.check(_lib.lib().rg_dense_train_fwd_as(*common, _lib.ptr(c(Ws_next)), attn, ap, _lib.ptr(hidden), _lib.ptr(x), _lib.ptr(ws),
                                                _lib.ptr(a_s), _lib.stream_ptr()))
    return hidden, x, ws, a_s


def rows_addmm(base, g, W):
    assert base.is_cuda and base.dtype == g.dtype == W.dtype == torch.float32 and base.stride(1) == 1 and g.stride(1) == 1
    n_rows, n = base.shape
    k = W.shape[0]
    assert g.shape[0] == n_rows and g.shape[1] >= k and W.shape[1] == n
    out = torch.empty((n_rows, n), dtype=torch.float32, device=base.device)
    Wc = W.detach().contiguous()
    _lib.check(_lib.lib().rg_rows_addmm(C.c_void_p(base.data_ptr()), base.stride(0), C.c_void_p(g.data_ptr()), g.stride(0), k, _lib.ptr(Wc), n,
                                        n_rows, _lib.ptr(out), n, _lib.stream_ptr()))
    return out


def dense_train_bwd2(g_h, ws, x, mask, keep, act, W_h, w_ih, w_hh, prev_idx, n_old):
    n, d = x.shape
    dev = x.device
    f = lambda rows, cols: torch.empty((rows, cols), dtype=torch.float32, device=dev)
    dgi, dgh_n, dpre, dagg, g_prev = f(n, 3 * d), f(n, d), f(n, d), f(n, d), f(n_old, d)
    c = lambda t: None if t is None else t.detach().contiguous()
    _lib.check(_lib.lib().rg_dense_train_bwd2(n, d, _lib.ptr(c(g_h)), _lib.ptr(ws), _lib.ptr(x), _lib.ptr(c(mask)), float(keep),
                                              {"idd": 0, "relu": 1, "tanh": 2}[act], _lib.ptr(c(W_h)), _lib.ptr(c(w_ih)), _lib.ptr(c(w_hh)),
                                              _lib.ptr(prev_idx), _lib.ptr(dgi), _lib.ptr(dgh_n), _lib.ptr(dpre), _lib.ptr(dagg), _lib.ptr(g_prev),
                                              _lib.stream_ptr()))
    return dgi, dgh_n, dpre, dagg, g_prev


def dense_train_bwd_supported(d):
    return 16 <= d <= 64 and d % 4 == 0


def dense_train_bwd(g_h, ws, x, mask, keep, act, W_h, w_ih, w_hh):
    n, d = x.shape
    dev = x.device
    f = lambda cols: torch.empty((n, cols), dtype=torch.float32, device=dev)
    dgi, dgh, dpre, dagg, dh0 = f(3 * d), f(3 * d), f(d), f(d), f(d)
    c = lambda t: None if t is None else t.detach().contiguous()
    _lib.check(_lib.lib().rg_dense_train_bwd(n, d, _lib.ptr(c(g_h)), _lib.ptr(ws), _lib.ptr(x), _lib.ptr(c(mask)), float(keep),
                                             {"idd": 0, "relu": 1, "tanh": 2}[act], _lib.ptr(c(W_h)), _lib.ptr(c(w_ih)), _lib.ptr(c(w_hh)),
                                             _lib.ptr(dgi), _lib.ptr(dgh), _lib.ptr(dpre), _lib.ptr(dagg), _lib.ptr(dh0), _lib.stream_ptr()))
    return dgi, dgh, dpre, dagg, dh0


def attn_tables(layers, q_rel, d, ld, attn_dim, ap):
    L, dev = len(layers), q_rel.device
    n_rows, B = layers[0].rela_embed.weight.shape[0], q_rel.numel()
    a_r = torch.empty((L, n_rows, ap), dtype=torch.float32, device=dev)
    a_q = torch.empty((L, B, ap), dtype=torch.float32, device=dev)
    rela_p = torch.empty((L, n_rows, ld), dtype=torch.float32, device=dev) if ld != d else None
    arr = lambda ts: (C.c_void_p * L)(*[t.data_ptr() for t in ts])
    for l in layers:
        for t in (l.rela_embed.weight, l.Wr_attn.weight, l.Wqr_attn.weight, l.Wqr_attn.bias):
            assert t.is_contiguous() and t.dtype == torch.float32 and t.is_cuda
    assert q_rel.dtype == torch.int64 and q_rel.is_contiguous()
    _lib.check(_lib.lib().rg_attn_tables(L, n_rows, B, d, ld, attn_dim, ap, arr([l.rela_embed.weight for l in layers]),
                                         arr([l.Wr_attn.weight for l in layers]), arr([l.Wqr_attn.weight for l in layers]),
                                         arr([l.Wqr_attn.bias for l in layers]), _lib.ptr(q_rel), _lib.ptr(a_r), _lib.ptr(a_q),
                                         _lib.ptr(rela_p), _lib.stream_ptr()))
    return [(a_r[i], a_q[i], rela_p[i] if rela_p is not None else layers[i].rela_embed.weight) for i in range(L)]


def rank(scores, ans_ptr, ans_idx, filt_ptr, filt_idx):
    assert scores.is_cuda and scores.dtype == torch.float32 and scores.is_contiguous()
    B, n_ent = scores.shape
    out = torch.empty(ans_idx.numel(), dtype=torch.float32, device=scores.device)
    _lib.check(_lib.lib().rg_rank(_lib.ptr(scores), B, n_ent, _lib.ptr(ans_ptr), _lib.ptr(ans_idx),
                                  _lib.ptr(filt_ptr), _lib.ptr(filt_idx), _lib.ptr(out), _lib.stream_ptr()))
    return out


def topk(scores, k, q_key=None, known=None):
    assert scores.is_cuda and scores.dtype == torch.float32 and scores.is_contiguous() and scores.dim() == 2
    B, n_ent = scores.shape
    idx = torch.empty((B, k), dtype=torch.int32, device=scores.device)
    val = torch.empty((B, k), dtype=torch.float32, device=scores.device)
    if known is None or known[0].numel() == 0:
        keys = ptr = tails = q_key = None
        n_keys = 0
    else:
        keys, ptr, tails = known
        assert q_key is not None and q_key.dtype == torch.int64 and q_key.is_contiguous() and q_key.numel() == B
        assert keys.dtype == torch.int64 and ptr.dtype == torch.int64 and tails.dtype == torch.int32
        assert all(t.is_cuda and t.is_contiguous() for t in (q_key, keys, ptr, tails)) and ptr.numel() == keys.numel() + 1
        n_keys = keys.numel()
    _lib.check(_lib.lib().rg_topk(_lib.ptr(scores), B, n_ent, int(k), _lib.ptr(q_key), _lib.ptr(keys), _lib.ptr(ptr), _lib.ptr(tails),
                                  n_keys, _lib.ptr(idx), _lib.ptr(val), _lib.stream_ptr()))
    return idx, val
```

Measured before the change: 30.33 billion edges/s.

## Drive level-1 word-parallel layer from query subjects via out-edge positions

```diff
diff --git a/include/redgnn.h b/include/redgnn.h
--- a/include/redgnn.h
+++ b/include/redgnn.h
@@ -21,6 +21,7 @@
                            int add_inverse, void* stream, rg_graph** out);
 int rg_graph_export_packs(const rg_graph* g, int32_t* n_packs, int32_t* n_vrows, int32_t* ent_host, int32_t* pack_host, int32_t* rows_host,
                           int32_t* vrows_host);
+int rg_graph_export_out_pos(const rg_graph* g, int32_t* out_pos_host);
 int rg_tgraph_create(int32_t n_ent, int32_t n_rela_rows, int32_t n_time, const int32_t* quads_host, int64_t n,
                      rg_graph** out);
 int rg_tgraph_create_excluding(int32_t n_ent, int32_t n_rela_rows, int32_t n_time, const int32_t* quads_host, int64_t n,
diff --git a/red-gnn_amd/_lib.py b/red-gnn_amd/_lib.py
--- a/red-gnn_amd/_lib.py
+++ b/red-gnn_amd/_lib.py
@@ -6,7 +6,7 @@
 
 SYMBOLS = [
     "rg_last_error", "rg_version", "rg_hipgraph_fill_nodes",
-    "rg_graph_create", "rg_graph_create_device", "rg_graph_export_packs", "rg_tgraph_create", "rg_tgraph_create_excluding", "rg_graph_destroy", "rg_graph_n_fact", "rg_graph_export",
+    "rg_graph_create", "rg_graph_create_device", "rg_graph_export_packs", "rg_graph_export_out_pos", "rg_tgraph_create", "rg_tgraph_create_excluding", "rg_graph_destroy", "rg_graph_n_fact", "rg_graph_export",
     "rg_frontier_workspace_bytes", "rg_frontier_create", "rg_frontier_destroy", "rg_frontier_reset",
     "rg_frontier_reset_nodes", "rg_frontier_expand", "rg_frontier_nodes", "rg_frontier_edges_scratch_bytes", "rg_frontier_edges",
     "rg_layer_fwd_scratch_bytes", "rg_layer_fwd", "rg_layer_fwd_plan", "rg_tlayer_fwd", "rg_xlayer_fwd", "rg_frontier_set_window", "rg_layer_bwd_scratch_bytes", "rg_layer_bwd", "rg_tlayer_bwd_scratch_bytes", "rg_tlayer_bwd", "rg_xlayer_bwd", "rg_dense_fwd_supported", "rg_dense_scratch_bytes", "rg_dense_fwd", "rg_dense_fwd_dev", "rg_dense_train_fwd", "rg_dense_train_fwd_as", "rg_rows_addmm", "rg_dense_train_bwd", "rg_dense_train_bwd2", "rg_split3_roundtrip", "rg_split3_product_check", "rg_gram_tn_scratch_bytes", "rg_gram_tn", "rg_rank",
@@ -41,6 +41,7 @@
     L.rg_graph_create.argtypes = [i32, i32, vp, i64, C.c_int, C.POINTER(vp)]
     L.rg_graph_create_device.argtypes = [i32, i32, vp, i64, C.c_int, vp, C.POINTER(vp)]
     L.rg_graph_export_packs.argtypes = [vp, C.POINTER(i32), C.POINTER(i32), vp, vp, vp, vp]
+    L.rg_graph_export_out_pos.argtypes = [vp, vp]
     L.rg_tgraph_create.argtypes = [i32, i32, i32, vp, i64, C.POINTER(vp)]
     L.rg_tgraph_create_excluding.argtypes = [i32, i32, i32, vp, i64, vp, i64, C.POINTER(vp)]
     L.rg_graph_destroy.argtypes = [vp]
diff --git a/red-gnn_amd/csrc/common.h b/red-gnn_amd/csrc/common.h
--- a/red-gnn_amd/csrc/common.h
+++ b/red-gnn_amd/csrc/common.h
@@ -123,6 +123,7 @@
   uint32_t* out_pk = nullptr;
   rg_vrows in_vr, out_vr;
   rg_packs in_pk_packs;
+  int32_t* out_pos = nullptr;
   int32_t* rel_ptr = nullptr;
   int2* rel_ht = nullptr;
   rg_vrows rel_vr;
@@ -147,6 +148,8 @@
   const int32_t* win_lo = nullptr;
   const int32_t* win_hi = nullptr;
   int32_t win_n_data = 0;
+  int32_t* subjects = nullptr;
+  bool single_subjects = false;
   mutable bool queues_clean = false;
   int32_t* queues = nullptr;
   int64_t* counts_pinned = nullptr;
diff --git a/red-gnn_amd/csrc/frontier.hip b/red-gnn_amd/csrc/frontier.hip
--- a/red-gnn_amd/csrc/frontier.hip
+++ b/red-gnn_amd/csrc/frontier.hip
@@ -5,7 +5,7 @@
 namespace {
 
 __global__ void reset_level0_kernel(const int32_t* __restrict__ q_sub, int B, int n_ent, int BW, int W, uint32_t* __restrict__ bitsT,
-                                    int2* __restrict__ bm0, int32_t* __restrict__ counters) {
+                                    int2* __restrict__ bm0, int32_t* __restrict__ counters, int32_t* __restrict__ subjects) {
   const int64_t i = (int64_t)blockIdx.x * blockDim.x + threadIdx.x;
   if (i >= (int64_t)B * W) return;
   const int b = (int)(i / W), w = (int)(i - (int64_t)b * W);
@@ -14,6 +14,7 @@
   const int ew = ok ? e >> 5 : W;
   bm0[i] = make_int2(w == ew ? (int)(1u << (e & 31)) : 0, b + (w > ew ? 1 : 0));
   if (w == 0) {
+    subjects[b] = ok ? e : -1;
     if (ok) atomicOr(&bitsT[(int64_t)e * BW + (b >> 5)], 1u << (b & 31));
     else atomicOr((unsigned*)&counters[1], 1u);
     if (b == 0) { counters[0] = B; counters[4] = B; }
@@ -312,6 +313,7 @@
   off[4] = take(rg::scan_scratch_elems((int64_t)B * W) * 4);
   off[5] = take(1024 + RG_QUEUE_BYTES);
   off[6] = take((size_t)n_levels * B * W * 8);
+  off[7] = take((size_t)B * 4);
   return o;
 }
 
@@ -346,6 +348,7 @@
   f->scan_scratch = (int32_t*)(base + off[4]);
   f->counters = (int32_t*)(base + off[5]);
   f->queues = f->counters + 256;
+  f->subjects = (int32_t*)(base + off[7]);
   for (int l = 0; l < n_levels; ++l) f->bm[l] = (int2*)(base + off[6] + (size_t)l * batch * f->W * 8);
   if (hipHostMalloc((void**)&f->counts_pinned, 1024, hipHostMallocDefault) != hipSuccess) {
     delete f;
@@ -385,8 +388,9 @@
   f->queues_clean = false;
   const int64_t nw = (int64_t)f->B * f->W;
   hipLaunchKernelGGL(reset_level0_kernel, dim3(rg::ceil_div(nw, 256)), dim3(256), 0, s, q_sub, f->B, f->n_ent, f->BW, f->W,
-                     f->bitsT[0], f->bm[0], f->counters);
-  RG_LAUNCH_CHECK();
+                     f->bitsT[0], f->bm[0], f->counters, f->subjects);
+  RG_LAUNCH_CHECK();
+  f->single_subjects = true;
   f->n_nodes[0] = f->B;
   return 0;
 }
@@ -402,6 +406,7 @@
   RG_CHECK(f && (nodes || n == 0) && n >= 0, "rg_frontier_reset_nodes: bad argument");
   hipStream_t s = (hipStream_t)stream;
   f->level = 0; f->tcur = 0; f->n_edges = 0;
+  f->single_subjects = false;
   if (rg::zero2_async(f->bitsT[0], rg::align_up((size_t)f->n_ent * f->BW * 4, 16), f->counters, 1024, s)) return 1;
   f->queues_clean = false;
   if (n > 0) {
diff --git a/red-gnn_amd/csrc/graph.hip b/red-gnn_amd/csrc/graph.hip
--- a/red-gnn_amd/csrc/graph.hip
+++ b/red-gnn_amd/csrc/graph.hip
@@ -271,7 +271,7 @@
 extern "C" {
 
 const char* rg_last_error(void) { return rg::g_err.c_str(); }
-int rg_version(void) { return 10; }
+int rg_version(void) { return 11; }
 
 static int build_graph(int32_t n_ent, int32_t n_rel, int32_t n_rela_rows, const std::vector<int32_t>& H,
                        const std::vector<int32_t>& R, const std::vector<int32_t>& T, const std::vector<int32_t>* TIME,
@@ -362,9 +362,15 @@
   A.add(&g->out_vr.rows, hv_out.rows); A.add(&g->out_vr.split, hv_out.split);
   A.add(&g->rel_vr.rows, hv_rel.rows); A.add(&g->rel_vr.split, hv_rel.split);
   HostPacks hp;
+  std::vector<int32_t> out_pos;
   if (!TIME && !in_pk.empty() && n_rela_rows < (1 << 12)) {
     host_packs(hv_in.rows, in_pk, &hp, &g->in_pk_packs);
     A.add(&g->in_pk_packs.ent, hp.ent); A.add(&g->in_pk_packs.pack, hp.pack); A.add(&g->in_pk_packs.rows, hp.rows);
+    out_pos.resize(n_fact);
+    std::vector<int32_t> po(out_ptr.begin(), out_ptr.end() - 1);
+    for (size_t p = 0; p < hp.ent.size(); ++p)
+      if (hp.ent[p].x != -1) out_pos[po[hp.ent[p].x & 0xFFFFF]++] = (int32_t)p;
+    A.add(&g->out_pos, out_pos);
   }
 
   std::vector<char> staging(A.total);
@@ -488,4 +494,11 @@
   return 0;
 }
 
-}
+int rg_graph_export_out_pos(const rg_graph* g, int32_t* out_pos) {
+  RG_CHECK(g != nullptr && out_pos != nullptr, "rg_graph_export_out_pos: NULL argument");
+  RG_CHECK(g->out_pos != nullptr, "rg_graph_export_out_pos: the graph has no word-parallel packs (temporal graph, or ids too wide to pack)");
+  RG_HIP(hipMemcpy(out_pos, g->out_pos, (size_t)g->n_fact * sizeof(int32_t), hipMemcpyDeviceToHost));
+  return 0;
+}
+
+}
diff --git a/red-gnn_amd/csrc/graph_device.hip b/red-gnn_amd/csrc/graph_device.hip
--- a/red-gnn_amd/csrc/graph_device.hip
+++ b/red-gnn_amd/csrc/graph_device.hip
@@ -126,6 +126,11 @@
 __global__ void pack_count_kernel(const int32_t* __restrict__ pack_nrows, int4* __restrict__ pack, int n_packs) {
   const int p = blockIdx.x * blockDim.x + threadIdx.x;
   if (p < n_packs) pack[p].y = pack_nrows[p];
+}
+
+__global__ void ent_head_keys_kernel(const int2* __restrict__ ent, int64_t n, int n_ent, uint64_t* __restrict__ keys) {
+  const int64_t p = (int64_t)blockIdx.x * blockDim.x + threadIdx.x;
+  if (p < n) keys[p] = ent[p].x == -1 ? (uint64_t)n_ent : (uint64_t)(ent[p].x & 0xFFFFF);
 }
 
 __global__ void fill_int2_kernel(int2* __restrict__ p, int64_t n, int2 v) {
@@ -309,6 +314,7 @@
     add((void**)&g->in_pk_packs.ent, nullptr, (size_t)n_packs * RG_PACK * 8);
     add((void**)&g->in_pk_packs.pack, nullptr, (size_t)n_packs * 16);
     add((void**)&g->in_pk_packs.rows, nullptr, (size_t)g->in_vr.n * 8);
+    add((void**)&g->out_pos, nullptr, (size_t)n_fact * 4);
   }
   hipError_t e = hipMalloc(&g->arena, total);
   if (e != hipSuccess) {
@@ -327,6 +333,15 @@
     hipLaunchKernelGGL(pack_emit_kernel, dim3(g->in_vr.n), dim3(64), 0, s, g->in_vr.rows, place, g->in_vr.n, pack_row0, g->in_pk, g->in_pk_packs.ent,
                        g->in_pk_packs.pack, g->in_pk_packs.rows);
     hipLaunchKernelGGL(pack_count_kernel, dim3(blocks(n_packs)), dim3(256), 0, s, pack_nrows, g->in_pk_packs.pack, n_packs);
+    const int64_t n_pos = (int64_t)n_packs * RG_PACK;
+    uint64_t* pos_keys = tmp.get<uint64_t>(n_pos);
+    uint32_t* pos_sorted = tmp.get<uint32_t>(n_pos);
+    int pos_bits = 1;
+    while (((int64_t)1 << pos_bits) <= n_ent) ++pos_bits;
+    if (!pos_keys || !pos_sorted) { rg::set_error("rg_graph_create_device: out of device memory"); rg_graph_destroy(g); return 1; }
+    hipLaunchKernelGGL(ent_head_keys_kernel, dim3(blocks(n_pos)), dim3(256), 0, s, g->in_pk_packs.ent, n_pos, n_ent, pos_keys);
+    if (sort_perm(tmp, pos_keys, pos_bits, n_pos, pos_sorted, s)) { rg_graph_destroy(g); return 1; }
+    (void)hipMemcpyAsync(g->out_pos, pos_sorted, (size_t)n_fact * 4, hipMemcpyDeviceToDevice, s);
   }
   e = hipStreamSynchronize(s);
   if (e == hipSuccess) e = hipGetLastError();
diff --git a/red-gnn_amd/csrc/layer_fwd.hip b/red-gnn_amd/csrc/layer_fwd.hip
--- a/red-gnn_amd/csrc/layer_fwd.hip
+++ b/red-gnn_amd/csrc/layer_fwd.hip
@@ -32,7 +32,9 @@
   RG_CHECK(f && g && hidden && rela && a_s && a_r && a_q && w_alpha && b_alpha && agg_out, "rg_layer_fwd: NULL argument");
   RG_CHECK((((uintptr_t)hidden | (uintptr_t)rela | (uintptr_t)a_s | (uintptr_t)a_r | (uintptr_t)a_q | (uintptr_t)agg_out |
              (uintptr_t)scratch) & 15) == 0, "rg_layer_fwd: float buffers must be 16-B aligned");
-  RG_CHECK(walk >= 0 && walk <= 7, "rg_layer_fwd: walk=%d not in 0..7", walk);
+  RG_CHECK(walk >= 0 && walk <= 15, "rg_layer_fwd: walk=%d not in 0..15", walk);
+  const bool bitmap_fill = (walk & 8) != 0;
+  walk &= 7;
   rgfwd::FwdArgs A;
   if (rgfwd::fill_common("rg_layer_fwd", f, g, level, n_new, d, ld, ap, attn_dim, scratch, scratch_bytes,
                          rg_layer_fwd_scratch_bytes(f, g, ld), &A)) return 1;
@@ -64,9 +66,17 @@
     W.hidden = A.hidden; W.rela = A.rela; W.ld4 = A.ld4; W.a_s = A.a_s; W.a_r = A.a_r; W.a_q = A.a_q;
     W.w_alpha = w_alpha; W.b_alpha = b_alpha; W.attn_dim = attn_dim; W.n_rela_rows = g->n_rela_rows;
     W.agg = A.agg; W.partial = A.partial; W.queues = f->queues; W.queues_clean = A.walk.queues_clean;
+    const bool from_subjects = !bitmap_fill && level == 1 && f->single_subjects && g->out_pos != nullptr;
+    if (from_subjects) {
+      W.subjects = f->subjects; W.out_ptr = g->out_ptr; W.out_pos = g->out_pos; W.B = f->B;
+      W.n_chunk_items = (int64_t)f->B * rg::ceil_div(std::max(g->max_out_deg, 1), RG_PACK);
+      W.sub_l = (int32_t)std::max<int64_t>(std::min<int64_t>(W.n_chunk_items / 4096, 64), 1);
+      W.n_items = rg::ceil_div(W.n_chunk_items, W.sub_l);
+    }
     const int64_t n_e = level == f->level ? (f->n_edges >= 0 ? f->n_edges : f->edge_hint) : -1;
     const int64_t by_work = n_e < 0 ? 2 : 200 * W.n_items / std::max<int64_t>(n_e, 1);
     W.ipt = (int32_t)std::max<int64_t>(std::min<int64_t>(std::min<int64_t>(by_work, W.n_items / 8192), 32), 1);
+    if (from_subjects) W.ipt = 1;
     const size_t n_part = (size_t)f->B * g->in_vr.n_slots;
     W.written = n_part ? (uint8_t*)scratch + rg::align_up(n_part * ld * sizeof(float), 256) : nullptr;
     if (n_part && rg::zero_async(W.written, rg::align_up(n_part, 256), s)) return 1;
diff --git a/red-gnn_amd/csrc/layer_fwd_wp.h b/red-gnn_amd/csrc/layer_fwd_wp.h
--- a/red-gnn_amd/csrc/layer_fwd_wp.h
+++ b/red-gnn_amd/csrc/layer_fwd_wp.h
@@ -28,6 +28,11 @@
   int32_t* queues;
   int32_t ipt;
   bool queues_clean;
+  const int32_t* subjects = nullptr;
+  const int32_t* out_ptr = nullptr;
+  const int32_t* out_pos = nullptr;
+  int32_t B = 0, sub_l = 0;
+  int64_t n_chunk_items = 0;
 };
 
 int launch(const WpArgs& A, int ap4, hipStream_t s);
diff --git a/red-gnn_amd/csrc/layer_fwd_wp.hip b/red-gnn_amd/csrc/layer_fwd_wp.hip
--- a/red-gnn_amd/csrc/layer_fwd_wp.hip
+++ b/red-gnn_amd/csrc/layer_fwd_wp.hip
@@ -15,7 +15,7 @@
   return (uint32_t)__builtin_amdgcn_readfirstlane((int)v);
 }
 
-template <int G, int F, int AP4, bool RELA_LDS, bool EXACT>
+template <int G, int F, int AP4, bool RELA_LDS, bool EXACT, bool SUBJ>
 __global__ __launch_bounds__(WP_BLOCK, 4) void layer_fwd_wp_kernel(WpArgs A) {
   extern __shared__ float4 lds[];
   constexpr int GW = 64 / G, RW = G * F + 1;
@@ -84,6 +84,120 @@
       acc[f].z = fmaf(al, hv[f].z + rv.z, acc[f].z);
       acc[f].w = fmaf(al, hv[f].w + rv.w, acc[f].w);
     }
+  };
+
+  auto qbit = [](int key) -> int { return SUBJ ? key & 31 : key >> 8; };
+  auto run_queue = [&](const int qn, const int bw, const int row0) {
+    __builtin_amdgcn_fence(__ATOMIC_ACQ_REL, "wavefront");
+    __builtin_amdgcn_wave_barrier();
+    {
+      int2 en[4];
+      int s[4], out[4];
+      bool valid[4];
+#pragma unroll
+      for (int j = 0; j < 4; ++j) {
+        const int i = j * 64 + lane;
+        valid[j] = i < qn;
+        en[j] = valid[j] ? q8[i] : make_int2(0, -1);
+        const int prev_key = (valid[j] && i > 0) ? q8[i - 1].y : -2;
+        const unsigned long long hm = __ballot(valid[j] && en[j].y != prev_key);
+        if (lane == 0) hmask[j] = hm;
+      }
+      int2 wp[4], dst[4];
+#pragma unroll
+      for (int j = 0; j < 4; ++j) {
+        wp[j] = make_int2(0, 0); dst[j] = make_int2(0, 0);
+        if (valid[j]) {
+          const int hd = en[j].x & 0xFFFFF, bq = bw * 32 + qbit(en[j].y);
+          wp[j] = A.bm_old[(int64_t)bq * A.W + (hd >> 5)];
+          dst[j] = A.rows[SUBJ ? en[j].y >> 5 : row0 + (en[j].y & 255)];
+        }
+      }
+#pragma unroll
+      for (int j = 0; j < 4; ++j) {
+        s[j] = 0; out[j] = 0;
+        if (valid[j]) {
+          const int hd = en[j].x & 0xFFFFF, bq = bw * 32 + qbit(en[j].y);
+          s[j] = rg::bm_rank(wp[j], hd);
+          if (dst[j].y < 0) {
+            const int2 wn = A.bm_new[(int64_t)bq * A.W + (dst[j].x >> 5)];
+            out[j] = rg::bm_rank(wn, dst[j].x);
+          } else {
+            out[j] = -(bq * A.n_slots + dst[j].y) - 1;
+          }
+        }
+      }
+#pragma unroll
+      for (int j = 0; j < 4; ++j) {
+        if (valid[j]) {
+          const int r = (uint32_t)en[j].x >> 20;
+          const float4* aq_p = A.a_q + (int64_t)(bw * 32 + qbit(en[j].y)) * AP4;
+          float z = b_alpha;
+#pragma unroll
+          for (int k = 0; k < AP4; ++k) {
+            const float4 as = A.a_s[(int64_t)s[j] * AP4 + k];
+            const float4 ar = ar_l[r * AP4 + k];
+            const float4 w = w_l[k];
+            rg::attn_acc_fwd(z, w, as, ar, aq_p[k]);
+          }
+          const float alpha = rg::attn_alpha(z);
+          const uint32_t hoff = (uint32_t)s[j] * row_bytes;
+          const uint32_t roff = (uint32_t)r * (RELA_LDS ? (uint32_t)(RW * 16) : row_bytes);
+          st[j * 64 + lane] = make_float4(__int_as_float((int)hoff), __int_as_float((int)roff), alpha, __int_as_float(out[j]));
+        }
+      }
+    }
+    __builtin_amdgcn_fence(__ATOMIC_ACQ_REL, "wavefront");
+    __builtin_amdgcn_wave_barrier();
+    auto next_head = [&](int c) -> int {
+      int pos = qn;
+#pragma unroll
+      for (int w = 3; w >= 0; --w) {
+        unsigned long long m = hmask[w];
+        if (w == (c >> 6)) m &= ~0ull << (c & 63);
+        else if (w < (c >> 6)) m = 0ull;
+        if (m) pos = w * 64 + __ffsll((long long)m) - 1;
+      }
+      return pos;
+    };
+    int e = 0, end = qn;
+    if constexpr (GW > 1) {
+      e = gi_w == 0 ? 0 : next_head(gi_w * qn / GW);
+      end = gi_w == GW - 1 ? qn : next_head((gi_w + 1) * qn / GW);
+    }
+    if (e < end) {
+      float4 acc[F], hvA[F], hvB[F];
+#pragma unroll
+      for (int f = 0; f < F; ++f) acc[f] = rg::f4zero();
+      float4 tA = st[e], tB;
+      int cur = __float_as_int(tA.w);
+      gather(tA, hvA);
+      for (;;) {
+        tB = st[min(e + 1, end - 1)];
+        gather(tB, hvB);
+        consume(tA, hvA, acc);
+        if (e + 1 >= end || __float_as_int(tB.w) != cur) {
+          store_row(cur, acc);
+#pragma unroll
+          for (int f = 0; f < F; ++f) acc[f] = rg::f4zero();
+          cur = __float_as_int(tB.w);
+        }
+        if (e + 1 >= end) break;
+        tA = st[min(e + 2, end - 1)];
+        gather(tA, hvA);
+        consume(tB, hvB, acc);
+        if (e + 2 >= end || __float_as_int(tA.w) != cur) {
+          store_row(cur, acc);
+#pragma unroll
+          for (int f = 0; f < F; ++f) acc[f] = rg::f4zero();
+          cur = __float_as_int(tA.w);
+        }
+        if (e + 2 >= end) break;
+        e += 2;
+      }
+    }
+    __builtin_amdgcn_fence(__ATOMIC_ACQ_REL, "wavefront");
+    __builtin_amdgcn_wave_barrier();
   };
 
   auto run_item = [&](long long item) {
@@ -110,116 +224,74 @@
         qn += c0 + c1;
         todo &= todo - 1;
       }
-      __builtin_amdgcn_fence(__ATOMIC_ACQ_REL, "wavefront");
-      __builtin_amdgcn_wave_barrier();
-      {
-        int2 en[4];
-        int s[4], out[4];
-        bool valid[4];
-#pragma unroll
-        for (int j = 0; j < 4; ++j) {
-          const int i = j * 64 + lane;
-          valid[j] = i < qn;
-          en[j] = valid[j] ? q8[i] : make_int2(0, -1);
-          const int prev_key = (valid[j] && i > 0) ? q8[i - 1].y : -2;
-          const unsigned long long hm = __ballot(valid[j] && en[j].y != prev_key);
-          if (lane == 0) hmask[j] = hm;
-        }
-        int2 wp[4], dst[4];
-#pragma unroll
-        for (int j = 0; j < 4; ++j) {
-          wp[j] = make_int2(0, 0); dst[j] = make_int2(0, 0);
-          if (valid[j]) {
-            const int hd = en[j].x & 0xFFFFF, bq = bw * 32 + (en[j].y >> 8);
-            wp[j] = A.bm_old[(int64_t)bq * A.W + (hd >> 5)];
-            dst[j] = A.rows[row0 + (en[j].y & 255)];
-          }
-        }
-#pragma unroll
-        for (int j = 0; j < 4; ++j) {
-          s[j] = 0; out[j] = 0;
-          if (valid[j]) {
-            const int hd = en[j].x & 0xFFFFF, bq = bw * 32 + (en[j].y >> 8);
-            s[j] = rg::bm_rank(wp[j], hd);
-            if (dst[j].y < 0) {
-              const int2 wn = A.bm_new[(int64_t)bq * A.W + (dst[j].x >> 5)];
-              out[j] = rg::bm_rank(wn, dst[j].x);
-            } else {
-              out[j] = -(bq * A.n_slots + dst[j].y) - 1;
-            }
-          }
-        }
-#pragma unroll
-        for (int j = 0; j < 4; ++j) {
-          if (valid[j]) {
-            const int r = (uint32_t)en[j].x >> 20;
-            const float4* aq_p = A.a_q + (int64_t)(bw * 32 + (en[j].y >> 8)) * AP4;
-            float z = b_alpha;
-#pragma unroll
-            for (int k = 0; k < AP4; ++k) {
-              const float4 as = A.a_s[(int64_t)s[j] * AP4 + k];
-              const float4 ar = ar_l[r * AP4 + k];
-              const float4 w = w_l[k];
-              rg::attn_acc_fwd(z, w, as, ar, aq_p[k]);
-            }
-            const float alpha = rg::attn_alpha(z);
-            const uint32_t hoff = (uint32_t)s[j] * row_bytes;
-            const uint32_t roff = (uint32_t)r * (RELA_LDS ? (uint32_t)(RW * 16) : row_bytes);
-            st[j * 64 + lane] = make_float4(__int_as_float((int)hoff), __int_as_float((int)roff), alpha, __int_as_float(out[j]));
-          }
-        }
-      }
-      __builtin_amdgcn_fence(__ATOMIC_ACQ_REL, "wavefront");
-      __builtin_amdgcn_wave_barrier();
-      auto next_head = [&](int c) -> int {
-        int pos = qn;
-#pragma unroll
-        for (int w = 3; w >= 0; --w) {
-          unsigned long long m = hmask[w];
-          if (w == (c >> 6)) m &= ~0ull << (c & 63);
-          else if (w < (c >> 6)) m = 0ull;
-          if (m) pos = w * 64 + __ffsll((long long)m) - 1;
-        }
-        return pos;
-      };
-      int e = 0, end = qn;
-      if constexpr (GW > 1) {
-        e = gi_w == 0 ? 0 : next_head(gi_w * qn / GW);
-        end = gi_w == GW - 1 ? qn : next_head((gi_w + 1) * qn / GW);
-      }
-      if (e < end) {
-        float4 acc[F], hvA[F], hvB[F];
-#pragma unroll
-        for (int f = 0; f < F; ++f) acc[f] = rg::f4zero();
-        float4 tA = st[e], tB;
-        int cur = __float_as_int(tA.w);
-        gather(tA, hvA);
-        for (;;) {
-          tB = st[min(e + 1, end - 1)];
-          gather(tB, hvB);
-          consume(tA, hvA, acc);
-          if (e + 1 >= end || __float_as_int(tB.w) != cur) {
-            store_row(cur, acc);
-#pragma unroll
-            for (int f = 0; f < F; ++f) acc[f] = rg::f4zero();
-            cur = __float_as_int(tB.w);
-          }
-          if (e + 1 >= end) break;
-          tA = st[min(e + 2, end - 1)];
-          gather(tA, hvA);
-          consume(tB, hvB, acc);
-          if (e + 2 >= end || __float_as_int(tA.w) != cur) {
-            store_row(cur, acc);
-#pragma unroll
-            for (int f = 0; f < F; ++f) acc[f] = rg::f4zero();
-            cur = __float_as_int(tA.w);
-          }
-          if (e + 2 >= end) break;
-          e += 2;
-        }
-      }
-      __builtin_amdgcn_fence(__ATOMIC_ACQ_REL, "wavefront");
-      __builtin_amdgcn_wave_barrier();
+      run_queue(qn, bw, row0);
+    }
+  };
+
+  auto run_chunk = [&](const int q, const int c, const int beg, const int n) {
+    const int base = c * RG_PACK, rem = min(n - base, QCAP);
+    const int bw = q >> 5, b = q & 31;
+    int2 en[4];
+    int key[4], pos[4];
+#pragma unroll
+    for (int j = 0; j < 4; ++j) {
+      const int i = j * 64 + lane;
+      pos[j] = i < rem ? A.out_pos[beg + base + i] : -1;
+    }
+    const int prev0 = c > 0 ? A.out_pos[beg + base - 1] : -1;
+#pragma unroll
+    for (int j = 0; j < 4; ++j) {
+      en[j] = make_int2(0, 0);
+      key[j] = 0;
+      if (pos[j] >= 0) {
+        en[j] = A.ent[pos[j]];
+        key[j] = A.pack[pos[j] / RG_PACK].x;
+      }
+    }
+    int prev_key = -1;
+    if (prev0 >= 0) prev_key = A.pack[prev0 / RG_PACK].x + A.ent[prev0].y;
+    unsigned long long heads[4];
+#pragma unroll
+    for (int j = 0; j < 4; ++j) {
+      key[j] = pos[j] >= 0 ? key[j] + en[j].y : -1;
+      int before = __shfl_up(key[j], 1, 64);
+      if (lane == 0) before = prev_key;
+      heads[j] = __ballot(pos[j] >= 0 && key[j] != before);
+      prev_key = __shfl(key[j], 63, 64);
+    }
+    int start = rem, end = rem;
+    if (heads[1]) start = 64 + __ffsll((long long)heads[1]) - 1;
+    if (heads[0]) start = __ffsll((long long)heads[0]) - 1;
+    if (heads[3]) end = 192 + __ffsll((long long)heads[3]) - 1;
+    if (heads[2]) end = 128 + __ffsll((long long)heads[2]) - 1;
+    start = __builtin_amdgcn_readfirstlane(start);
+    end = __builtin_amdgcn_readfirstlane(end);
+    if (start >= end) return;
+#pragma unroll
+    for (int j = 0; j < 4; ++j) {
+      const int i = j * 64 + lane;
+      if (i >= start && i < end) q8[i - start] = make_int2(en[j].x, (key[j] << 5) | b);
+    }
+    run_queue(end - start, bw, 0);
+  };
+  auto run_subjects = [&](long long t) {
+    const long long it = t + (long long)lane * A.n_items;
+    int q = 0, c = 0, beg = 0, n = 0;
+    if (lane < A.sub_l && it < A.n_chunk_items) {
+      c = (int)(it / A.B);
+      q = (int)(it - (long long)c * A.B);
+      const int sub = A.subjects[q];
+      if (sub >= 0) {
+        beg = A.out_ptr[sub];
+        n = A.out_ptr[sub + 1] - beg;
+      }
+    }
+    unsigned long long m = __ballot(c * RG_PACK < n);
+    while (m) {
+      const int l = __ffsll((long long)m) - 1;
+      m &= m - 1;
+      run_chunk(__builtin_amdgcn_readfirstlane(__shfl(q, l, 64)), __builtin_amdgcn_readfirstlane(__shfl(c, l, 64)),
+                __builtin_amdgcn_readfirstlane(__shfl(beg, l, 64)), __builtin_amdgcn_readfirstlane(__shfl(n, l, 64)));
     }
   };
 
@@ -252,13 +324,16 @@
     const int cnt = resolve(off, &first);
     if (cnt == 0) break;
     off = ticket();
-    for (int k = 0; k < cnt; ++k) run_item(first + k);
+    for (int k = 0; k < cnt; ++k) {
+      if constexpr (SUBJ) run_subjects(first + k);
+      else run_item(first + k);
+    }
   }
 }
 
-template <int G, int F, int AP4, bool RELA_LDS, bool EXACT>
-int launch4(const WpArgs& A, size_t lds, hipStream_t s) {
-  auto kern = layer_fwd_wp_kernel<G, F, AP4, RELA_LDS, EXACT>;
+template <int G, int F, int AP4, bool RELA_LDS, bool EXACT, bool SUBJ>
+int launch5(const WpArgs& A, size_t lds, hipStream_t s) {
+  auto kern = layer_fwd_wp_kernel<G, F, AP4, RELA_LDS, EXACT, SUBJ>;
   if (lds > 64 * 1024) RG_HIP(hipFuncSetAttribute((const void*)kern, hipFuncAttributeMaxDynamicSharedMemorySize, (int)lds));
   const int per_cu = lds <= 80 * 1024 ? 2 : 1;
   const int grid = (int)std::max<int64_t>(std::min<int64_t>(rg::ceil_div(A.n_items, WP_WAVES * A.ipt), 256 * per_cu), 1);
@@ -268,6 +343,11 @@
   return 0;
 }
 
+template <int G, int F, int AP4, bool RELA_LDS, bool EXACT>
+int launch4(const WpArgs& A, size_t lds, hipStream_t s) {
+  return A.subjects ? launch5<G, F, AP4, RELA_LDS, EXACT, true>(A, lds, s) : launch5<G, F, AP4, RELA_LDS, EXACT, false>(A, lds, s);
+}
+
 template <int G, int F, int AP4, bool RELA_LDS>
 int launch3(const WpArgs& A, size_t lds, hipStream_t s) {
   if constexpr (G * F >= 16) {
diff --git a/red-gnn_amd/engine.py b/red-gnn_amd/engine.py
--- a/red-gnn_amd/engine.py
+++ b/red-gnn_amd/engine.py
@@ -75,6 +75,11 @@
         rows = np.empty((n_vrows.value if n_packs.value else 0, 2), np.int32)
         _lib.check(L.rg_graph_export_packs(self.handle, None, None, _lib.ptr(ent), _lib.ptr(pack), _lib.ptr(rows), _lib.ptr(vr)))
         return vr, ent, pack, rows
+
+    def export_out_pos(self):
+        pos = np.empty(self.n_fact, np.int32)
+        _lib.check(_lib.lib().rg_graph_export_out_pos(self.handle, _lib.ptr(pos)))
+        return pos
 
     def export(self):
         op = np.empty(self.n_ent + 1, np.int32)
@@ -434,7 +439,8 @@
     _lib.check(_lib.lib().rg_layer_fwd(frontier.handle, graph.handle, level, max(int(n_hint), 1),
                                        _lib.ptr(hidden), _lib.ptr(rela), d, ld, _lib.ptr(a_s), _lib.ptr(a_r),
                                        _lib.ptr(a_q), ap, _lib.ptr(w_alpha), _lib.ptr(b_alpha), attn_dim,
-                                       _lib.ptr(agg), _lib.ptr(scratch), scratch.numel(), FORCE_WALK or max(int(walk), 1), _lib.stream_ptr()))
+                                       _lib.ptr(agg), _lib.ptr(scratch), scratch.numel(), (FORCE_WALK & 7 or max(int(walk), 1)) | (FORCE_WALK & 8),
+                                       _lib.stream_ptr()))
 
 
 def tlayer_fwd(frontier, graph, level, n_new, q_time, hidden_dir, rela_dir, time_dir, d, a_s, a_r, a_q, w_alpha, b_alpha, attn_dim):
```

Measured after the change: 30.80 billion edges/s, median of 6. About the same (+1.5%).
